# rasd3/TODA

Hardware: AMD Instinct MI355X
Metric: LiDAR training samples/sec (higher is better)
Workload: dtype f32

## Files before the change

include/toda.h:

```cpp
#ifndef TODA_H_
#define TODA_H_

#include <stddef.h>
#include <stdint.h>

#ifdef __cplusplus
extern "C" {
#endif

#define TODA_OK 0
#define TODA_EINVAL (-1)
#define TODA_EWORKSPACE (-2)
#define TODA_ELAUNCH (-3)
#define TODA_EFAULT (-4)

#define TODA_FAULT_BN2D 1u
#define TODA_FAULT_WINO 2u
#define TODA_FAULT_FPS 4u

const char* toda_last_error(void);
int toda_abi_version(void);
int toda_device_fault(void);

size_t toda_voxelize_workspace_bytes(int n_points, int max_voxels);
int toda_voxelize_hard(const float* points, int n, int c,
                       const float* range_host ,
                       const float* vsize_host ,
                       const int32_t* grid_host ,
                       int max_pts, int max_voxels,
                       float* voxels, int32_t* coords_zyx, int32_t* num_pts,
                       int32_t* m_dev, void* ws, size_t ws_bytes, void* stream);
size_t toda_voxelize_batch_workspace_bytes(int batch, int n_cap);
int toda_voxelize_batch(const float* const* points_host, const int32_t* n_points_host, int batch, int n_cap,
                        int c, int row_stride,
                        const float* range_host, const float* vsize_host, const int32_t* grid_host,
                        int max_pts, int max_voxels,
                        float* voxels, int32_t* coords_bzyx, int32_t* num_pts, int32_t* counts_dev,
                        void* ws, size_t ws_bytes, int ws_clean, void* stream);

int toda_mean_vfe_fwd(const float* voxels, const float* num_pts, int m, int p, int c,
                      float* out, void* stream);
int toda_mean_vfe_bwd(const float* grad_out, const float* num_pts, int m, int p, int c,
                      float* grad_voxels, void* stream);

size_t toda_dynvox_workspace_bytes(int n, int batch, const int32_t* grid_host, int pillar);
int toda_dynvox_count(const float* points, int n, int width, int batch, const float* range_host, const float* vsize_host,
                      const int32_t* grid_host, int pillar, int32_t* counts_dev, void* ws, size_t ws_bytes, void* stream);
int toda_dynvox_index(const float* points, int n, int width, int batch, const float* range_host, const float* vsize_host,
                      const int32_t* grid_host, int pillar, int m, int k, uint8_t* keep, int32_t* rows, int32_t* inv,
                      int32_t* seg_pts, int32_t* seg_off, int32_t* cnt, int32_t* coords, void* ws, size_t ws_bytes,
                      void* stream);
int toda_dynvox_seg_sum(const float* src, int ld, int col0, int ncol, const int32_t* rowmap, const int32_t* seg_off,
                        const int32_t* seg_pts, int m, int divide, float* out, void* stream);
int toda_dynvox_pillar_decorate(const float* points, int width, const int32_t* rows, const int32_t* inv,
                                const int32_t* coords, const float* mean, int k, const float* vsize_host,
                                const float* offset_host, int use_abs_xyz, int with_dist, float* out, int f, void* stream);
int toda_dynvox_seg_max_fwd(const float* x, int c, const int32_t* seg_off, const int32_t* seg_pts, int m, float* out,
                            int32_t* arg, void* stream);
int toda_dynvox_seg_max_bwd(const float* gout, const int32_t* arg, int m, int c, int k, float* gx, void* stream);
int toda_dynvox_gather_concat(const float* x, const float* xmax, const int32_t* inv, int k, int c, float* out, void* stream);

size_t toda_gridindex_bytes(int batch, const int32_t* shape_host );
int toda_gridindex_from_coords(const int32_t* idx, int n, const int32_t* n_dev,
                               int batch, const int32_t* shape_host,
                               void* gi, int32_t* rowof, void* stream);
int toda_gridindex_from_coords_unordered(const int32_t* idx, int n, const int32_t* n_dev,
                                         int batch, const int32_t* shape_host,
                                         void* gi, int32_t* rowof, int gi_clean, void* stream);
int toda_gridindex_clear(const int32_t* idx, int n, const int32_t* n_dev, int batch,
                         const int32_t* shape_host, void* gi, void* stream);
int toda_gridindex_from_conv(const int32_t* idx_in, int n_in, const int32_t* n_in_dev,
                             int batch, const int32_t* shape_in_host,
                             const int32_t* ksize_host, const int32_t* stride_host,
                             const int32_t* pad_host, const int32_t* shape_out_host,
                             void* gi_out, int32_t* idx_out, int32_t* n_out_dev,
                             int out_cap, void* stream);
int toda_gridindex_from_bitmap(const void* gi_in, int batch, const int32_t* shape_in_host,
                               const int32_t* ksize_host, const int32_t* stride_host,
                               const int32_t* pad_host, const int32_t* shape_out_host,
                               void* gi_out, int32_t* idx_out, int32_t* n_out_dev,
                               int out_cap, int in_rows_marked, void* stream);

int toda_rulebook_subm(const int32_t* idx, int n, int batch, const int32_t* shape_host,
                       const int32_t* ksize_host, const int32_t* dilation_host,
                       const void* gi, const int32_t* rowof,
                       int32_t* nbr, int32_t* pair_cnt, int cnt_zeroed, void* stream);
int toda_rulebook_conv(const int32_t* idx_in, int n_in, int batch,
                       const int32_t* shape_in_host, const int32_t* ksize_host,
                       const int32_t* stride_host, const int32_t* pad_host,
                       const int32_t* shape_out_host, const void* gi_out, int n_out,
                       int32_t* nbr_o2i, int32_t* nbr_i2o, int32_t* pair_cnt,
                       const int32_t* idx_out, const void* gi_in, const int32_t* rowof_in,
                       int cnt_zeroed, void* stream);

size_t toda_spconv_packed_weight_floats(int k_vol, int c_gather, int c_produce);
int toda_matrix_path(void);
int toda_set_matrix_path(int mode);
int toda_spconv_split_supported(int c_gather, int c_produce);
int toda_spconv_pack_weight(const float* w, int cout, int k_vol, int cin,
                            int transpose, int flip_k, float* wp, void* stream);
int toda_spconv_pack_weights(int n, const float* const* w_host, const int32_t* cout_host, const int32_t* k_vol_host,
                             const int32_t* cin_host, const int32_t* transpose_host, const int32_t* flip_k_host,
                             float* const* wp_host, void* stream);
int toda_spconv_gather_gemm(const float* in, int n_in, int c_gather, const float* wp,
                            const int32_t* nbr, int n_out, int k_vol, int c_produce,
                            const float* bias , float* out, void* stream);
int toda_spconv_gather_gemm_ordered(const float* in, int n_in, int c_gather, const float* wp,
                                    const int32_t* nbr, int n_out, int k_vol, int c_produce,
                                    const float* bias, float* out, const int32_t* order, void* stream);

int toda_rulebook_class_order(const int32_t* in_coords, int n_in, const int32_t* stride_host, const int32_t* padding_host,
                              int32_t* order, unsigned char* cls_sorted, void* stream);
int toda_spconv_gather_gemm_classed(const float* in, int n_in, int c_gather, const float* wp, const int32_t* nbr, int n_out,
                                    int k_vol, int c_produce, const float* bias, float* out, const int32_t* order,
                                    const unsigned char* cls_sorted, const int32_t* ksize_host, const int32_t* stride_host,
                                    const int32_t* padding_host, void* stream);
int toda_spconv_gather_gemm_compact_supported(int c_gather, int c_produce, int k_vol);
int toda_spconv_gather_gemm_compact(const float* in, int n_in, int c_gather, const float* w, int w_cout, int w_cin,
                                    int transpose, int flip_k, const int32_t* nbr, int n_out, int k_vol, int c_produce,
                                    const float* bias , float* out, void* stream);
size_t toda_spconv_gather_gemm_compact_stats_doubles(int n_out, int c_produce);
int toda_spconv_gather_gemm_compact_stats(const float* in, int n_in, int c_gather, const float* w, int w_cout, int w_cin,
                                          int transpose, int flip_k, const int32_t* nbr, int n_out, int k_vol,
                                          int c_produce, const float* bias , float* out, double* sums,
                                          size_t sums_doubles, int* blocks_out , void* stream);

size_t toda_spconv_wgrad_workspace_bytes(int n_out, int k_vol, int cin, int cout);
int toda_spconv_wgrad(const float* in, int n_in, const float* dout, const int32_t* nbr,
                      int n_out, int k_vol, int cin, int cout, float* dw,
                      void* ws, size_t ws_bytes, void* stream);
int toda_sparse_to_dense_fwd(const float* feat, const int32_t* idx, int n, int c,
                             int batch, const int32_t* shape_host, float* dense, void* stream);
int toda_sparse_to_dense_bwd(const float* grad_dense, const int32_t* idx, int n, int c,
                             int batch, const int32_t* shape_host, float* grad_feat, void* stream);

int toda_pillar_scatter_fwd(const float* feat, const int32_t* idx, int n, int c,
                            int batch, int ny, int nx, float* canvas, void* stream);
int toda_pillar_scatter_bwd(const float* grad_canvas, const int32_t* idx, int n, int c,
                            int batch, int ny, int nx, float* grad_feat, void* stream);

size_t toda_rows_reduce_doubles(int n, int c);
int toda_rows_moments(const float* x, int n, int c, double* sums ,
                      void* stream);
int toda_rows_affine_act(const float* x, const float* scale, const float* shift,
                         const float* residual , int n, int c, int relu,
                         float* y, void* stream);

int toda_bn_finalize(const double* sums , int n, int c,
                     const float* gamma, const float* beta, float* running_mean ,
                     float* running_var , float momentum, float eps, int training,
                     float* mean, float* invstd, float* scale, float* shift, void* stream);
int toda_bn_finalize_partials(double* sums, int blocks, int n, int c, const float* gamma, const float* beta,
                              float* running_mean , float* running_var , float momentum, float eps,
                              float* mean, float* invstd, float* scale, float* shift, void* stream);
int toda_rows_bn_bwd(const float* dy, const float* x, const float* stats, const float* gamma,
                     int n, int c, int relu, double* sums , float* dx,
                     void* stream);

int toda_rows_bn_bwd_res(const float* dy, const float* x, const float* residual , const float* stats,
                         const float* gamma, int n, int c, int relu, double* sums, float* dx,
                         float* dres , void* stream);
size_t toda_rows_bn_bwd_colsum_doubles(int n, int c);
int toda_rows_bn_bwd_res_colsum(const float* dy, const float* x, const float* residual , const float* stats,
                                const float* gamma, int n, int c, int relu, double* sums, float* dx,
                                float* dres , double* colsum_ws , float* dx_colsum ,
                                void* stream);

int toda_bn2d_supported(int batch, int c, int hw);
size_t toda_bn2d_sync_bytes(void);
int toda_bn2d_fwd(const float* x, int batch, int c, int hw, const float* gamma, const float* beta,
                  float* running_mean , float* running_var , float momentum, float eps, int relu,
                  float* y, float* save, void* sync , unsigned epoch, void* stream);
int toda_bn2d_bwd(const float* x, const float* dy, int batch, int c, int hw, const float* gamma, const float* beta,
                  const float* save, int relu, float* dx, float* dgamma, float* dbeta, void* sync ,
                  unsigned epoch, void* stream);
int toda_bn2d_fwd_into(const float* x, int batch, int c, int hw, const float* gamma, const float* beta,
                       float* running_mean , float* running_var , float momentum, float eps, int relu,
                       float* y, int y_channels, int y_channel0, float* save, void* sync , unsigned epoch,
                       void* stream);
int toda_bn2d_bwd_from(const float* x, const float* dy, int dy_channels, int dy_channel0, int batch, int c, int hw,
                       const float* gamma, const float* beta, const float* save, int relu, float* dx, float* dgamma,
                       float* dbeta, void* sync , unsigned epoch, void* stream);

int toda_center_assign(const float* gt_boxes, int batch, int n_gt, int code_size,
                       int num_classes, int fm_w, int fm_h,
                       const float* range_host , const float* vsize_host ,
                       int fm_stride, int max_objs, double gaussian_overlap, int min_radius,
                       float* heatmap ,
                       float* ret_boxes ,
                       int64_t* inds , int64_t* mask ,
                       void* stream);

size_t toda_anchor_assign_workspace_bytes(int batch, int n_gt);
int toda_anchor_assign(const void* const* anchors_host, const int32_t* locs_host, const int32_t* per_loc_host,
                       const float* matched_host, const float* unmatched_host, int n_classes, int anchor_stride,
                       const float* gt_boxes, int batch, int n_gt, int gt_stride, const int32_t* slot_of, int n_ids,
                       int code_size, int encode_angle_by_sincos, int multihead_order,
                       int32_t* labels , float* targets , float* weights ,
                       void* ws, size_t ws_bytes, void* stream);

int toda_boxes_iou_bev(const float* boxes_a, int na, const float* boxes_b, int nb,
                       float* iou , void* stream);
int toda_boxes_overlap_bev(const float* boxes_a, int na, const float* boxes_b, int nb,
                           float* overlap , void* stream);
size_t toda_nms_workspace_bytes(int n);
int toda_nms_rotated(const float* boxes_sorted, int n, float thresh, int64_t* keep ,
                     int32_t* n_keep_dev, void* ws, size_t ws_bytes, void* stream);

int toda_roi_grid_pool_bev(const float* feat, int B, int C, int H, int W, const float* rois, int N, int roi_stride,
                           float min_x, float min_y, float step_x, float step_y, int grid_size, float* out, void* stream);
int toda_roi_iou3d_max(const float* rois, int B, int N, int roi_stride, const int64_t* roi_labels, const float* gt, int M,
                       int gt_stride, int by_class, float* max_iou , int64_t* argmax , void* stream);

int toda_voxel_query(const float* new_xyz, const int32_t* new_coords, int M, const float* xyz, int N, const void* gi, const int32_t* rowof,
                     int batch, const int32_t* shape_host, float radius, const int32_t* ranges_host, int nsample, int32_t* idx,
                     uint8_t* empty, void* stream);
size_t toda_voxel_pool_moments_doubles(void);
int toda_voxel_pool_moments(const int32_t* idx, const uint8_t* empty, int M, int nsample, const float* xyz, int N, const float* new_xyz,
                            double* ws, void* stream);
int toda_voxel_pool_fwd(const float* f, int N, int C, const int32_t* idx, const uint8_t* empty, int M, int nsample, const float* xyz,
                        const float* new_xyz, const float* ab, float* out, uint8_t* arg, void* stream);
size_t toda_voxel_pool_table_bytes(int M, int nsample, int N);
int toda_voxel_pool_table(const int32_t* idx, const uint8_t* empty, int M, int nsample, int N, int32_t* off, int32_t* ent, void* ws,
                          size_t ws_bytes, void* stream);
int toda_voxel_pool_bwd_feat(const float* gout, const uint8_t* arg, int M, int nsample, int C, const int32_t* off, const int32_t* ent,
                             int N, float* gf, void* stream);
size_t toda_voxel_pool_bwd_pos_doubles(int C);
int toda_voxel_pool_bwd_pos(const float* gout, const uint8_t* arg, const int32_t* idx, const uint8_t* empty, int M, int nsample, int C,
                            const float* xyz, int N, const float* new_xyz, double* ws, float* gab, void* stream);

int toda_fps_resident_blocks(void);
size_t toda_fps_workspace_bytes(int batch, int npoint);
int toda_fps(const float* xyz, const int32_t* starts_host, int batch, int npoint, int mode, float* temp, int32_t* idx, void* ws,
             size_t ws_bytes, void* stream);
int toda_ball_query_stack(const float* xyz, int N, const int32_t* xyz_start, const float* new_xyz, const int32_t* new_start, int batch,
                          int M, int nr, const float* radii_host, const int32_t* nsample_host, int32_t* const* idx_host,
                          uint8_t* const* empty_host, void* stream);
int toda_sa_gather_fwd(const float* P, int N, int C, const float* wd, const int32_t* idx, const uint8_t* empty, int M, int nsample,
                       const float* xyz, const float* new_xyz, float* z, void* stream);
int toda_sa_gather_bwd_feat(const float* gz, int M, int nsample, int C, const int32_t* off, const int32_t* ent, int N, float* gP,
                            void* stream);
size_t toda_sa_gather_bwd_pos_doubles(int C);
int toda_sa_gather_bwd_pos(const float* gz, const int32_t* idx, const uint8_t* empty, int M, int nsample, int C, const float* xyz, int N,
                           const float* new_xyz, double* ws, float* gwd, void* stream);
int toda_sa_max_fwd(const float* y, int M, int nsample, int C, float* out, uint8_t* arg, void* stream);
int toda_sa_max_bwd(const float* g, const uint8_t* arg, int M, int nsample, int C, float* gy, void* stream);
int toda_bev_interp_fwd(const float* map, int B, int C, int H, int W, const float* xy, const int32_t* bidx, int K, float* out,
                        int32_t* taps, float* wts, void* stream);
int toda_bev_interp_bwd(const float* g, int K, int C, const int32_t* off, const int32_t* ent, const float* wts, int B, int H, int W,
                        float* gmap, void* stream);

int toda_points_in_boxes(const float* points, int n, const int32_t* n_dev, int c, const float* boxes,
                         int k, int box_stride, int mode, int32_t* flags, void* stream);
int toda_points_sector(const float* points, int n, const int32_t* n_dev, int c, double lo, double hi,
                       int32_t* flags, void* stream);
int toda_points_rect(const float* points, int n, const int32_t* n_dev, int c, const double* lo_xy_host,
                     const double* hi_xy_host, int closed, int32_t* flags, void* stream);
int toda_points_polar_cell(const float* points, int n, const int32_t* n_dev, int c, float phase,
                           const double* yaw_edges_host, int n_yaw, const double* dis_edges_host, int n_dis,
                           float dis_lo, float dis_hi, int32_t* cell, void* stream);
int toda_points_polar_select(const float* points, int n, const int32_t* n_dev, int c, double lo, double hi, int yaw_mode,
                             int dis_mode, double dis_th, const float* pitch_range_dev, int32_t* flags, void* stream);
size_t toda_points_pitch_range_workspace_bytes(void);
int toda_points_pitch_range(const float* points, int n, const int32_t* n_dev, int c, float* range_dev, void* ws,
                            size_t ws_bytes, void* stream);
int toda_points_pitch_band(const float* points, int n, const int32_t* n_dev, int c, float z_offset, float clip_lo,
                           float clip_hi, const double* edges_host, int n_bands, int32_t* band, void* stream);
size_t toda_rows_select_workspace_bytes(int n);
int toda_rows_select_append(const float* src, int n, const int32_t* n_dev, int c, const int32_t* keys,
                            int match, int invert, float* dst, int cap_rows, int32_t* cursor_dev,
                            void* ws, size_t ws_bytes, void* stream);
int toda_points_rotate_z(const float* src, int n, const int32_t* n_dev, int c, double cosv, double sinv,
                         float* dst, void* stream);
int toda_points_world_transform(const float* src, int n, const int32_t* n_dev, int c, int flip_x, int flip_y,
                                int rotate, float cosv, float sinv, int rescale, float scale, float* dst,
                                void* stream);

int toda_points_box_steps_chunk(void);
int toda_points_box_steps(const float* src, int n, const int32_t* n_dev, int c, const double* steps, int n_steps,
                          float* dst, int32_t* keep, void* stream);
size_t toda_points_column_range_workspace_bytes(void);
int toda_points_column_range(const float* points, int n, const int32_t* n_dev, int c, int col, float* range_dev,
                             void* ws, size_t ws_bytes, void* stream);
int toda_points_in_pyramids(const float* points, int n, const int32_t* n_dev, int c, const double* pyramids, int np,
                            uint32_t* bits, int32_t* counts, void* stream);

int toda_points_fov_flags(const float* points, int n, const int32_t* n_dev, int c, const float* m_host,
                          const float* p2_host, int img_h, int img_w, int32_t* flags, void* stream);

int toda_sweeps_merge_max_sweeps(void);
int toda_sweeps_merge(const float* rows, int n, int n_sweeps, const int32_t* offsets_host, const double* matrices_host,
                      const int32_t* has_matrix_host, const int32_t* drop_ego_host, const double* time_lags_host,
                      float radius, const float* shift_host, float* out, int32_t* flags, void* stream);

int toda_waymo_frame(const float* rows, int n, int c_in, int use_nlz, float* out, int32_t* flags, void* stream);

int toda_spconv_gather_gemm_stats_supported(int c_gather, int c_produce);
size_t toda_spconv_gather_gemm_stats_doubles(int n_out, int c_produce);
int toda_spconv_gather_gemm_stats(const float* in, int n_in, int c_gather, const float* packed_w, const int32_t* nbr,
                                  int n_out, int k_vol, int c_produce, const float* bias, float* out, double* sums,
                                  size_t sums_doubles, void* stream);
int toda_spconv_gather_gemm_stats_partials(const float* in, int n_in, int c_gather, const float* wp, const int32_t* nbr,
                                           int n_out, int k_vol, int c_produce, const float* bias , float* out,
                                           double* sums, size_t sums_doubles, int* blocks_out, void* stream);

int toda_conv3x3_supported(int batch, int cin, int cout, int H, int W);
size_t toda_conv3x3_weight_floats(int cout, int cin);
int toda_conv3x3_transform_weight(const float* w, int cout, int cin, int mode, float* u, void* stream);
typedef struct toda_conv3x3_weight_entry {
    const float* w;
    int32_t cout, cin, mode, reserved;
    float* u;
} toda_conv3x3_weight_entry;
int toda_conv3x3_transform_weight_batch(const toda_conv3x3_weight_entry* table_host, int n, void* stream);
size_t toda_conv3x3_workspace_bytes(void);
size_t toda_conv3x3_wgrad_workspace_bytes(int batch, int cin, int cout, int H, int W);
int toda_conv3x3_wgrad(const float* x, const float* dy, int batch, int cin, int cout, int H, int W, float* dw,
                       void* ws, size_t ws_bytes, void* stream);
int toda_conv3x3_fwd(const float* x, const float* u, const float* bias, int batch, int cin, int cout, int H,
                     int W, float* y, void* ws, size_t ws_bytes, void* stream);

int toda_conv3x3s2_supported(int batch, int cin, int cout, int H, int W);
int toda_conv3x3s2_fwd(const float* x, const float* w, int batch, int cin, int cout, int H, int W, float* y, void* stream);
int toda_conv3x3s2_dgrad(const float* dy, const float* w, int batch, int cin, int cout, int H, int W, float* dx, void* stream);
size_t toda_conv3x3s2_wgrad_workspace_bytes(int batch, int cin, int cout, int H, int W);
int toda_conv3x3s2_wgrad(const float* x, const float* dy, int batch, int cin, int cout, int H, int W, float* dw, void* ws,
                         size_t ws_bytes, void* stream);
int toda_deconv_supported(int batch, int cin, int cout, int H, int W, int s);
int toda_deconv_fwd(const float* x, const float* w, int batch, int cin, int cout, int H, int W, int s, float* y, void* stream);
int toda_deconv_dgrad(const float* dy, const float* w, int batch, int cin, int cout, int H, int W, int s, float* dx, void* stream);
size_t toda_deconv_wgrad_workspace_bytes(int batch, int cin, int cout, int H, int W, int s);
int toda_deconv_wgrad(const float* x, const float* dy, int batch, int cin, int cout, int H, int W, int s, float* dw, void* ws,
                      size_t ws_bytes, void* stream);

size_t toda_center_loss_workspace_bytes(int batch, int classes, int H, int W, int max_objs, int code_size);
int toda_center_loss_fwd(const float* hm_logits, const float* heatmap, int batch, int classes, int H, int W, int n_branch,
                         const float* const* reg_maps_host, const int32_t* reg_channels_host, const int64_t* inds,
                         const int64_t* mask, const float* target_boxes, int max_objs, int code_size,
                         const float* code_weights_host, float cls_weight, float loc_weight, float* hm_prob, float* out4,
                         void* ws, size_t ws_bytes, void* stream);
int toda_center_loss_bwd(const float* out4, const float* up_hm, const float* up_loc, int batch, int classes, int H, int W,
                         int n_branch, float* const* reg_grads_host, const int32_t* reg_channels_host, const int64_t* inds,
                         const int64_t* mask, int max_objs, int code_size, const float* code_weights_host, float cls_weight, float loc_weight,
                         float* hm_grad, const void* ws, size_t ws_bytes, void* stream);

int toda_conv3x3_narrow_supported(int batch, int cin, int cout, int H, int W);
int toda_conv3x3_narrow_fwd(int n, const float* const* x_host, const float* const* w_host, const float* const* bias_host,
                            const int32_t* cout_host, int batch, int cin, int H, int W, long long x_image_stride,
                            float* const* y_host, void* stream);
int toda_conv3x3_narrow_dgrad(int n, const float* const* dy_host, const float* const* w_host, const int32_t* cout_host,
                              int batch, int cin, int H, int W, long long dx_image_stride, float* const* dx_host, void* stream);
size_t toda_conv3x3_narrow_wgrad_workspace_bytes(int n, int batch, int cin, int H);
int toda_conv3x3_narrow_wgrad(int n, const float* const* x_host, const float* const* dy_host, const int32_t* cout_host,
                              int batch, int cin, int H, int W, long long x_image_stride, float* out, void* ws, size_t ws_bytes,
                              void* stream);

int toda_timing_begin(int capacity);
int toda_timing_end(float* ms_out_host, int cap, int* n_out_host);

int toda_clip_adam_chunk(void);
int toda_clip_adam_step(const unsigned long long* param, const unsigned long long* grad, const unsigned long long* exp_avg,
                        const unsigned long long* exp_avg_sq, const long long* numel, const int* chunk_tensor,
                        const long long* chunk_off, int n_chunks, double* partial, float* norm_out, float max_norm,
                        float lr, float beta1, float beta2, float eps, float weight_decay, int step, void* stream);

int toda_eval_overlaps(const float* box3d, const float* bbox, const int32_t* box_off, const float* query3d,
                       const float* query_bbox, const int32_t* query_off, const long long* out_off, int n_frames,
                       long long n_pairs, int metric, int criterion, float* out, void* stream);
size_t toda_eval_match_workspace_bytes(int n_frames, int n_thresh, int n_det_total);
int toda_eval_match_scores(const float* overlaps, const long long* ov_off, const int32_t* det_off, const int32_t* gt_off,
                           const int32_t* ign_det, const int32_t* ign_gt, const double* det_score, int n_frames,
                           int n_det_total, double min_overlap, double* scores_out, int32_t* count_out, void* ws,
                           size_t ws_bytes, void* stream);
int toda_eval_match(const float* overlaps, const long long* ov_off, const int32_t* det_off, const int32_t* gt_off,
                    const int32_t* ign_det, const int32_t* ign_gt, const double* det_score, const double* det_alpha,
                    const double* gt_alpha, const double* det_bbox, const double* dc_bbox, const int32_t* dc_off, int n_frames,
                    int n_det_total, const double* thresholds, int n_thresh, double min_overlap, int metric, int compute_aos,
                    double* pr, void* ws, size_t ws_bytes, void* stream);

#ifdef __cplusplus
}
#endif
#endif
```

toda_amd/csrc/bn_fold.cuh:

```cuda
#pragma once
#include "common.h"

namespace toda {

constexpr int DN_BLOCK = 256;

__device__ __forceinline__ double fold_column(const double* __restrict__ src, int blocks, double* part) {
    double acc = 0.0;
    for (int g = threadIdx.x; g < blocks; g += DN_BLOCK) acc += src[g];
    part[threadIdx.x] = acc;
    __syncthreads();
    for (int w = DN_BLOCK / 2; w > 0; w >>= 1) {
        if (threadIdx.x < w) part[threadIdx.x] += part[threadIdx.x + w];
        __syncthreads();
    }
    return part[0];
}

__device__ __forceinline__ void bn_write_channel(int ch, float mean, float var, float eps, const float* __restrict__ gamma,
                                                 const float* __restrict__ beta, float* __restrict__ mean_out,
                                                 float* __restrict__ invstd_out, float* __restrict__ scale_out,
                                                 float* __restrict__ shift_out) {
    const float invstd = 1.0f / sqrtf(var + eps);
    const float g = gamma ? gamma[ch] : 1.0f, b = beta ? beta[ch] : 0.0f;
    mean_out[ch] = mean;
    invstd_out[ch] = invstd;
    scale_out[ch] = g * invstd;
    shift_out[ch] = b - mean * g * invstd;
}

__device__ __forceinline__ void bn_train_channel(int ch, double sum, double sumsq, int n, const float* __restrict__ gamma,
                                                 const float* __restrict__ beta, float* __restrict__ running_mean,
                                                 float* __restrict__ running_var, float momentum, float eps,
                                                 float* __restrict__ mean_out, float* __restrict__ invstd_out,
                                                 float* __restrict__ scale_out, float* __restrict__ shift_out) {
    const double m = sum / (double)n;
    double v = sumsq / (double)n - m * m;
    if (v < 0.0) v = 0.0;
    const float mean = (float)m, var = (float)v;
    if (running_mean) {
        const double unbiased = n > 1 ? v * (double)n / (double)(n - 1) : v;
        running_mean[ch] = (1.0f - momentum) * running_mean[ch] + momentum * mean;
        running_var[ch] = (1.0f - momentum) * running_var[ch] + momentum * (float)unbiased;
    }
    bn_write_channel(ch, mean, var, eps, gamma, beta, mean_out, invstd_out, scale_out, shift_out);
}

__global__ void __launch_bounds__(DN_BLOCK) fold_partials_kernel(double* __restrict__ sums, int blocks, int cols);

}
```

toda_amd/csrc/dense.hip:

```cpp
#include "bn_fold.cuh"
#include "common.h"

namespace toda {

typedef float f32x4 __attribute__((ext_vector_type(4)));

constexpr int DN_ROWS = 64;
constexpr int DN_CH = 32;

struct DenseGeom {
    int D, H, W;
    int pillar;
};

__device__ __forceinline__ long long spatial_offset(const int4 q, const DenseGeom& g) {
    if (g.pillar) return (long long)q.y + (long long)q.z * g.W + q.w;
    return ((long long)q.y * g.H + q.z) * g.W + q.w;
}

template <bool FWD>
__global__ void __launch_bounds__(DN_BLOCK)
dense_tile_kernel(float* __restrict__ feat, const int4* __restrict__ idx, int n, int c, DenseGeom g,
                  float* __restrict__ dense) {
    __shared__ float tile[DN_CH][DN_ROWS + 1];
    __shared__ long long base[DN_ROWS];
    const int row0 = blockIdx.x * DN_ROWS, c0 = blockIdx.y * DN_CH;
    const long long vol = (long long)g.D * g.H * g.W;
    if (threadIdx.x < DN_ROWS) {
        const int r = row0 + threadIdx.x;
        long long b = -1;
        if (r < n) {
            const int4 q = idx[r];
            b = (long long)q.x * c * vol + spatial_offset(q, g);
        }
        base[threadIdx.x] = b;
    }
    const int fr = threadIdx.x >> 2, fc = (threadIdx.x & 3) * 8;
    const int dr = threadIdx.x & 63, dc = threadIdx.x >> 6;
    if (FWD) {
        if (row0 + fr < n) {
#pragma unroll
            for (int j = 0; j < 8; ++j) {
                const int ch = c0 + fc + j;
                tile[fc + j][fr] = ch < c ? feat[(size_t)(row0 + fr) * c + ch] : 0.f;
            }
        }
        __syncthreads();
        const long long b = base[dr];
        if (b >= 0) {
#pragma unroll
            for (int j = 0; j < DN_CH / 4; ++j) {
                const int ch = dc + 4 * j;
                if (c0 + ch < c) dense[b + (long long)(c0 + ch) * vol] = tile[ch][dr];
            }
        }
    } else {
        __syncthreads();
        const long long b = base[dr];
#pragma unroll
        for (int j = 0; j < DN_CH / 4; ++j) {
            const int ch = dc + 4 * j;
            tile[ch][dr] = (b >= 0 && c0 + ch < c) ? dense[b + (long long)(c0 + ch) * vol] : 0.f;
        }
        __syncthreads();
        if (row0 + fr < n) {
#pragma unroll
            for (int j = 0; j < 8; ++j) {
                const int ch = c0 + fc + j;
                if (ch < c) feat[(size_t)(row0 + fr) * c + ch] = tile[fc + j][fr];
            }
        }
    }
}

#ifndef TODA_MOM_ROWS
#define TODA_MOM_ROWS 256
#endif
constexpr int MOM_ROWS = TODA_MOM_ROWS;
constexpr int MOM_MAX_BLOCKS = 2048;

template <class Load>
__device__ __forceinline__ void rows_reduce2(int n, int c, int rows_per_block, Load load, double* __restrict__ sums) {
    __shared__ float sh[2][DN_BLOCK][4];
    const int lanes = c >> 2;
    const int rows_par = DN_BLOCK / lanes;
    const int cl = threadIdx.x % lanes, rsub = threadIdx.x / lanes;
    const int row_begin = blockIdx.x * rows_per_block;
    const int row_end = min(n, row_begin + rows_per_block);
    f32x4 s0 = f32x4{0.f, 0.f, 0.f, 0.f}, t0 = s0, s1 = s0, t1 = s0;
    int r = row_begin + rsub;
    for (; r + rows_par < row_end; r += 2 * rows_par) {
        f32x4 a, b, a2, b2;
        load(r, cl, a, b);
        load(r + rows_par, cl, a2, b2);
        s0 += a;
        t0 += b;
        s1 += a2;
        t1 += b2;
    }
    if (r < row_end) {
        f32x4 a, b;
        load(r, cl, a, b);
        s0 += a;
        t0 += b;
    }
    s0 += s1;
    t0 += t1;
#pragma unroll
    for (int j = 0; j < 4; ++j) {
        sh[0][threadIdx.x][j] = s0[j];
        sh[1][threadIdx.x][j] = t0[j];
    }
    __syncthreads();
    if (threadIdx.x < 2 * c) {
        const int q = threadIdx.x / c, ch = threadIdx.x % c;
        double acc = 0.0;
        for (int j = 0; j < rows_par; ++j) acc += sh[q][j * lanes + (ch >> 2)][ch & 3];
        sums[2 * c + (size_t)(q * c + ch) * gridDim.x + blockIdx.x] = acc;
    }
}

__global__ void __launch_bounds__(DN_BLOCK)
fold_partials_kernel(double* __restrict__ sums, int blocks, int cols) {
    __shared__ double part[DN_BLOCK];
    const double total = fold_column(sums + cols + (size_t)blockIdx.x * blocks, blocks, part);
    if (threadIdx.x == 0) sums[blockIdx.x] = total;
}

static inline void reduce_plan(int n, int* blocks, int* rows_per_block) {
    const int g = cdiv(n > 0 ? n : 1, MOM_ROWS);
    *blocks = g < MOM_MAX_BLOCKS ? g : MOM_MAX_BLOCKS;
    *rows_per_block = cdiv(n > 0 ? n : 1, *blocks);
}

__global__ void __launch_bounds__(DN_BLOCK)
rows_moments_kernel(const float* __restrict__ x, int n, int c, int rows_per_block, double* __restrict__ sums) {
    const f32x4* x4 = reinterpret_cast<const f32x4*>(x);
    const int lanes = c >> 2;
    rows_reduce2(n, c, rows_per_block, [&](int r, int cl, f32x4& a, f32x4& b) {
        a = x4[(size_t)r * lanes + cl];
        b = a * a;
    }, sums);
}

constexpr int EW_BLOCKS = 2048;

__global__ void __launch_bounds__(DN_BLOCK)
rows_affine_act_kernel(const f32x4* __restrict__ x, const float* __restrict__ scale, const float* __restrict__ shift,
                       const f32x4* __restrict__ res, long long n4, int c, int relu, f32x4* __restrict__ y) {
    const long long t0 = (long long)blockIdx.x * DN_BLOCK + threadIdx.x;
    const long long stride = (long long)gridDim.x * DN_BLOCK;
    const int ch = (int)((t0 * 4) % c);
    const f32x4 sc = *reinterpret_cast<const f32x4*>(scale + ch), sf = *reinterpret_cast<const f32x4*>(shift + ch);
    for (long long t = t0; t < n4; t += stride) {
        f32x4 v = x[t] * sc + sf;
        if (res) v += res[t];
        if (relu) {
#pragma unroll
            for (int j = 0; j < 4; ++j) v[j] = fmaxf(v[j], 0.f);
        }
        y[t] = v;
    }
}

__global__ void __launch_bounds__(DN_BLOCK)
rows_bn_bwd_reduce_kernel(const float* __restrict__ dy, const float* __restrict__ x, const float* __restrict__ res,
                          const float* __restrict__ stats, int n, int c, int relu, int rows_per_block,
                          double* __restrict__ sums) {
    const f32x4* dy4 = reinterpret_cast<const f32x4*>(dy);
    const f32x4* x4 = reinterpret_cast<const f32x4*>(x);
    const f32x4* r4 = reinterpret_cast<const f32x4*>(res);
    const int lanes = c >> 2;
    const int cl0 = threadIdx.x % lanes;
    const f32x4 mu = reinterpret_cast<const f32x4*>(stats)[cl0];
    const f32x4 is = reinterpret_cast<const f32x4*>(stats + c)[cl0];
    const f32x4 sc = reinterpret_cast<const f32x4*>(stats + 2 * c)[cl0];
    const f32x4 sf = reinterpret_cast<const f32x4*>(stats + 3 * c)[cl0];
    rows_reduce2(n, c, rows_per_block, [&](int r, int cl, f32x4& a, f32x4& b) {
        const f32x4 g = dy4[(size_t)r * lanes + cl], xv = x4[(size_t)r * lanes + cl];
        const f32x4 rv = r4 ? r4[(size_t)r * lanes + cl] : f32x4{0.f, 0.f, 0.f, 0.f};
#pragma unroll
        for (int j = 0; j < 4; ++j) {
            float pre = xv[j] * sc[j] + sf[j];
            if (r4) pre += rv[j];
            const float dz = (relu && !(pre > 0.f)) ? 0.f : g[j];
            a[j] = dz;
            b[j] = dz * ((xv[j] - mu[j]) * is[j]);
        }
    }, sums);
}

__global__ void __launch_bounds__(DN_BLOCK)
rows_bn_bwd_apply_kernel(const f32x4* __restrict__ dy, const f32x4* __restrict__ x, const f32x4* __restrict__ res,
                         const float* __restrict__ stats, const float* __restrict__ gamma, double* __restrict__ sums,
                         long long n4, int c, int n, int relu, f32x4* __restrict__ dx, f32x4* __restrict__ dres,
                         double* __restrict__ colsum_part) {
    if (blockIdx.x == 0 && threadIdx.x < 2 * c) reinterpret_cast<float*>(sums + 2 * c)[threadIdx.x] = (float)sums[threadIdx.x];
    const long long t0 = (long long)blockIdx.x * DN_BLOCK + threadIdx.x;
    const long long stride = (long long)gridDim.x * DN_BLOCK;
    const int ch = (int)((t0 * 4) % c);
    const float inv_n = 1.0f / (float)n;
    const f32x4 mu = *reinterpret_cast<const f32x4*>(stats + ch);
    const f32x4 is = *reinterpret_cast<const f32x4*>(stats + c + ch);
    const f32x4 sc = *reinterpret_cast<const f32x4*>(stats + 2 * c + ch);
    const f32x4 sf = *reinterpret_cast<const f32x4*>(stats + 3 * c + ch);
    const f32x4 ga = *reinterpret_cast<const f32x4*>(gamma + ch);
    f32x4 m1, m2;
#pragma unroll
    for (int j = 0; j < 4; ++j) {
        m1[j] = (float)(sums[ch + j] * (double)inv_n);
        m2[j] = (float)(sums[c + ch + j] * (double)inv_n);
    }
    const f32x4 k1 = ga * is, k2 = is * m2;
    f32x4 csum = {0.f, 0.f, 0.f, 0.f};
    for (long long t = t0; t < n4; t += stride) {
        const f32x4 g = dy[t], xv = x[t];
        const f32x4 rv = res ? res[t] : f32x4{0.f, 0.f, 0.f, 0.f};
        f32x4 out, dzv;
#pragma unroll
        for (int j = 0; j < 4; ++j) {
            float pre = xv[j] * sc[j] + sf[j];
            if (res) pre += rv[j];
            const float dz = (relu && !(pre > 0.f)) ? 0.f : g[j];
            dzv[j] = dz;
            out[j] = k1[j] * (dz - m1[j] - (xv[j] - mu[j]) * k2[j]);
        }
        dx[t] = out;
        csum += out;
        if (dres) dres[t] = dzv;
    }
    if (colsum_part) {
        __shared__ float cs[DN_BLOCK][4];
#pragma unroll
        for (int j = 0; j < 4; ++j) cs[threadIdx.x][j] = csum[j];
        __syncthreads();
        if (threadIdx.x < c) {
            const int lanes = c >> 2, cl = threadIdx.x >> 2, j = threadIdx.x & 3;
            double acc = 0.0;
            for (int t = cl; t < DN_BLOCK; t += lanes) acc += (double)cs[t][j];
            colsum_part[(size_t)threadIdx.x * gridDim.x + blockIdx.x] = acc;
        }
    }
}

__global__ void __launch_bounds__(DN_BLOCK)
colsum_fold_kernel(const double* __restrict__ part, int blocks, float* __restrict__ out) {
    __shared__ double sh[DN_BLOCK];
    const double total = fold_column(part + (size_t)blockIdx.x * blocks, blocks, sh);
    if (threadIdx.x == 0) out[blockIdx.x] = (float)total;
}

__global__ void __launch_bounds__(DN_BLOCK)
bn_finalize_kernel(const double* __restrict__ sums, int n, int c, const float* __restrict__ gamma,
                   const float* __restrict__ beta, float* __restrict__ running_mean, float* __restrict__ running_var,
                   float momentum, float eps, int training, float* __restrict__ mean_out, float* __restrict__ invstd_out,
                   float* __restrict__ scale_out, float* __restrict__ shift_out) {
    const int ch = threadIdx.x;
    if (ch >= c) return;
    if (training)
        bn_train_channel(ch, sums[ch], sums[c + ch], n, gamma, beta, running_mean, running_var, momentum, eps, mean_out, invstd_out,
                         scale_out, shift_out);
    else
        bn_write_channel(ch, running_mean[ch], running_var[ch], eps, gamma, beta, mean_out, invstd_out, scale_out, shift_out);
}

__global__ void __launch_bounds__(DN_BLOCK)
bn_fold_finalize_kernel(double* __restrict__ sums, int blocks, int n, int c, const float* __restrict__ gamma,
                        const float* __restrict__ beta, float* __restrict__ running_mean, float* __restrict__ running_var,
                        float momentum, float eps, float* __restrict__ mean_out, float* __restrict__ invstd_out,
                        float* __restrict__ scale_out, float* __restrict__ shift_out) {
    __shared__ double part[DN_BLOCK];
    const int ch = blockIdx.x;
    const double sum = fold_column(sums + 2 * c + (size_t)ch * blocks, blocks, part);
    __syncthreads();
    const double sumsq = fold_column(sums + 2 * c + (size_t)(c + ch) * blocks, blocks, part);
    if (threadIdx.x != 0) return;
    sums[ch] = sum;
    sums[c + ch] = sumsq;
    bn_train_channel(ch, sum, sumsq, n, gamma, beta, running_mean, running_var, momentum, eps, mean_out, invstd_out, scale_out,
                     shift_out);
}

static int ew_grid(long long n4, int c) {
    long long blocks = (n4 + DN_BLOCK - 1) / DN_BLOCK;
    if (blocks > EW_BLOCKS) blocks = EW_BLOCKS;
    while ((blocks * DN_BLOCK * 4) % c != 0) ++blocks;
    return (int)blocks;
}

static int scatter_common(bool fwd, float* feat, const int32_t* idx, int n, int c, int batch, DenseGeom g,
                          float* dense, hipStream_t s) {
    TODA_CHECK_ARG(n >= 0 && c >= 1 && batch >= 1, "sparse<->dense: bad sizes n=%d c=%d batch=%d", n, c, batch);
    const size_t total = (size_t)batch * c * g.D * g.H * g.W;
    if (fwd) TODA_HIP(hipMemsetAsync(dense, 0, total * sizeof(float), s));
    if (n == 0) return TODA_OK;
    const dim3 grid(cdiv(n, DN_ROWS), cdiv(c, DN_CH));
    if (fwd)
        hipLaunchKernelGGL(HIP_KERNEL_NAME(dense_tile_kernel<true>), grid, dim3(DN_BLOCK), 0, s, feat, (const int4*)idx, n,
                           c, g, dense);
    else
        hipLaunchKernelGGL(HIP_KERNEL_NAME(dense_tile_kernel<false>), grid, dim3(DN_BLOCK), 0, s, feat, (const int4*)idx, n,
                           c, g, dense);
    TODA_LAUNCH_CHECK();
    return TODA_OK;
}

}

using namespace toda;

extern "C" int toda_sparse_to_dense_fwd(const float* feat, const int32_t* idx, int n, int c, int batch,
                                        const int32_t* shape_host, float* dense, void* stream) {
    const DenseGeom g{shape_host[0], shape_host[1], shape_host[2], 0};
    return scatter_common(true, const_cast<float*>(feat), idx, n, c, batch, g, dense, (hipStream_t)stream);
}
extern "C" int toda_sparse_to_dense_bwd(const float* grad_dense, const int32_t* idx, int n, int c, int batch,
                                        const int32_t* shape_host, float* grad_feat, void* stream) {
    const DenseGeom g{shape_host[0], shape_host[1], shape_host[2], 0};
    return scatter_common(false, grad_feat, idx, n, c, batch, g, const_cast<float*>(grad_dense), (hipStream_t)stream);
}
extern "C" int toda_pillar_scatter_fwd(const float* feat, const int32_t* idx, int n, int c, int batch, int ny, int nx,
                                       float* canvas, void* stream) {
    const DenseGeom g{1, ny, nx, 1};
    return scatter_common(true, const_cast<float*>(feat), idx, n, c, batch, g, canvas, (hipStream_t)stream);
}
extern "C" int toda_pillar_scatter_bwd(const float* grad_canvas, const int32_t* idx, int n, int c, int batch, int ny,
                                       int nx, float* grad_feat, void* stream) {
    const DenseGeom g{1, ny, nx, 1};
    return scatter_common(false, grad_feat, idx, n, c, batch, g, const_cast<float*>(grad_canvas), (hipStream_t)stream);
}

extern "C" size_t toda_rows_reduce_doubles(int n, int c) {
    int blocks, rpb;
    reduce_plan(n, &blocks, &rpb);
    return (size_t)2 * c * (1 + (size_t)blocks);
}

extern "C" int toda_rows_moments(const float* x, int n, int c, double* sums, void* stream) {
    hipStream_t s = (hipStream_t)stream;
    TODA_CHECK_ARG(c >= 4 && c % 4 == 0 && c <= DN_BLOCK / 2 && DN_BLOCK % c == 0,
                   "rows_moments: channels must be a multiple of 4 dividing 256, <= 128 (got %d)", c);
    if (n <= 0) {
        TODA_HIP(hipMemsetAsync(sums, 0, 2 * c * sizeof(double), s));
        return TODA_OK;
    }
    int blocks, rpb;
    reduce_plan(n, &blocks, &rpb);
    hipLaunchKernelGGL(rows_moments_kernel, dim3(blocks), dim3(DN_BLOCK), 0, s, x, n, c, rpb, sums);
    hipLaunchKernelGGL(fold_partials_kernel, dim3(2 * c), dim3(DN_BLOCK), 0, s, sums, blocks, 2 * c);
    TODA_LAUNCH_CHECK();
    return TODA_OK;
}

extern "C" int toda_rows_affine_act(const float* x, const float* scale, const float* shift, const float* residual,
                                    int n, int c, int relu, float* y, void* stream) {
    TODA_CHECK_ARG(c >= 4 && c % 4 == 0 && c <= 1024, "rows_affine_act: channels must be a multiple of 4, <= 1024 (got %d)", c);
    if (n <= 0) return TODA_OK;
    const long long n4 = (long long)n * c / 4;
    hipLaunchKernelGGL(rows_affine_act_kernel, dim3(ew_grid(n4, c)), dim3(DN_BLOCK), 0, (hipStream_t)stream,
                       (const f32x4*)x, scale, shift, (const f32x4*)residual, n4, c, relu, (f32x4*)y);
    TODA_LAUNCH_CHECK();
    return TODA_OK;
}

extern "C" size_t toda_rows_bn_bwd_colsum_doubles(int n, int c) {
    if (n <= 0 || c < 4) return 1;
    return (size_t)c * ew_grid((long long)n * c / 4, c);
}

extern "C" int toda_rows_bn_bwd_res_colsum(const float* dy, const float* x, const float* residual, const float* stats,
                                           const float* gamma, int n, int c, int relu, double* sums, float* dx, float* dres,
                                           double* colsum_ws, float* dx_colsum, void* stream) {
    hipStream_t s = (hipStream_t)stream;
    TODA_CHECK_ARG((colsum_ws == nullptr) == (dx_colsum == nullptr), "rows_bn_bwd: colsum workspace and result go together");
    TODA_CHECK_ARG(c >= 4 && c % 4 == 0 && c <= DN_BLOCK / 2 && DN_BLOCK % c == 0,
                   "rows_bn_bwd: channels must be a multiple of 4 dividing 256, <= 128 (got %d)", c);
    if (n <= 0) {
        TODA_HIP(hipMemsetAsync(sums, 0, 3 * c * sizeof(double), s));
        if (dx_colsum) TODA_HIP(hipMemsetAsync(dx_colsum, 0, c * sizeof(float), s));
        return TODA_OK;
    }
    int blocks, rpb;
    reduce_plan(n, &blocks, &rpb);
    hipLaunchKernelGGL(rows_bn_bwd_reduce_kernel, dim3(blocks), dim3(DN_BLOCK), 0, s, dy, x, residual, stats, n, c, relu, rpb, sums);
    hipLaunchKernelGGL(fold_partials_kernel, dim3(2 * c), dim3(DN_BLOCK), 0, s, sums, blocks, 2 * c);
    const long long n4 = (long long)n * c / 4;
    const int grid = ew_grid(n4, c);
    hipLaunchKernelGGL(rows_bn_bwd_apply_kernel, dim3(grid), dim3(DN_BLOCK), 0, s, (const f32x4*)dy,
                       (const f32x4*)x, (const f32x4*)residual, stats, gamma, sums, n4, c, n, relu, (f32x4*)dx, (f32x4*)dres, colsum_ws);
    if (dx_colsum) hipLaunchKernelGGL(colsum_fold_kernel, dim3(c), dim3(DN_BLOCK), 0, s, (const double*)colsum_ws, grid, dx_colsum);
    TODA_LAUNCH_CHECK();
    return TODA_OK;
}

extern "C" int toda_rows_bn_bwd_res(const float* dy, const float* x, const float* residual, const float* stats,
                                    const float* gamma, int n, int c, int relu, double* sums, float* dx, float* dres,
                                    void* stream) {
    return toda_rows_bn_bwd_res_colsum(dy, x, residual, stats, gamma, n, c, relu, sums, dx, dres, nullptr, nullptr, stream);
}

extern "C" int toda_rows_bn_bwd(const float* dy, const float* x, const float* stats, const float* gamma, int n, int c,
                                int relu, double* sums, float* dx, void* stream) {
    return toda_rows_bn_bwd_res(dy, x, nullptr, stats, gamma, n, c, relu, sums, dx, nullptr, stream);
}

extern "C" int toda_bn_finalize_partials(double* sums, int blocks, int n, int c, const float* gamma, const float* beta,
                                         float* running_mean, float* running_var, float momentum, float eps, float* mean,
                                         float* invstd, float* scale, float* shift, void* stream) {
    TODA_CHECK_ARG(sums && mean && invstd && scale && shift, "bn_finalize_partials: null argument");
    TODA_CHECK_ARG(c >= 1 && c <= DN_BLOCK && blocks >= 1 && n >= 1, "bn_finalize_partials: channels must be <= 256, blocks and rows >= 1 (got %d, %d, %d)", c,
                   blocks, n);
    TODA_CHECK_ARG((running_mean == nullptr) == (running_var == nullptr), "bn_finalize_partials: running_mean and running_var go together");
    hipLaunchKernelGGL(bn_fold_finalize_kernel, dim3(c), dim3(DN_BLOCK), 0, (hipStream_t)stream, sums, blocks, n, c, gamma, beta, running_mean,
                       running_var, momentum, eps, mean, invstd, scale, shift);
    TODA_LAUNCH_CHECK();
    return TODA_OK;
}

extern "C" int toda_bn_finalize(const double* sums, int n, int c, const float* gamma, const float* beta,
                                float* running_mean, float* running_var, float momentum, float eps, int training,
                                float* mean, float* invstd, float* scale, float* shift, void* stream) {
    TODA_CHECK_ARG(c >= 1 && c <= DN_BLOCK, "bn_finalize: channels must be <= 256 (got %d)", c);
    TODA_CHECK_ARG(training || (running_mean && running_var), "bn_finalize: eval mode needs running statistics");
    TODA_CHECK_ARG(!training || n >= 1, "bn_finalize: training mode needs rows >= 1 (got %d)", n);
    hipLaunchKernelGGL(bn_finalize_kernel, dim3(1), dim3(DN_BLOCK), 0, (hipStream_t)stream, sums, n, c, gamma, beta,
                       running_mean, running_var, momentum, eps, training, mean, invstd, scale, shift);
    TODA_LAUNCH_CHECK();
    return TODA_OK;
}
```

toda_amd/csrc/spconv.hip:

```cpp
#include <stdlib.h>

#include <type_traits>

#include <hip/hip_ext.h>

#include <mutex>
#include <vector>

#include "bn_fold.cuh"
#include "common.h"


namespace toda {

typedef float f32x4 __attribute__((ext_vector_type(4)));

constexpr int SC_BLOCK = 256;

static int tiles_pow2(int channels) {
    int t = (channels + 15) / 16, p = 1;
    while (p < t) p <<= 1;
    return p;
}

// ... 919 lines not shown
    int max_chunks = env_chunks > 0 ? env_chunks : ((tiles_pow2(cin) * tiles_pow2(cout) >= 16) ? 48 : 144);
    if (env_chunks <= 0 && k_vol <= 9) max_chunks *= 2;
    int ch = k_vol <= 9 ? n_out / 1024 : n_out / 2048;
    if (ch < 1) ch = 1;
    if (ch > max_chunks) ch = max_chunks;
    if (env_chunks <= 0 && k_vol > 9 && max_chunks == 48 && n_out / 4096 > 48) ch = n_out / 4096 < 96 ? n_out / 4096 : 96;
    if (ch >= 8) ch = (ch + 7) / 8 * 8;
    int rpc = (n_out + ch - 1) / ch;
    rpc = (rpc + 15) / 16 * 16;
    if (rpc < 16) rpc = 16;
    *rows_per_chunk = rpc;
    *chunks = n_out > 0 ? (n_out + rpc - 1) / rpc : 1;
}

}

#include "spconv_split.cuh"

using namespace toda;

#include <atomic>
static std::atomic<int> g_matrix_path{-1};
static int matrix_path() {
    int m = g_matrix_path.load(std::memory_order_relaxed);
    if (m < 0) {
        const char* e = getenv("TODA_MM");
        m = (e && (e[0] == 'n' || e[0] == '0')) ? 0 : 1;
        g_matrix_path.store(m, std::memory_order_relaxed);
    }
    return m;
}
static inline bool use_split(int c_gather, int c_produce) { return matrix_path() == 1 && toda::split_shape_ok(c_gather, c_produce); }

extern "C" int toda_matrix_path(void) { return matrix_path(); }
extern "C" int toda_set_matrix_path(int mode) {
    TODA_CHECK_ARG(mode == 0 || mode == 1, "set_matrix_path: mode must be 0 (native) or 1 (split)");
    g_matrix_path.store(mode, std::memory_order_relaxed);
    return TODA_OK;
}
extern "C" int toda_spconv_split_supported(int c_gather, int c_produce) { return toda::split_shape_ok(c_gather, c_produce) ? 1 : 0; }

extern "C" size_t toda_spconv_packed_weight_floats(int k_vol, int c_gather, int c_produce) {
    const size_t native = (size_t)k_vol * tiles_pow2(c_gather) * tiles_pow2(c_produce) * 256;
    if (!toda::split_shape_ok(c_gather, c_produce)) return native;
    const size_t split = toda::split_packed_bytes(k_vol, c_gather, c_produce) / 4;
    return split > native ? split : native;
}

static void split_pack_fill(toda::SplitPackBatch& b, int i, const float* w, int cout, int k_vol, int cin, int transpose, int flip_k, float* wp) {
    const int cgather = transpose ? cout : cin, cprod = transpose ? cin : cout;
    b.w[i] = w, b.wps[i] = reinterpret_cast<toda::u32x4*>(wp), b.cout[i] = cout, b.K[i] = k_vol, b.cin[i] = cin;
    b.transpose[i] = transpose != 0, b.flip[i] = flip_k != 0;
    b.KC[i] = (unsigned char)(cgather / 32), b.NT[i] = (unsigned char)(cprod / 16);
}

extern "C" int toda_spconv_pack_weight(const float* w, int cout, int k_vol, int cin, int transpose, int flip_k,
                                       float* wp, void* stream) {
    TODA_CHECK_ARG(cout >= 1 && cin >= 1 && k_vol >= 1, "pack_weight: bad shape");
    const int cgather = transpose ? cout : cin, cprod = transpose ? cin : cout;
    TODA_CHECK_ARG(cgather <= 128 && cprod <= 128, "pack_weight: channels > 128 unsupported (gather %d, produce %d)",
                   cgather, cprod);
    if (use_split(cgather, cprod)) {
        toda::SplitPackBatch b = {};
        split_pack_fill(b, 0, w, cout, k_vol, cin, transpose, flip_k, wp);
        hipLaunchKernelGGL(split_pack_batch_kernel, dim3(cdiv((long long)k_vol * b.KC[0] * b.NT[0] * 192, SC_BLOCK), 1), dim3(SC_BLOCK), 0,
                           (hipStream_t)stream, b);
        TODA_LAUNCH_CHECK();
        return TODA_OK;
    }
    const int Q = tiles_pow2(cgather), NT = tiles_pow2(cprod);
    const long long total = (long long)k_vol * Q * NT * 256;
    hipLaunchKernelGGL(pack_weight_kernel, dim3(cdiv(total, SC_BLOCK)), dim3(SC_BLOCK), 0, (hipStream_t)stream, w, cout,
                       k_vol, cin, transpose, flip_k, Q, NT, wp);
    TODA_LAUNCH_CHECK();
    return TODA_OK;
}

extern "C" int toda_spconv_pack_weights(int n, const float* const* w, const int32_t* cout, const int32_t* k_vol, const int32_t* cin,
                                        const int32_t* transpose, const int32_t* flip_k, float* const* wp, void* stream) {
    TODA_CHECK_ARG(n >= 0 && w && cout && k_vol && cin && transpose && flip_k && wp, "pack_weights: null argument");
    PackBatch b = {};
    toda::SplitPackBatch sb = {};
    int m = 0, sm = 0;
    long long most = 0, smost = 0;
    auto flush = [&]() -> int {
        if (m > 0) {
            hipLaunchKernelGGL(pack_weight_batch_kernel, dim3(cdiv(most, SC_BLOCK), m), dim3(SC_BLOCK), 0, (hipStream_t)stream, b);
            TODA_LAUNCH_CHECK();
        }
        m = 0, most = 0;
        return TODA_OK;
    };
    auto sflush = [&]() -> int {
        if (sm > 0) {
            hipLaunchKernelGGL(split_pack_batch_kernel, dim3(cdiv(smost, SC_BLOCK), sm), dim3(SC_BLOCK), 0, (hipStream_t)stream, sb);
            TODA_LAUNCH_CHECK();
        }
        sm = 0, smost = 0;
        return TODA_OK;
    };
    for (int s = 0; s < n; ++s) {
        TODA_CHECK_ARG(w[s] && wp[s] && cout[s] >= 1 && cin[s] >= 1 && k_vol[s] >= 1, "pack_weights: bad segment %d", s);
        const int cgather = transpose[s] ? cout[s] : cin[s], cprod = transpose[s] ? cin[s] : cout[s];
        TODA_CHECK_ARG(cgather <= 128 && cprod <= 128, "pack_weights: channels > 128 unsupported (segment %d)", s);
        if (use_split(cgather, cprod)) {
            split_pack_fill(sb, sm, w[s], cout[s], k_vol[s], cin[s], transpose[s], flip_k[s], wp[s]);
            const long long total = (long long)k_vol[s] * sb.KC[sm] * sb.NT[sm] * 192;
            if (total > smost) smost = total;
            if (++sm == toda::SPLIT_PACK_MAX_SEG) {
                const int rc = sflush();
                if (rc != TODA_OK) return rc;
            }
            continue;
        }
        const int i = m;
        b.w[i] = w[s], b.wp[i] = wp[s], b.cout[i] = cout[s], b.K[i] = k_vol[s], b.cin[i] = cin[s];
        b.transpose[i] = transpose[s] != 0, b.flip[i] = flip_k[s] != 0;
        b.Q[i] = (unsigned char)tiles_pow2(cgather), b.NT[i] = (unsigned char)tiles_pow2(cprod);
        const long long total = (long long)k_vol[s] * b.Q[i] * b.NT[i] * 256;
        if (total > most) most = total;
        if (++m == PACK_MAX_SEG) {
            const int rc = flush();
            if (rc != TODA_OK) return rc;
        }
    }
    {
        const int rc = flush();
        if (rc != TODA_OK) return rc;
    }
    return sflush();
}

namespace toda {
constexpr int CLS_ROWS = 8192, CLS_PER = CLS_ROWS / 256;
struct ClassGeom {
    int stride[3], pad[3];
};
__global__ void __launch_bounds__(256)
class_order_kernel(const int4* __restrict__ coords, int n, const ClassGeom gm, int32_t* __restrict__ order, unsigned char* __restrict__ cls_sorted) {
    __shared__ int cnt[8][256 + 1];
    const int base = blockIdx.x * CLS_ROWS, t = threadIdx.x;
    unsigned char c[CLS_PER];
    int mine[8] = {0, 0, 0, 0, 0, 0, 0, 0};
#pragma unroll
    for (int i = 0; i < CLS_PER; ++i) {
        const int r = base + t * CLS_PER + i;
        int cl = 0;
        if (r < n) {
            const int4 v = coords[r];
            cl = (((v.y + gm.pad[0]) % gm.stride[0]) * gm.stride[1] + (v.z + gm.pad[1]) % gm.stride[1]) * gm.stride[2] + (v.w + gm.pad[2]) % gm.stride[2];
            ++mine[cl & 7];
        }
        c[i] = (unsigned char)cl;
    }
#pragma unroll
    for (int k = 0; k < 8; ++k) cnt[k][t] = mine[k];
    __syncthreads();
    if (t < 8) {
        int run = 0;
        for (int j = 0; j < 256; ++j) {
            const int v = cnt[t][j];
            cnt[t][j] = run;
            run += v;
        }
        cnt[t][256] = run;
    }
    __syncthreads();
    int cls_base[8], run = 0;
#pragma unroll
    for (int k = 0; k < 8; ++k) {
        cls_base[k] = run + cnt[k][t];
        run += cnt[k][256];
    }
#pragma unroll
    for (int i = 0; i < CLS_PER; ++i) {
        const int r = base + t * CLS_PER + i;
        if (r >= n) break;
        const int k = c[i] & 7;
        int pos = 0;
#pragma unroll
        for (int q = 0; q < 8; ++q)
            if (q == k) pos = cls_base[q]++;
        order[base + pos] = r;
        cls_sorted[base + pos] = c[i];
    }
}

static int class_table(const int32_t* ksize, const int32_t* stride, const int32_t* pad, GatherClasses* out) {
    const int n_class = stride[0] * stride[1] * stride[2];
    if (n_class < 1 || n_class > 8 || ksize[0] * ksize[1] * ksize[2] > 27) return -1;
    *out = GatherClasses{};
    for (int rz = 0; rz < stride[0]; ++rz)
        for (int ry = 0; ry < stride[1]; ++ry)
            for (int rx = 0; rx < stride[2]; ++rx) {
                const int c = (rz * stride[1] + ry) * stride[2] + rx;
                int m = 0;
                for (int kz = 0; kz < ksize[0]; ++kz)
                    for (int ky = 0; ky < ksize[1]; ++ky)
                        for (int kx = 0; kx < ksize[2]; ++kx)
                            if (kz % stride[0] == rz && ky % stride[1] == ry && kx % stride[2] == rx)
                                out->k[c][m++] = (unsigned char)((kz * ksize[1] + ky) * ksize[2] + kx);
                out->count[c] = (unsigned char)m;
            }
    return 0;
}
}

extern "C" int toda_rulebook_class_order(const int32_t* in_coords, int n_in, const int32_t* stride, const int32_t* padding, int32_t* order,
                                         unsigned char* cls_sorted, void* stream) {
    TODA_CHECK_ARG(in_coords && stride && padding && order && cls_sorted && n_in >= 0, "rulebook_class_order: null argument");
    ClassGeom gm;
    for (int a = 0; a < 3; ++a) {
        TODA_CHECK_ARG(stride[a] >= 1 && stride[a] <= 2 && padding[a] >= 0, "rulebook_class_order: stride 1 or 2 per axis (got %d)", stride[a]);
        gm.stride[a] = stride[a], gm.pad[a] = padding[a];
    }
    if (n_in == 0) return TODA_OK;
    hipLaunchKernelGGL(class_order_kernel, dim3(cdiv(n_in, CLS_ROWS)), dim3(256), 0, (hipStream_t)stream, (const int4*)in_coords, n_in, gm, order,
                       cls_sorted);
    TODA_LAUNCH_CHECK();
    return TODA_OK;
}

namespace toda {
struct LaunchTimer {
    std::vector<hipEvent_t> ev;
    int used = 0;
    bool on = false;
};
static LaunchTimer g_timer;
static std::mutex g_timer_mu;
static inline void timer_next(hipEvent_t* start, hipEvent_t* stop) {
    *start = *stop = nullptr;
    if (!g_timer.on) return;
    std::lock_guard<std::mutex> lock(g_timer_mu);
    if (!g_timer.on || 2 * (g_timer.used + 1) > (int)g_timer.ev.size()) return;
    *start = g_timer.ev[2 * g_timer.used];
    *stop = g_timer.ev[2 * g_timer.used + 1];
    g_timer.used++;
}
}

#define GG_LAUNCH(kernel, grid, block, shmem, stream, ...)                                              \
    do {                                                                                               \
        hipEvent_t t0_, t1_;                                                                           \
        toda::timer_next(&t0_, &t1_);                                                                  \
        hipExtLaunchKernelGGL(kernel, grid, block, shmem, stream, t0_, t1_, 0, __VA_ARGS__);           \
    } while (0)

extern "C" int toda_timing_begin(int capacity) {
    TODA_CHECK_ARG(capacity > 0 && capacity <= (1 << 20), "timing_begin: capacity in (0, 2^20]");
    std::lock_guard<std::mutex> lock(toda::g_timer_mu);
    for (hipEvent_t e : g_timer.ev) (void)hipEventDestroy(e);
    g_timer.ev.assign((size_t)2 * capacity, nullptr);
    for (auto& e : g_timer.ev) TODA_HIP(hipEventCreate(&e));
    g_timer.used = 0;
    g_timer.on = true;
    return TODA_OK;
}

extern "C" int toda_timing_end(float* ms_out, int cap, int* n_out) {
    std::lock_guard<std::mutex> lock(toda::g_timer_mu);
    g_timer.on = false;
    const int n = g_timer.used < cap ? g_timer.used : cap;
    for (int i = 0; i < n; ++i) {
        TODA_HIP(hipEventSynchronize(g_timer.ev[2 * i + 1]));
        TODA_HIP(hipEventElapsedTime(&ms_out[i], g_timer.ev[2 * i], g_timer.ev[2 * i + 1]));
    }
    if (n_out) *n_out = g_timer.used;
    for (hipEvent_t e : g_timer.ev) (void)hipEventDestroy(e);
    g_timer.ev.clear();
    g_timer.used = 0;
    return TODA_OK;
}

namespace toda {
static bool gg_stats_supported(int c_gather, int c_produce) {
    const int Q = tiles_pow2(c_gather), NT = tiles_pow2(c_produce);
    return (c_gather & 3) == 0 && Q >= 2 && NT >= Q && Q * NT <= 32 && !(Q == 8 && NT == 8) && c_produce % 4 == 0 && c_produce == 16 * NT;
}

template <int V>
using tile_c = std::integral_constant<int, V>;
template <class F>
static void with_tiles(int tiles, F&& f) {
    switch (tiles) {
        case 1: f(tile_c<1>{}); break;
        case 2: f(tile_c<2>{}); break;
        case 4: f(tile_c<4>{}); break;
        default: f(tile_c<8>{}); break;
    }
}
template <class F>
static void with_tiles(int a, int b, F&& f) {
    with_tiles(a, [&](auto ta) { with_tiles(b, [&](auto tb) { f(ta, tb); }); });
}

struct GatherRoute {
    enum Family { SPLIT, LDS_128, LDS, REG } family;
    int rt, block, grid;
    bool vec;
};
}

static int gather_route(int c_gather, int c_produce, int n_out, bool stats, bool cls_sorted, GatherRoute* r) {
    const int Q = tiles_pow2(c_gather), NT = tiles_pow2(c_produce);
    const bool vec_ok = (c_gather & 3) == 0;
    static const int env_lds_raw = getenv("TODA_GG_LDS") ? atoi(getenv("TODA_GG_LDS")) : 1;
    const int env_lds = env_lds_raw == 2 ? 1 : (env_lds_raw == 1 ? (Q >= 2 && NT >= Q) : 0);
    r->rt = 2, r->block = SC_BLOCK, r->vec = vec_ok;
    if (use_split(c_gather, c_produce)) {
        TODA_CHECK_ARG(!(cls_sorted && stats), "gather_gemm (split path): no statistics on a class-sorted launch");
        r->family = GatherRoute::SPLIT;
    } else if (vec_ok && Q == 8 && NT == 8 && !cls_sorted) {
        r->family = GatherRoute::LDS_128, r->rt = 1, r->block = 512;
    } else if ((env_lds || stats) && !cls_sorted && vec_ok && Q * NT <= 32) {
        r->family = GatherRoute::LDS, r->rt = NT < 8 ? 2 : 1;
    } else {
        TODA_CHECK_ARG(!stats, "gather_gemm: statistics requested on a launch shape without the fused epilogue");
        TODA_CHECK_ARG(vec_ok || Q == 1, "gather_gemm: gathered channel counts above 16 must be multiples of 4 (got %d)", c_gather);
        r->family = GatherRoute::REG;
        r->rt = NT < 8 ? 2 : (Q < 8 ? 1 : 2);
    }
    r->grid = cdiv(cdiv(n_out, 16 * r->rt), r->block / 64);
    return TODA_OK;
}

static int gather_gemm_impl(const float* in, int n_in, int c_gather, const float* wp, const int32_t* nbr, int n_out, int k_vol,
                            int c_produce, const float* bias, float* out, const int32_t* order, double* stats, int* blocks_out, void* stream,
                            const unsigned char* cls_sorted = nullptr, const toda::GatherClasses* cls_table = nullptr) {
    toda::GatherClasses classes = {};
    if (cls_sorted && cls_table) classes = *cls_table;
    else cls_sorted = nullptr;
    TODA_CHECK_ARG(c_gather >= 1 && c_gather <= 128 && c_produce >= 1 && c_produce <= 128,
                   "gather_gemm: channels must be in [1,128] (gather %d, produce %d)", c_gather, c_produce);
    TODA_CHECK_ARG(n_out >= 0 && n_in >= 0 && k_vol >= 1, "gather_gemm: bad sizes");
    TODA_CHECK_ARG((unsigned long long)n_in * c_gather * 4ull < 0xFFFFFFF0ull, "gather_gemm: gathered table must be < 4 GiB");
    if (n_out == 0) return TODA_OK;
    if (n_in == 0) {
        TODA_CHECK_ARG(bias == nullptr, "gather_gemm: empty input with bias is unsupported");
        TODA_HIP(hipMemsetAsync(out, 0, (size_t)n_out * c_produce * sizeof(float), (hipStream_t)stream));
        return TODA_OK;
    }
    GatherRoute r;
    const int rc = gather_route(c_gather, c_produce, n_out, stats != nullptr, cls_sorted != nullptr, &r);
    if (rc != TODA_OK) return rc;
    hipStream_t s = (hipStream_t)stream;
    const dim3 grid(r.grid), block(r.block);
    switch (r.family) {
        case GatherRoute::SPLIT:
            with_tiles(c_gather / 32, c_produce / 16, [&](auto kc, auto nt) {
                constexpr int KC = decltype(kc)::value, NT = decltype(nt)::value;
                if constexpr (KC <= 4 && NT >= 2)
                    GG_LAUNCH(HIP_KERNEL_NAME(gg_split_kernel<KC, NT, (NT == 8 ? 3 : 4), (NT == 2)>), grid, block, 0, s, in, n_in,
                              reinterpret_cast<const toda::u32x4*>(wp), nbr, n_out, k_vol, c_produce, bias, out, order, stats, cls_sorted, classes);
            });
            break;
        case GatherRoute::LDS_128:
            GG_LAUNCH(HIP_KERNEL_NAME(gather_gemm_lds_kernel<8, 8, 1, true, false, 512>), grid, block, 0, s, in, n_in, c_gather, wp, nbr, n_out,
                      k_vol, c_produce, bias, out, order, stats);
            break;
        case GatherRoute::LDS:
            with_tiles(tiles_pow2(c_gather), tiles_pow2(c_produce), [&](auto q, auto nt) {
                constexpr int Q = decltype(q)::value, NT = decltype(nt)::value, RT = NT < 8 ? 2 : 1;
                GG_LAUNCH(HIP_KERNEL_NAME(gather_gemm_lds_kernel<Q, NT, RT, true, true, SC_BLOCK, (Q <= 4 && NT <= 4 && RT == 2)>), grid, block, 0,
                          s, in, n_in, c_gather, wp, nbr, n_out, k_vol, c_produce, bias, out, order, stats);
            });
            break;
        case GatherRoute::REG: {
            auto reg = [&](auto q, auto nt, auto rt, auto vec) {
                constexpr int Q = decltype(q)::value, NT = decltype(nt)::value, RT = decltype(rt)::value;
                constexpr bool VEC = decltype(vec)::value;
                if (cls_sorted && VEC)
                    GG_LAUNCH(HIP_KERNEL_NAME(gather_gemm_kernel<Q, NT, RT, true, true>), grid, block, 0, s, in, n_in, c_gather, wp, nbr, n_out,
                              k_vol, c_produce, bias, out, order, cls_sorted, classes);
                else
                    GG_LAUNCH(HIP_KERNEL_NAME(gather_gemm_kernel<Q, NT, RT, VEC>), grid, block, 0, s, in, n_in, c_gather, wp, nbr, n_out, k_vol,
                              c_produce, bias, out, order, nullptr, classes);
            };
            if (!r.vec) {
                with_tiles(tiles_pow2(c_produce), [&](auto nt) {
                    reg(tile_c<1>{}, nt, tile_c<(decltype(nt)::value < 8 ? 2 : 1)>{}, std::false_type{});
                });
            } else {
                with_tiles(tiles_pow2(c_gather), tiles_pow2(c_produce), [&](auto q, auto nt) {
                    if constexpr (decltype(nt)::value < 8) reg(q, nt, tile_c<2>{}, std::true_type{});
                    else if (r.rt == 2) reg(q, nt, tile_c<2>{}, std::true_type{});
                    else reg(q, nt, tile_c<1>{}, std::true_type{});
                });
            }
            break;
        }
    }
    TODA_LAUNCH_CHECK();
    if (stats) {
        if (blocks_out) {
            *blocks_out = r.grid;
        } else {
            hipLaunchKernelGGL(toda::fold_partials_kernel, dim3(2 * c_produce), dim3(256), 0, s, stats, r.grid, 2 * c_produce);
            TODA_LAUNCH_CHECK();
        }
    }
    return TODA_OK;
}

extern "C" int toda_spconv_gather_gemm_ordered(const float* in, int n_in, int c_gather, const float* wp, const int32_t* nbr,
                                               int n_out, int k_vol, int c_produce, const float* bias, float* out,
                                               const int32_t* order, void* stream) {
    return gather_gemm_impl(in, n_in, c_gather, wp, nbr, n_out, k_vol, c_produce, bias, out, order, nullptr, nullptr, stream);
}

extern "C" int toda_spconv_gather_gemm_classed(const float* in, int n_in, int c_gather, const float* wp, const int32_t* nbr, int n_out, int k_vol,
                                               int c_produce, const float* bias, float* out, const int32_t* order,
                                               const unsigned char* cls_sorted, const int32_t* ksize, const int32_t* stride,
                                               const int32_t* padding, void* stream) {
    TODA_CHECK_ARG(order && cls_sorted && ksize && stride && padding, "gather_gemm_classed: null argument");
    TODA_CHECK_ARG(ksize[0] * ksize[1] * ksize[2] == k_vol, "gather_gemm_classed: kernel size does not match the table's %d offsets", k_vol);
    GatherClasses table;
    TODA_CHECK_ARG(class_table(ksize, stride, padding, &table) == 0, "gather_gemm_classed: needs <= 8 residue classes and <= 27 offsets");
    return gather_gemm_impl(in, n_in, c_gather, wp, nbr, n_out, k_vol, c_produce, bias, out, order, nullptr, nullptr, stream, cls_sorted, &table);
}

extern "C" int toda_spconv_gather_gemm_stats_supported(int c_gather, int c_produce) {
    return gg_stats_supported(c_gather, c_produce) ? 1 : 0;
}

extern "C" size_t toda_spconv_gather_gemm_stats_doubles(int n_out, int c_produce) {
    return (size_t)2 * c_produce * (1 + (size_t)cdiv(n_out > 0 ? n_out : 1, 64));
}

extern "C" int toda_spconv_gather_gemm_stats(const float* in, int n_in, int c_gather, const float* wp, const int32_t* nbr,
                                             int n_out, int k_vol, int c_produce, const float* bias, float* out, double* sums,
                                             size_t sums_doubles, void* stream) {
    TODA_CHECK_ARG(sums != nullptr && gg_stats_supported(c_gather, c_produce) && n_out > 0 && n_in > 0,
                   "gather_gemm_stats: unsupported channel pair (%d -> %d) or empty table", c_gather, c_produce);
    TODA_CHECK_ARG(sums_doubles >= toda_spconv_gather_gemm_stats_doubles(n_out, c_produce), "gather_gemm_stats: statistics buffer too small");
    return gather_gemm_impl(in, n_in, c_gather, wp, nbr, n_out, k_vol, c_produce, bias, out, nullptr, sums, nullptr, stream);
}

extern "C" int toda_spconv_gather_gemm_stats_partials(const float* in, int n_in, int c_gather, const float* wp, const int32_t* nbr,
                                                      int n_out, int k_vol, int c_produce, const float* bias, float* out, double* sums,
                                                      size_t sums_doubles, int* blocks_out, void* stream) {
    TODA_CHECK_ARG(sums != nullptr && blocks_out != nullptr && gg_stats_supported(c_gather, c_produce) && n_out > 0 && n_in > 0,
                   "gather_gemm_stats_partials: unsupported channel pair (%d -> %d), empty table or null argument", c_gather, c_produce);
    TODA_CHECK_ARG(sums_doubles >= toda_spconv_gather_gemm_stats_doubles(n_out, c_produce), "gather_gemm_stats_partials: statistics buffer too small");
    *blocks_out = 0;
    const int rc = gather_gemm_impl(in, n_in, c_gather, wp, nbr, n_out, k_vol, c_produce, bias, out, nullptr, sums, blocks_out, stream);
    if (rc == TODA_OK && *blocks_out <= 0) {
        set_error("gather_gemm_stats_partials: the launch took no statistics");
        return TODA_EINVAL;
    }
    return rc;
}

extern "C" int toda_spconv_gather_gemm(const float* in, int n_in, int c_gather, const float* wp, const int32_t* nbr,
                                       int n_out, int k_vol, int c_produce, const float* bias, float* out,
                                       void* stream) {
    return toda_spconv_gather_gemm_ordered(in, n_in, c_gather, wp, nbr, n_out, k_vol, c_produce, bias, out, nullptr, stream);
}

extern "C" int toda_spconv_gather_gemm_compact_supported(int c_gather, int c_produce, int k_vol) {
    return k_vol == CG_K && c_gather >= 1 && c_gather <= 32 && c_produce >= 1 && c_produce <= 32 && c_produce % 4 == 0;
}

static int gather_gemm_compact_impl(const float* in, int n_in, int c_gather, const float* w, int w_cout, int w_cin, int transpose,
                                    int flip_k, const int32_t* nbr, int n_out, int k_vol, int c_produce, const float* bias,
                                    float* out, double* stats, void* stream) {
    TODA_CHECK_ARG(toda_spconv_gather_gemm_compact_supported(c_gather, c_produce, k_vol),
                   "gather_gemm_compact: needs K = 27, <= 32 gathered and <= 32 produced channels (a multiple of 4) (got K %d, %d -> %d)", k_vol, c_gather,
                   c_produce);
    TODA_CHECK_ARG((transpose ? w_cout : w_cin) == c_gather && (transpose ? w_cin : w_cout) == c_produce,
                   "gather_gemm_compact: weight [%d][27][%d] (transpose %d) does not map %d -> %d channels", w_cout, w_cin, transpose, c_gather, c_produce);
    TODA_CHECK_ARG(n_out >= 0 && n_in >= 0, "gather_gemm_compact: bad sizes");
    TODA_CHECK_ARG((unsigned long long)n_in * c_gather * 4ull < 0xFFFFFFF0ull && (unsigned long long)n_out * CG_K * 4ull < 0xFFFFFFF0ull,
                   "gather_gemm_compact: gathered table and neighbour table must be < 4 GiB each");
    if (n_out == 0) return TODA_OK;
    hipStream_t s = (hipStream_t)stream;
    const dim3 grid(cdiv(n_out, CG_ROWS), cdiv(c_produce, 16));
    const bool vec = c_gather % 4 == 0;
#define CG_LAUNCH(QQ, VV)                                                                                                       \
    hipLaunchKernelGGL(HIP_KERNEL_NAME(gather_gemm_compact_kernel<QQ, VV>), grid, dim3(CG_BLOCK), 0, s, in, n_in, c_gather, w, w_cout, w_cin, \
                       transpose, flip_k, nbr, n_out, c_produce, bias, out, stats)
    if (c_gather <= 16) {
        if (vec) CG_LAUNCH(1, true);
        else CG_LAUNCH(1, false);
    } else {
        if (vec) CG_LAUNCH(2, true);
        else CG_LAUNCH(2, false);
    }
#undef CG_LAUNCH
    TODA_LAUNCH_CHECK();
    return TODA_OK;
}

extern "C" int toda_spconv_gather_gemm_compact(const float* in, int n_in, int c_gather, const float* w, int w_cout, int w_cin, int transpose,
                                               int flip_k, const int32_t* nbr, int n_out, int k_vol, int c_produce, const float* bias,
                                               float* out, void* stream) {
    return gather_gemm_compact_impl(in, n_in, c_gather, w, w_cout, w_cin, transpose, flip_k, nbr, n_out, k_vol, c_produce, bias, out, nullptr, stream);
}

extern "C" size_t toda_spconv_gather_gemm_compact_stats_doubles(int n_out, int c_produce) {
    return (size_t)2 * c_produce * (1 + (size_t)cdiv(n_out > 0 ? n_out : 1, CG_ROWS));
}

extern "C" int toda_spconv_gather_gemm_compact_stats(const float* in, int n_in, int c_gather, const float* w, int w_cout, int w_cin,
                                                     int transpose, int flip_k, const int32_t* nbr, int n_out, int k_vol, int c_produce,
                                                     const float* bias, float* out, double* sums, size_t sums_doubles, int* blocks_out,
                                                     void* stream) {
    TODA_CHECK_ARG(sums != nullptr && n_out > 0, "gather_gemm_compact_stats: null statistics buffer or no output rows");
    TODA_CHECK_ARG(sums_doubles >= toda_spconv_gather_gemm_compact_stats_doubles(n_out, c_produce), "gather_gemm_compact_stats: statistics buffer too small");
    const int rc = gather_gemm_compact_impl(in, n_in, c_gather, w, w_cout, w_cin, transpose, flip_k, nbr, n_out, k_vol, c_produce, bias, out, sums, stream);
    if (rc != TODA_OK) return rc;
    const int blocks = cdiv(n_out, CG_ROWS);
    if (blocks_out) {
        *blocks_out = blocks;
        return TODA_OK;
    }
    hipLaunchKernelGGL(toda::fold_partials_kernel, dim3(2 * c_produce), dim3(256), 0, (hipStream_t)stream, sums, blocks, 2 * c_produce);
    TODA_LAUNCH_CHECK();
    return TODA_OK;
}

extern "C" size_t toda_spconv_wgrad_workspace_bytes(int n_out, int k_vol, int cin, int cout) {
    int chunks, rpc;
    wgrad_plan(n_out, k_vol, cin, cout, &chunks, &rpc);
    return align_up((size_t)chunks * k_vol * cin * cout * sizeof(float), 256);
}

extern "C" int toda_spconv_wgrad(const float* in, int n_in, const float* dout, const int32_t* nbr, int n_out, int k_vol,
                                 int cin, int cout, float* dw, void* ws, size_t ws_bytes, void* stream) {
    TODA_CHECK_ARG(cin >= 1 && cin <= 128 && cout >= 1 && cout <= 128, "wgrad: channels must be in [1,128]");
    TODA_CHECK_ARG(n_out >= 0 && n_in >= 0 && k_vol >= 1, "wgrad: bad sizes");
    TODA_CHECK_ARG((unsigned long long)n_in * cin * 4ull < 0xFFFFFFF0ull && (unsigned long long)n_out * cout * 4ull < 0xFFFFFFF0ull,
                   "wgrad: feature tables must be < 4 GiB");
    hipStream_t s = (hipStream_t)stream;
    const long long elems = (long long)cout * k_vol * cin;
    if (n_out == 0 || n_in == 0) {
        TODA_HIP(hipMemsetAsync(dw, 0, elems * sizeof(float), s));
        return TODA_OK;
    }
    int chunks, rpc;
    wgrad_plan(n_out, k_vol, cin, cout, &chunks, &rpc);
    const size_t need = (size_t)chunks * elems * sizeof(float);
    if (ws_bytes < need) {
        set_error("wgrad: workspace %zu < required %zu", ws_bytes, need);
        return TODA_EWORKSPACE;
    }
    const int MT = tiles_pow2(cin), NT = tiles_pow2(cout);
    static const int env_sub = getenv("TODA_WG_SUB") ? atoi(getenv("TODA_WG_SUB")) : 7;
    static const int env_wg_xcd = getenv("TODA_WG_XCD") ? atoi(getenv("TODA_WG_XCD")) : 1;
    const int chunks_launch = env_wg_xcd ? (chunks + 7) / 8 * 8 : chunks;
    const int xcd_chunks = env_wg_xcd ? chunks_launch : -chunks;
    const bool exact = cin == 16 * MT && cout == 16 * NT;
    float* slab = (float*)ws;

    enum { SPLIT, COOP, TILED } family;
    int mtb = MT < 4 ? MT : 4, ntb = NT < 4 ? NT : 4, nsub_n = 1, grid = chunks_launch * k_vol;
    if (matrix_path() == 1 && toda::wgrad_split_shape_ok(cin, cout)) {
        family = SPLIT;
    } else if (MT == 8 && NT == 8 && (env_sub & 4)) {
        family = COOP, nsub_n = 2;
    } else {
        family = TILED;
        if (MT == 8 && (env_sub & 1)) mtb = 8;
        if (NT == 8 && (env_sub & 2)) ntb = 8;
        nsub_n = NT / ntb;
        grid *= (MT / mtb) * nsub_n;
    }
    auto split = [&](auto kernel) {
        hipLaunchKernelGGL(kernel, dim3(grid), dim3(SC_BLOCK), 0, s, in, n_in, dout, nbr, n_out, k_vol, rpc, slab, xcd_chunks);
    };
    auto native = [&](auto kernel) {
        hipLaunchKernelGGL(kernel, dim3(grid), dim3(SC_BLOCK), 0, s, in, n_in, cin, dout, cout, nbr, n_out, k_vol, rpc, MT, NT, nsub_n, slab,
                           xcd_chunks);
    };
    switch (family) {
        case SPLIT:
            if (cin == 128 && cout == 128) split(wgrad_split_kernel<4, 4, 2, 2>);
            else if (cin == 64 && cout == 128) split(wgrad_split_kernel<4, 4, 1, 2>);
            else if (cin == 128 && cout == 64) split(wgrad_split_kernel<4, 4, 2, 1>);
            else if (cin == 32 && cout == 32) split(wgrad_split_kernel<2, 2>);
            else if (cin == 32) split(wgrad_split_kernel<2, 4>);
            else if (cout == 32) split(wgrad_split_kernel<4, 2>);
            else split(wgrad_split_kernel<4, 4>);
            break;
        case COOP:
            if (exact) native(wgrad_kernel<4, 4, true, true>);
            else native(wgrad_kernel<4, 4, true>);
            break;
        case TILED:
            with_tiles(mtb, ntb, [&](auto m, auto n) {
                constexpr int MTB = decltype(m)::value, NTB = decltype(n)::value;
                if (exact) native(wgrad_kernel<MTB, NTB, false, true>);
                else native(wgrad_kernel<MTB, NTB>);
            });
            break;
    }
    hipLaunchKernelGGL(wgrad_reduce_kernel, dim3(cdiv(elems, SC_BLOCK)), dim3(SC_BLOCK), 0, s, slab, chunks, elems, dw);
    TODA_LAUNCH_CHECK();
    return TODA_OK;
}
```

toda_amd/csrc/spconv_split.cuh:

```cuda
#pragma once
#include "split_common.cuh"

namespace toda {

#ifndef WGS_ACCS
#define WGS_ACCS 2
#endif
#ifndef SP_STAMPS
#define SP_STAMPS 0
#endif
#if SP_STAMPS
#define SP_STAMP(i)                                                                               \
    do {                                                                                          \
        unsigned long long t_;                                                                    \
        __builtin_amdgcn_sched_barrier(0);                                                        \
        asm volatile("s_memtime %0\n\ts_waitcnt lgkmcnt(0)" : "=s"(t_)::"memory");                \
        __builtin_amdgcn_sched_barrier(0);                                                        \
        seg[i] += t_ - t_prev;                                                                    \
        t_prev = t_;                                                                              \
    } while (0)
#else
#define SP_STAMP(i)
#endif
#ifndef SP_ABLATE
#define SP_ABLATE 0
#endif
__device__ __forceinline__ void sp_split8(const f32x4& v0, const f32x4& v1, u32x4& h, u32x4& m, u32x4& l) {
#pragma unroll
    for (int p = 0; p < 4; ++p) {
        const float x0 = p < 2 ? v0[2 * p] : v1[2 * p - 4], x1 = p < 2 ? v0[2 * p + 1] : v1[2 * p - 3];
        h[p] = sp_pack_hi(x0, x1);
#if SP_ABLATE & 1
        m[p] = h[p] ^ 0x00010001u, l[p] = h[p] ^ 0x00020002u;
        continue;
#endif
        const float r0 = x0 - sp_trunc(x0), r1 = x1 - sp_trunc(x1);
        m[p] = sp_pack_hi(r0, r1);
        const float l0 = r0 - sp_trunc(r0), l1 = r1 - sp_trunc(r1);
        l[p] = sp_pack_hi(l0, l1);
    }
}
__device__ __forceinline__ unsigned short sp_plane_of(float v, int plane) {
    const float h = sp_trunc(v), r = v - h, m = sp_trunc(r), l = r - m;
    const float pick = plane == 0 ? h : (plane == 1 ? m : l);
    return (unsigned short)(__builtin_bit_cast(unsigned, pick) >> 16);
}

constexpr int SPLIT_PACK_MAX_SEG = 48;
struct SplitPackBatch {
    const float* w[SPLIT_PACK_MAX_SEG];
    u32x4* wps[SPLIT_PACK_MAX_SEG];
    int cout[SPLIT_PACK_MAX_SEG], K[SPLIT_PACK_MAX_SEG], cin[SPLIT_PACK_MAX_SEG];
    unsigned char transpose[SPLIT_PACK_MAX_SEG], flip[SPLIT_PACK_MAX_SEG], KC[SPLIT_PACK_MAX_SEG], NT[SPLIT_PACK_MAX_SEG];
};
__global__ void __launch_bounds__(SC_BLOCK)
split_pack_batch_kernel(const SplitPackBatch b) {
    const int sg = blockIdx.y;
    const int K = b.K[sg], KC = b.KC[sg], NT = b.NT[sg], cin = b.cin[sg], cout = b.cout[sg];
    const long long e = (long long)blockIdx.x * SC_BLOCK + threadIdx.x;
    if (e >= (long long)K * KC * NT * 192) return;
    const int lane = (int)(e & 63);
    long long t = e >> 6;
    const int plane = (int)(t % 3);
    t /= 3;
    const int n = (int)(t % NT);
    t /= NT;
    const int kc = (int)(t % KC);
    const int k = (int)(t / KC);
    const int c = lane & 15, g = lane >> 4;
    const int pch = NT * c + n;
    const int kk = b.flip[sg] ? K - 1 - k : k;
    const float* __restrict__ w = b.w[sg];
    unsigned short v[8];
#pragma unroll
    for (int j = 0; j < 8; ++j) {
        const int gch = 32 * kc + 16 * (j >> 2) + 4 * g + (j & 3);
        float x = 0.0f;
        if (!b.transpose[sg]) {
            if (gch < cin && pch < cout) x = w[((size_t)pch * K + kk) * cin + gch];
        } else {
            if (gch < cout && pch < cin) x = w[((size_t)gch * K + kk) * cin + pch];
        }
        v[j] = sp_plane_of(x, plane);
    }
    b.wps[sg][e] = u32x4{(unsigned)v[0] | ((unsigned)v[1] << 16), (unsigned)v[2] | ((unsigned)v[3] << 16), (unsigned)v[4] | ((unsigned)v[5] << 16),
                         (unsigned)v[6] | ((unsigned)v[7] << 16)};
}

template <int KC, int NT, int WAVES, bool IL = false>
__global__ void __launch_bounds__(SC_BLOCK, WAVES)
gg_split_kernel(const float* __restrict__ in, int n_in, const u32x4* __restrict__ wps, const int* __restrict__ nbr, int n_out, int K, int cp,
                const float* __restrict__ bias, float* __restrict__ out, const int* __restrict__ order, double* __restrict__ stats,
                const unsigned char* __restrict__ cls_sorted, const GatherClasses classes) {
    constexpr int RT = 2;
    constexpr int CG = 32 * KC;
    constexpr int UNITS = NT * 3;
    constexpr int SLICE = UNITS * 64;
    static_assert(2 * SLICE * 16 >= (SC_BLOCK / 64) * 2 * 16 * NT * 4, "the statistics scratch aliases the weight buffers");
    __shared__ u32x4 wl[2 * SLICE];
    const int lane = threadIdx.x & 63, wv = threadIdx.x >> 6;
    const int blk = xcd_chunked_block(blockIdx.x, gridDim.x);
    const int wave = blk * (SC_BLOCK / 64) + wv;
    const int r = lane & 15, g = lane >> 4;
    const int row0 = wave * (16 * RT);

    f32x4 acc[RT][NT];
#pragma unroll
    for (int n = 0; n < NT; ++n) {
        float b = 0.0f;
        if (bias && NT * r + n < cp) b = bias[NT * r + n];
#pragma unroll
        for (int rt = 0; rt < RT; ++rt) acc[rt][n] = f32x4{b, b, b, b};
    }
    const __amdgpu_buffer_rsrc_t in_rsrc = table_rsrc(in, (unsigned)n_in * (unsigned)CG * 4u);
    int rows[RT];
    bool live[RT];
#pragma unroll
    for (int rt = 0; rt < RT; ++rt) {
        live[rt] = row0 + rt * 16 + r < n_out;
        rows[rt] = live[rt] ? (order ? order[row0 + rt * 16 + r] : row0 + rt * 16 + r) : n_out - 1;
    }
    int KE = K;
    bool listed = false;
    unsigned long long kpack = 0;
    if (cls_sorted) {
        const int p = row0 + (lane & (16 * RT - 1));
        const int c = cls_sorted[p < n_out ? p : n_out - 1], c0 = __builtin_amdgcn_readfirstlane(c);
        const bool same = __all(c == c0 || p >= n_out);
        int* cw = reinterpret_cast<int*>(wl);
        if (lane == 0) cw[wv] = same ? c0 : -1;
        __syncthreads();
        int cb = cw[0];
#pragma unroll
        for (int w = 1; w < SC_BLOCK / 64; ++w) cb = (cw[w] == cb) ? cb : -1;
        __syncthreads();
        if (cb >= 0 && classes.count[cb & 7] > 0 && classes.count[cb & 7] <= 8) {
            listed = true;
            KE = classes.count[cb & 7];
#pragma unroll
            for (int i = 0; i < 8; ++i) kpack |= (unsigned long long)classes.k[cb & 7][i] << (8 * i);
            kpack = ((unsigned long long)__builtin_amdgcn_readfirstlane((int)(kpack >> 32)) << 32) | (unsigned)__builtin_amdgcn_readfirstlane((int)kpack);
        }
    }
    auto kof = [&](int j) { return listed ? (int)((kpack >> (8 * j)) & 0xFF) : j; };
    auto load_ids = [&](int j, int (&dst)[RT]) {
        const int kk = kof(j < KE ? j : KE - 1);
#pragma unroll
        for (int rt = 0; rt < RT; ++rt) {
            dst[rt] = __builtin_nontemporal_load(nbr + (size_t)kk * n_out + rows[rt]);
        }
    };
    auto gather = [&](const int (&src)[RT], int part, bool valid, f32x4 (&raw)[RT][2]) {
#pragma unroll
        for (int rt = 0; rt < RT; ++rt) {
            const bool ok = src[rt] >= 0 && valid;
            const unsigned base = (unsigned)src[rt] * (unsigned)(CG * 4) + (unsigned)(16 * g) + 128u * (unsigned)part;
#pragma unroll
            for (int i = 0; i < 2; ++i)
                raw[rt][i] = __builtin_bit_cast(f32x4, __builtin_amdgcn_raw_buffer_load_b128(in_rsrc, ok ? base + 64u * i : OOB, 0, 0));
        }
    };
    auto gather_rt = [&](const int (&src)[RT], int part, bool valid, f32x4 (&raw)[RT][2], int rt) {
        const bool ok = src[rt] >= 0 && valid;
        const unsigned base = (unsigned)src[rt] * (unsigned)(CG * 4) + (unsigned)(16 * g) + 128u * (unsigned)part;
#pragma unroll
        for (int i = 0; i < 2; ++i)
            raw[rt][i] = __builtin_bit_cast(f32x4, __builtin_amdgcn_raw_buffer_load_b128(in_rsrc, ok ? base + 64u * i : OOB, 0, 0));
    };
    auto stage = [&](int st, int buf) {
        const int sc = st < KE * KC ? st : KE * KC - 1;
        const int ss = kof(sc / KC) * KC + sc % KC;
#pragma unroll
        for (int t = 0; t < (UNITS + SC_BLOCK / 64 - 1) / (SC_BLOCK / 64); ++t) {
            const int u = t * (SC_BLOCK / 64) + wv;
            if (UNITS % (SC_BLOCK / 64) == 0 || u < UNITS)
                __builtin_amdgcn_global_load_lds(reinterpret_cast<const float*>(wps + (size_t)ss * SLICE + u * 64 + lane),
                                                 reinterpret_cast<float*>(&wl[buf * SLICE + u * 64]), 16, 0, 0);
        }
    };

    int idA[RT], idB[RT], idC[RT];
    f32x4 raw[RT][2];
    load_ids(0, idA);
    load_ids(1, idB);
    stage(0, 0);
    gather(idA, 0, true, raw);
    __syncthreads();

#if SP_STAMPS
    unsigned long long seg[6] = {0, 0, 0, 0, 0, 0}, t_prev;
    asm volatile("s_memtime %0\n\ts_waitcnt lgkmcnt(0)" : "=s"(t_prev)::"memory");
#endif
    auto body = [&](int k, const int (&ids_cur)[RT], const int (&ids_nxt)[RT], int (&ids_new)[RT]) {
        SP_STAMP(5);
        bool any = false;
#pragma unroll
        for (int rt = 0; rt < RT; ++rt) any = any || __any(ids_cur[rt] >= 0);
#pragma unroll
        for (int part = 0; part < KC; ++part) {
            const int cur = (k * KC + part) & 1;
            u32x4 ah[RT], am[RT], al[RT];
            f32x4 (&rw)[RT][2] = raw;
            if (any) {
#pragma unroll
                for (int rt = 0; rt < RT; ++rt) sp_split8(rw[rt][0], rw[rt][1], ah[rt], am[rt], al[rt]);
            }
            SP_STAMP(0);
            if constexpr (IL) {
                constexpr int PIECES = RT + 2;
                auto piece = [&](int p) {
                    if (p == 0) {
#if !(SP_ABLATE & 4)
                        stage(k * KC + part + 1, cur ^ 1);
#endif
                    } else if (p <= RT) {
                        if (part + 1 < KC) gather_rt(ids_cur, part + 1, true, raw, p - 1);
                        else gather_rt(ids_nxt, 0, k + 1 < KE, raw, p - 1);
                    } else if (part == KC - 1) load_ids(k + 2, ids_new);
                    asm volatile("" ::: "memory");
                };
                if (any) {
                    const u32x4* __restrict__ wb = wl + cur * SLICE + lane;
#pragma unroll
                    for (int n = 0; n < NT; ++n) {
                        const bf16x8 bh = __builtin_bit_cast(bf16x8, wb[(n * 3 + 0) * 64]), bm = __builtin_bit_cast(bf16x8, wb[(n * 3 + 1) * 64]),
                                     bl = __builtin_bit_cast(bf16x8, wb[(n * 3 + 2) * 64]);
#pragma unroll
                        for (int p = 0; p < PIECES; ++p)
                            if (p * NT / PIECES == n) piece(p);
#define SP_TERM(AA, BB)                                                                                                              \
    _Pragma("unroll") for (int rt = 0; rt < RT; ++rt)                                                                                \
        acc[rt][n] = __builtin_amdgcn_mfma_f32_16x16x32_bf16(__builtin_bit_cast(bf16x8, AA[rt]), BB, acc[rt][n], 0, 0, 0)
                        SP_TERM(al, bh);
                        SP_TERM(ah, bl);
                        SP_TERM(am, bm);
                        SP_TERM(am, bh);
                        SP_TERM(ah, bm);
                        SP_TERM(ah, bh);
#undef SP_TERM
                    }
                } else {
#pragma unroll
                    for (int p = 0; p < PIECES; ++p) piece(p);
                }
            } else {
#if !(SP_ABLATE & 4)
            stage(k * KC + part + 1, cur ^ 1);
#endif
            asm volatile("" ::: "memory");
#if SP_ABLATE & 8
            if (k < 0)
#endif
            if (part + 1 < KC) gather(ids_cur, part + 1, true, raw);
            else gather(ids_nxt, 0, k + 1 < KE, raw);
            asm volatile("" ::: "memory");
#if !(SP_ABLATE & 16)
            if (part == KC - 1) load_ids(k + 2, ids_new);
#endif
            asm volatile("" ::: "memory");
            SP_STAMP(1);
            if (any) {
                const u32x4* __restrict__ wb = wl + cur * SLICE + lane;
#pragma unroll
                for (int n = 0; n < NT; ++n) {
                    const bf16x8 bh = __builtin_bit_cast(bf16x8, wb[(n * 3 + 0) * 64]), bm = __builtin_bit_cast(bf16x8, wb[(n * 3 + 1) * 64]),
                                 bl = __builtin_bit_cast(bf16x8, wb[(n * 3 + 2) * 64]);
#if SP_ABLATE & 2
#define SP_TERM(AA, BB)                                                                                                              \
    _Pragma("unroll") for (int rt = 0; rt < RT; ++rt)                                                                                \
        acc[rt][n][0] += __builtin_bit_cast(float, AA[rt][0] ^ __builtin_bit_cast(u32x4, BB)[0])
#else
#define SP_TERM(AA, BB)                                                                                                              \
    _Pragma("unroll") for (int rt = 0; rt < RT; ++rt)                                                                                \
        acc[rt][n] = __builtin_amdgcn_mfma_f32_16x16x32_bf16(__builtin_bit_cast(bf16x8, AA[rt]), BB, acc[rt][n], 0, 0, 0)
#endif
                    SP_TERM(al, bh);
                    SP_TERM(ah, bl);
                    SP_TERM(am, bm);
                    SP_TERM(am, bh);
                    SP_TERM(ah, bm);
                    SP_TERM(ah, bh);
#undef SP_TERM
                }
            }
            }
            SP_STAMP(2);
#if SP_ABLATE & (4 | 8 | 16)
            asm volatile("s_waitcnt vmcnt(0)" ::: "memory");
#else
            if (part == KC - 1) asm volatile("s_waitcnt vmcnt(%0)" ::"n"(RT * 2 + RT) : "memory");
            else asm volatile("s_waitcnt vmcnt(%0)" ::"n"(RT * 2) : "memory");
#endif
            SP_STAMP(3);
            __builtin_amdgcn_s_barrier();
            SP_STAMP(4);
        }
    };
    for (int k = 0;;) {
        body(k, idA, idB, idC);
        if (++k >= KE) break;
        body(k, idB, idC, idA);
        if (++k >= KE) break;
        body(k, idC, idA, idB);
        if (++k >= KE) break;
    }
    asm volatile("s_waitcnt vmcnt(0)" ::: "memory");
    if (row0 >= n_out && !stats) return;

#if SP_STAMPS
    if (stats) {
        if (lane == 0)
            for (int i = 0; i < 6; ++i) reinterpret_cast<unsigned long long*>(stats)[(size_t)wave * 6 + i] = seg[i];
        stats = nullptr;
    }
#endif
    if (stats) {
        float (*st_sh)[2][16 * NT] = reinterpret_cast<float (*)[2][16 * NT]>(wl);
        float sm[NT], sq[NT];
#pragma unroll
        for (int n = 0; n < NT; ++n) {
            sm[n] = sq[n] = 0.0f;
#pragma unroll
            for (int rt = 0; rt < RT; ++rt)
#pragma unroll
                for (int reg = 0; reg < 4; ++reg)
                    if (row0 + rt * 16 + 4 * g + reg < n_out) {
                        const float v = acc[rt][n][reg];
                        sm[n] += v;
                        sq[n] += v * v;
                    }
            sm[n] += __shfl_xor(sm[n], 16, 64);
            sq[n] += __shfl_xor(sq[n], 16, 64);
            sm[n] += __shfl_xor(sm[n], 32, 64);
            sq[n] += __shfl_xor(sq[n], 32, 64);
            if (g == 0) {
                st_sh[wv][0][NT * r + n] = sm[n];
                st_sh[wv][1][NT * r + n] = sq[n];
            }
        }
        __syncthreads();
        if ((int)threadIdx.x < 2 * cp) {
            const int qq = threadIdx.x / cp, ch = threadIdx.x - qq * cp;
            double a = 0.0;
#pragma unroll
            for (int w = 0; w < SC_BLOCK / 64; ++w) a += (double)st_sh[w][qq][ch];
            stats[2 * cp + (size_t)(qq * cp + ch) * gridDim.x + blk] = a;
        }
    }

    const bool full = cp == 16 * NT;
#pragma unroll
    for (int rt = 0; rt < RT; ++rt) {
#pragma unroll
        for (int reg = 0; reg < 4; ++reg) {
            const int pos = row0 + rt * 16 + 4 * g + reg;
            const int row = __shfl(rows[rt], 4 * g + reg, 64);
            if (pos >= n_out) continue;
            float* dst = out + (size_t)row * cp + NT * r;
            if (full) {
                if constexpr (NT == 2) {
                    *reinterpret_cast<float2*>(dst) = make_float2(acc[rt][0][reg], acc[rt][1][reg]);
                } else {
#pragma unroll
                    for (int n = 0; n < NT; n += 4)
                        *reinterpret_cast<f32x4*>(dst + n) = f32x4{acc[rt][n][reg], acc[rt][n + 1][reg], acc[rt][n + 2][reg], acc[rt][n + 3][reg]};
                }
            } else {
#pragma unroll
                for (int n = 0; n < NT; ++n)
                    if (NT * r + n < cp) dst[n] = acc[rt][n][reg];
            }
        }
    }
}

template <int MTB, int NTB, int QM = 1, int QN = 1>
__global__ void __launch_bounds__(SC_BLOCK, (MTB * NTB <= 4) ? 4 : ((MTB == 4 && NTB == 2) ? 3 : 2))
wgrad_split_kernel(const float* __restrict__ in, int n_in, const float* __restrict__ dout, const int* __restrict__ nbr, int n_out, int K,
                   int rows_per_chunk, float* __restrict__ slab, int xcd_chunks) {
    static_assert((MTB == 2 || MTB == 4) && (NTB == 2 || NTB == 4), "32 or 64 channels a side");
    static_assert(QM * QN == 1 || (MTB == 4 && NTB == 4), "quarters are 64 x 64");
    static_assert(QM * QN == 1 || QM * QN == 2 || QM * QN == 4, "1, 2 or 4 quarters");
    constexpr int NQ = QM * QN, TEAMS = (SC_BLOCK / 64) / NQ;
    constexpr int MT = MTB * QM, NT = NTB * QN;
    constexpr int cin = 16 * MT, cout = 16 * NT;
    constexpr int QCAP = 64 + 32;
    __shared__ float red[TEAMS == 1 ? 1 : NQ * MTB * NTB * 4 * 64];
    __shared__ int q_in[SC_BLOCK / 64][QCAP], q_out[SC_BLOCK / 64][QCAP];
    const int lane = threadIdx.x & 63, wv = threadIdx.x >> 6;
    const int ii = lane & 15, g = lane >> 4;
    const int n_chunks = xcd_chunks < 0 ? -xcd_chunks : xcd_chunks;
    int chunk, k;
    {
        const int b = blockIdx.x;
        if (xcd_chunks > 0) {
            const int xcd = b & 7, t = (b >> 3) / K;
            k = (b >> 3) - t * K;
            chunk = t * 8 + xcd;
        } else {
            chunk = b % n_chunks;
            k = b / n_chunks;
        }
    }
    const int row_begin = chunk * rows_per_chunk;
    if (row_begin >= n_out) return;
    const int row_end = min(n_out, row_begin + rows_per_chunk);
    int* qi = q_in[wv];
    int* qo = q_out[wv];

    f32x4 acc[MTB][NTB];
#if WGS_ACCS >= 2
    f32x4 acc_s[MTB][NTB];
#endif
#if WGS_ACCS >= 3
    f32x4 acc_m[MTB][NTB];
#endif
#pragma unroll
    for (int m = 0; m < MTB; ++m)
#pragma unroll
        for (int n = 0; n < NTB; ++n) {
            acc[m][n] = f32x4{0.f, 0.f, 0.f, 0.f};
#if WGS_ACCS >= 2
            acc_s[m][n] = f32x4{0.f, 0.f, 0.f, 0.f};
#endif
#if WGS_ACCS >= 3
            acc_m[m][n] = f32x4{0.f, 0.f, 0.f, 0.f};
#endif
        }
    const __amdgpu_buffer_rsrc_t in_rsrc = table_rsrc(in, (unsigned)n_in * (unsigned)cin * 4u);
    const __amdgpu_buffer_rsrc_t dout_rsrc = table_rsrc(dout, (unsigned)n_out * (unsigned)cout * 4u);
    const int qd = wv % NQ, team = wv / NQ;
    const int m0 = (qd / QN) * MTB, n0 = (qd % QN) * NTB;
    const unsigned lane_a = (unsigned)(MT * ii + m0) * 4u, lane_b = (unsigned)(NT * ii + n0) * 4u;
    constexpr unsigned row_a = (unsigned)cin * 4u, row_b = (unsigned)cout * 4u;

    auto round32 = [&](int d, int limit, auto full_tag) {
        constexpr bool FULL = decltype(full_tag)::value;
        float a[8][MTB], b[8][NTB];
#pragma unroll
        for (int j = 0; j < 8; ++j) {
            const int p = d + 8 * g + j;
            const bool ok = FULL || p < limit;
            const int pc = ok ? p : d;
            const unsigned ia = (unsigned)qi[pc] + lane_a, ib = (unsigned)qo[pc] + lane_b;
            if constexpr (MTB == 4) {
                const f32x4 v = __builtin_bit_cast(f32x4, __builtin_amdgcn_raw_buffer_load_b128(in_rsrc, ok ? ia : OOB, 0, 0));
#pragma unroll
                for (int m = 0; m < 4; ++m) a[j][m] = v[m];
            } else {
                const f32x2w v = __builtin_bit_cast(f32x2w, __builtin_amdgcn_raw_buffer_load_b64(in_rsrc, ok ? ia : OOB, 0, 0));
                a[j][0] = v[0], a[j][1] = v[1];
            }
            if constexpr (NTB == 4) {
                const f32x4 v = __builtin_bit_cast(f32x4, __builtin_amdgcn_raw_buffer_load_b128(dout_rsrc, ok ? ib : OOB, 0, 0));
#pragma unroll
                for (int n = 0; n < 4; ++n) b[j][n] = v[n];
            } else {
                const f32x2w v = __builtin_bit_cast(f32x2w, __builtin_amdgcn_raw_buffer_load_b64(dout_rsrc, ok ? ib : OOB, 0, 0));
                b[j][0] = v[0], b[j][1] = v[1];
            }
        }
        u32x4 ah[MTB], am[MTB], al[MTB];
#pragma unroll
        for (int m = 0; m < MTB; ++m)
#pragma unroll
            for (int q = 0; q < 4; ++q) {
                unsigned h_, m_, l_;
                sp_split2(a[2 * q][m], a[2 * q + 1][m], h_, m_, l_);
                ah[m][q] = h_, am[m][q] = m_, al[m][q] = l_;
            }
#pragma unroll
        for (int n = 0; n < NTB; ++n) {
            u32x4 bh, bm, bl;
#pragma unroll
            for (int q = 0; q < 4; ++q) {
                unsigned h_, m_, l_;
                sp_split2(b[2 * q][n], b[2 * q + 1][n], h_, m_, l_);
                bh[q] = h_, bm[q] = m_, bl[q] = l_;
            }
#define WS_TERM(ACC, AA, BB)                                                                                             \
    _Pragma("unroll") for (int m = 0; m < MTB; ++m)                                                                       \
        ACC[m][n] = __builtin_amdgcn_mfma_f32_16x16x32_bf16(__builtin_bit_cast(bf16x8, AA[m]), __builtin_bit_cast(bf16x8, BB), ACC[m][n], 0, 0, 0)
#if WGS_ACCS == 1
            WS_TERM(acc, al, bh);
            WS_TERM(acc, ah, bl);
            WS_TERM(acc, am, bm);
            WS_TERM(acc, am, bh);
            WS_TERM(acc, ah, bm);
            WS_TERM(acc, ah, bh);
#elif WGS_ACCS == 2
            WS_TERM(acc_s, al, bh);
            WS_TERM(acc_s, ah, bl);
            WS_TERM(acc_s, am, bm);
            WS_TERM(acc, am, bh);
            WS_TERM(acc, ah, bm);
            WS_TERM(acc, ah, bh);
#else
            WS_TERM(acc_s, al, bh);
            WS_TERM(acc_s, ah, bl);
            WS_TERM(acc_s, am, bm);
            WS_TERM(acc_m, am, bh);
            WS_TERM(acc_m, ah, bm);
            WS_TERM(acc, ah, bh);
#endif
#undef WS_TERM
        }
    };

    int qn = 0;
    constexpr int BSTEP = TEAMS * 64;
    const int base0 = row_begin + team * 64;
    int iv_next = nbr[(size_t)k * n_out + min(base0 + lane, n_out - 1)];
    for (int base = base0; base < row_end; base += BSTEP) {
        const int o = base + lane;
        const int iv = iv_next;
        iv_next = nbr[(size_t)k * n_out + min(o + BSTEP, n_out - 1)];
        const int i = o < row_end ? iv : -1;
        const unsigned long long vote = __ballot(i >= 0);
        if (vote == 0) continue;
        if (i >= 0) {
            const int pos = qn + __popcll(vote & ((1ull << lane) - 1));
            qi[pos] = (int)((unsigned)i * row_a);
            qo[pos] = (int)((unsigned)o * row_b);
        }
        qn += __popcll(vote);
        __builtin_amdgcn_wave_barrier();
        int done = 0;
        while (qn - done >= 32) {
            round32(done, qn, std::true_type{});
            done += 32;
        }
        const int left = qn - done;
        if (done > 0 && left > 0) {
            int ti = 0, to = 0;
            if (lane < left) {
                ti = qi[done + lane];
                to = qo[done + lane];
            }
            __builtin_amdgcn_wave_barrier();
            if (lane < left) {
                qi[lane] = ti;
                qo[lane] = to;
            }
        }
        qn = left;
        __builtin_amdgcn_wave_barrier();
    }
    if (qn > 0) round32(0, qn, std::false_type{});
#if WGS_ACCS >= 2
#pragma unroll
    for (int m = 0; m < MTB; ++m)
#pragma unroll
        for (int n = 0; n < NTB; ++n) {
#if WGS_ACCS >= 3
            acc[m][n] = (acc_s[m][n] + acc_m[m][n]) + acc[m][n];
#else
            acc[m][n] = acc_s[m][n] + acc[m][n];
#endif
        }
#endif

    for (int src = 1; src < TEAMS; ++src) {
        float* const rq = red + qd * (MTB * NTB * 4 * 64);
        if (team == src) {
#pragma unroll
            for (int m = 0; m < MTB; ++m)
#pragma unroll
                for (int n = 0; n < NTB; ++n)
#pragma unroll
                    for (int reg = 0; reg < 4; ++reg) rq[((m * NTB + n) * 4 + reg) * 64 + lane] = acc[m][n][reg];
        }
        __syncthreads();
        if (team == 0) {
#pragma unroll
            for (int m = 0; m < MTB; ++m)
#pragma unroll
                for (int n = 0; n < NTB; ++n)
#pragma unroll
                    for (int reg = 0; reg < 4; ++reg) acc[m][n][reg] += rq[((m * NTB + n) * 4 + reg) * 64 + lane];
        }
        __syncthreads();
    }
    if (team != 0) return;
    float* dst = slab + (size_t)chunk * cout * K * cin;
#pragma unroll
    for (int m = 0; m < MTB; ++m)
#pragma unroll
        for (int n = 0; n < NTB; ++n)
#pragma unroll
            for (int reg = 0; reg < 4; ++reg) {
                const int ci = MT * (4 * g + reg) + m0 + m;
                const int co = NT * ii + n0 + n;
                dst[((size_t)co * K + k) * cin + ci] = acc[m][n][reg];
            }
}

static inline bool wgrad_split_shape_ok(int cin, int cout) {
    return ((cin == 32 || cin == 64) && (cout == 32 || cout == 64)) || ((cin == 64 || cin == 128) && (cout == 64 || cout == 128));
}

static inline bool split_shape_ok(int c_gather, int c_produce) {
    return (c_gather == 32 || c_gather == 64 || c_gather == 128) && (c_produce == 32 || c_produce == 64 || c_produce == 128);
}
static inline size_t split_packed_bytes(int k_vol, int c_gather, int c_produce) {
    return (size_t)k_vol * (c_gather / 32) * (c_produce / 16) * 3 * 1024;
}

}
```

toda_amd/lib.py:

```python
import ctypes as C
import os

import torch

_HERE = os.path.dirname(os.path.abspath(__file__))
LIB_PATH = os.environ.get("TODA_HIP_LIB") or os.path.join(_HERE, "libtoda_hip.so")

_vp, _i, _sz, _dbl = C.c_void_p, C.c_int, C.c_size_t, C.c_double

SIGNATURES = {
    "toda_last_error": (C.c_char_p, []),
    "toda_abi_version": (_i, []),
    "toda_device_fault": (_i, []),
    "toda_voxelize_workspace_bytes": (_sz, [_i, _i]),
    "toda_voxelize_hard": (_i, [_vp, _i, _i, _vp, _vp, _vp, _i, _i, _vp, _vp, _vp, _vp, _vp, _sz, _vp]),
    "toda_mean_vfe_fwd": (_i, [_vp, _vp, _i, _i, _i, _vp, _vp]),
    "toda_mean_vfe_bwd": (_i, [_vp, _vp, _i, _i, _i, _vp, _vp]),
    "toda_dynvox_workspace_bytes": (_sz, [_i, _i, _vp, _i]),
    "toda_dynvox_count": (_i, [_vp, _i, _i, _i, _vp, _vp, _vp, _i, _vp, _vp, _sz, _vp]),
    "toda_dynvox_index": (_i, [_vp, _i, _i, _i, _vp, _vp, _vp, _i, _i, _i, _vp, _vp, _vp, _vp, _vp, _vp, _vp, _vp, _sz, _vp]),
    "toda_dynvox_seg_sum": (_i, [_vp, _i, _i, _i, _vp, _vp, _vp, _i, _i, _vp, _vp]),
    "toda_dynvox_pillar_decorate": (_i, [_vp, _i, _vp, _vp, _vp, _vp, _i, _vp, _vp, _i, _i, _vp, _i, _vp]),
    "toda_dynvox_seg_max_fwd": (_i, [_vp, _i, _vp, _vp, _i, _vp, _vp, _vp]),
    "toda_dynvox_seg_max_bwd": (_i, [_vp, _vp, _i, _i, _i, _vp, _vp]),
    "toda_dynvox_gather_concat": (_i, [_vp, _vp, _vp, _i, _i, _vp, _vp]),
    "toda_gridindex_bytes": (_sz, [_i, _vp]),
    "toda_gridindex_from_coords": (_i, [_vp, _i, _vp, _i, _vp, _vp, _vp, _vp]),
    "toda_gridindex_from_conv": (_i, [_vp, _i, _vp, _i, _vp, _vp, _vp, _vp, _vp, _vp, _vp, _vp, _i, _vp]),
    "toda_rulebook_subm": (_i, [_vp, _i, _i, _vp, _vp, _vp, _vp, _vp, _vp, _vp, _i, _vp]),
    "toda_rulebook_conv": (_i, [_vp, _i, _i, _vp, _vp, _vp, _vp, _vp, _vp, _i, _vp, _vp, _vp, _vp, _vp, _vp, _i, _vp]),
    "toda_voxelize_batch_workspace_bytes": (_sz, [_i, _i]),
    "toda_voxelize_batch": (_i, [_vp, _vp, _i, _i, _i, _i, _vp, _vp, _vp, _i, _i, _vp, _vp, _vp, _vp, _vp, _sz, _i, _vp]),
    "toda_gridindex_from_coords_unordered": (_i, [_vp, _i, _vp, _i, _vp, _vp, _vp, _i, _vp]),
    "toda_gridindex_clear": (_i, [_vp, _i, _vp, _i, _vp, _vp, _vp]),
    "toda_gridindex_from_bitmap": (_i, [_vp, _i, _vp, _vp, _vp, _vp, _vp, _vp, _vp, _vp, _i, _i, _vp]),
    "toda_spconv_packed_weight_floats": (_sz, [_i, _i, _i]),
    "toda_matrix_path": (_i, []),
    "toda_set_matrix_path": (_i, [_i]),
    "toda_spconv_split_supported": (_i, [_i, _i]),
    "toda_spconv_pack_weight": (_i, [_vp, _i, _i, _i, _i, _i, _vp, _vp]),
    "toda_spconv_pack_weights": (_i, [_i, _vp, _vp, _vp, _vp, _vp, _vp, _vp, _vp]),
    "toda_spconv_gather_gemm": (_i, [_vp, _i, _i, _vp, _vp, _i, _i, _i, _vp, _vp, _vp]),
    "toda_spconv_gather_gemm_ordered": (_i, [_vp, _i, _i, _vp, _vp, _i, _i, _i, _vp, _vp, _vp, _vp]),
    "toda_rulebook_class_order": (_i, [_vp, _i, _vp, _vp, _vp, _vp, _vp]),
    "toda_spconv_gather_gemm_classed": (_i, [_vp, _i, _i, _vp, _vp, _i, _i, _i, _vp, _vp, _vp, _vp, _vp, _vp, _vp, _vp]),
    "toda_spconv_gather_gemm_stats_supported": (_i, [_i, _i]),
    "toda_spconv_gather_gemm_stats_doubles": (_sz, [_i, _i]),
    "toda_spconv_gather_gemm_stats": (_i, [_vp, _i, _i, _vp, _vp, _i, _i, _i, _vp, _vp, _vp, _sz, _vp]),
    "toda_spconv_gather_gemm_stats_partials": (_i, [_vp, _i, _i, _vp, _vp, _i, _i, _i, _vp, _vp, _vp, _sz, _vp, _vp]),
    "toda_spconv_gather_gemm_compact_supported": (_i, [_i, _i, _i]),
    "toda_spconv_gather_gemm_compact": (_i, [_vp, _i, _i, _vp, _i, _i, _i, _i, _vp, _i, _i, _i, _vp, _vp, _vp]),
    "toda_spconv_gather_gemm_compact_stats_doubles": (_sz, [_i, _i]),
    "toda_spconv_gather_gemm_compact_stats": (_i, [_vp, _i, _i, _vp, _i, _i, _i, _i, _vp, _i, _i, _i, _vp, _vp, _vp, _sz, _vp, _vp]),
    "toda_spconv_wgrad_workspace_bytes": (_sz, [_i, _i, _i, _i]),
    "toda_spconv_wgrad": (_i, [_vp, _i, _vp, _vp, _i, _i, _i, _i, _vp, _vp, _sz, _vp]),
    "toda_sparse_to_dense_fwd": (_i, [_vp, _vp, _i, _i, _i, _vp, _vp, _vp]),
    "toda_sparse_to_dense_bwd": (_i, [_vp, _vp, _i, _i, _i, _vp, _vp, _vp]),
    "toda_pillar_scatter_fwd": (_i, [_vp, _vp, _i, _i, _i, _i, _i, _vp, _vp]),
    "toda_pillar_scatter_bwd": (_i, [_vp, _vp, _i, _i, _i, _i, _i, _vp, _vp]),
    "toda_rows_reduce_doubles": (_sz, [_i, _i]),
    "toda_rows_moments": (_i, [_vp, _i, _i, _vp, _vp]),
    "toda_rows_affine_act": (_i, [_vp, _vp, _vp, _vp, _i, _i, _i, _vp, _vp]),
    "toda_bn_finalize": (_i, [_vp, _i, _i, _vp, _vp, _vp, _vp, C.c_float, C.c_float, _i, _vp, _vp, _vp, _vp, _vp]),
    "toda_bn_finalize_partials": (_i, [_vp, _i, _i, _i, _vp, _vp, _vp, _vp, C.c_float, C.c_float, _vp, _vp, _vp, _vp, _vp]),
    "toda_rows_bn_bwd": (_i, [_vp, _vp, _vp, _vp, _i, _i, _i, _vp, _vp, _vp]),
    "toda_rows_bn_bwd_res": (_i, [_vp, _vp, _vp, _vp, _vp, _i, _i, _i, _vp, _vp, _vp, _vp]),
    "toda_rows_bn_bwd_colsum_doubles": (_sz, [_i, _i]),
    "toda_rows_bn_bwd_res_colsum": (_i, [_vp, _vp, _vp, _vp, _vp, _i, _i, _i, _vp, _vp, _vp, _vp, _vp, _vp]),
    "toda_conv3x3s2_supported": (_i, [_i, _i, _i, _i, _i]),
    "toda_conv3x3s2_fwd": (_i, [_vp, _vp, _i, _i, _i, _i, _i, _vp, _vp]),
    "toda_conv3x3s2_dgrad": (_i, [_vp, _vp, _i, _i, _i, _i, _i, _vp, _vp]),
    "toda_conv3x3s2_wgrad_workspace_bytes": (_sz, [_i, _i, _i, _i, _i]),
    "toda_conv3x3s2_wgrad": (_i, [_vp, _vp, _i, _i, _i, _i, _i, _vp, _vp, _sz, _vp]),
    "toda_deconv_supported": (_i, [_i, _i, _i, _i, _i, _i]),
    "toda_deconv_fwd": (_i, [_vp, _vp, _i, _i, _i, _i, _i, _i, _vp, _vp]),
    "toda_deconv_dgrad": (_i, [_vp, _vp, _i, _i, _i, _i, _i, _i, _vp, _vp]),
    "toda_deconv_wgrad_workspace_bytes": (_sz, [_i, _i, _i, _i, _i, _i]),
    "toda_deconv_wgrad": (_i, [_vp, _vp, _i, _i, _i, _i, _i, _i, _vp, _vp, _sz, _vp]),
    "toda_bn2d_supported": (_i, [_i, _i, _i]),
    "toda_bn2d_sync_bytes": (_sz, []),
    "toda_bn2d_fwd": (_i, [_vp, _i, _i, _i, _vp, _vp, _vp, _vp, C.c_float, C.c_float, _i, _vp, _vp, _vp, C.c_uint, _vp]),
    "toda_bn2d_bwd": (_i, [_vp, _vp, _i, _i, _i, _vp, _vp, _vp, _i, _vp, _vp, _vp, _vp, C.c_uint, _vp]),
    "toda_bn2d_fwd_into": (_i, [_vp, _i, _i, _i, _vp, _vp, _vp, _vp, C.c_float, C.c_float, _i, _vp, _i, _i, _vp, _vp, C.c_uint, _vp]),
    "toda_bn2d_bwd_from": (_i, [_vp, _vp, _i, _i, _i, _i, _i, _vp, _vp, _vp, _i, _vp, _vp, _vp, _vp, C.c_uint, _vp]),
    "toda_boxes_iou_bev": (_i, [_vp, _i, _vp, _i, _vp, _vp]),
    "toda_boxes_overlap_bev": (_i, [_vp, _i, _vp, _i, _vp, _vp]),
    "toda_nms_workspace_bytes": (_sz, [_i]),
    "toda_nms_rotated": (_i, [_vp, _i, C.c_float, _vp, _vp, _vp, _sz, _vp]),
    "toda_roi_grid_pool_bev": (_i, [_vp, _i, _i, _i, _i, _vp, _i, _i, C.c_float, C.c_float, C.c_float, C.c_float, _i, _vp, _vp]),
    "toda_roi_iou3d_max": (_i, [_vp, _i, _i, _i, _vp, _vp, _i, _i, _i, _vp, _vp, _vp]),
    "toda_voxel_query": (_i, [_vp, _vp, _i, _vp, _i, _vp, _vp, _i, _vp, C.c_float, _vp, _i, _vp, _vp, _vp]),
    "toda_voxel_pool_moments_doubles": (_sz, []),
    "toda_voxel_pool_moments": (_i, [_vp, _vp, _i, _i, _vp, _i, _vp, _vp, _vp]),
    "toda_voxel_pool_fwd": (_i, [_vp, _i, _i, _vp, _vp, _i, _i, _vp, _vp, _vp, _vp, _vp, _vp]),
    "toda_voxel_pool_table_bytes": (_sz, [_i, _i, _i]),
    "toda_voxel_pool_table": (_i, [_vp, _vp, _i, _i, _i, _vp, _vp, _vp, _sz, _vp]),
    "toda_voxel_pool_bwd_feat": (_i, [_vp, _vp, _i, _i, _i, _vp, _vp, _i, _vp, _vp]),
    "toda_voxel_pool_bwd_pos_doubles": (_sz, [_i]),
    "toda_voxel_pool_bwd_pos": (_i, [_vp, _vp, _vp, _vp, _i, _i, _i, _vp, _i, _vp, _vp, _vp, _vp]),
    "toda_fps_resident_blocks": (_i, []),
    "toda_fps_workspace_bytes": (_sz, [_i, _i]),
    "toda_fps": (_i, [_vp, _vp, _i, _i, _i, _vp, _vp, _vp, _sz, _vp]),
    "toda_ball_query_stack": (_i, [_vp, _i, _vp, _vp, _vp, _i, _i, _i, _vp, _vp, _vp, _vp, _vp]),
    "toda_sa_gather_fwd": (_i, [_vp, _i, _i, _vp, _vp, _vp, _i, _i, _vp, _vp, _vp, _vp]),
    "toda_sa_gather_bwd_feat": (_i, [_vp, _i, _i, _i, _vp, _vp, _i, _vp, _vp]),
    "toda_sa_gather_bwd_pos_doubles": (_sz, [_i]),
    "toda_sa_gather_bwd_pos": (_i, [_vp, _vp, _vp, _i, _i, _i, _vp, _i, _vp, _vp, _vp, _vp]),
    "toda_sa_max_fwd": (_i, [_vp, _i, _i, _i, _vp, _vp, _vp]),
    "toda_sa_max_bwd": (_i, [_vp, _vp, _i, _i, _i, _vp, _vp]),
    "toda_bev_interp_fwd": (_i, [_vp, _i, _i, _i, _i, _vp, _vp, _i, _vp, _vp, _vp, _vp]),
    "toda_bev_interp_bwd": (_i, [_vp, _i, _i, _vp, _vp, _vp, _i, _i, _i, _vp, _vp]),
    "toda_clip_adam_chunk": (_i, []),
    "toda_clip_adam_step": (_i, [_vp, _vp, _vp, _vp, _vp, _vp, _vp, _i, _vp, _vp, C.c_float, C.c_float, C.c_float, C.c_float, C.c_float, C.c_float, _i, _vp]),
    "toda_points_in_boxes": (_i, [_vp, _i, _vp, _i, _vp, _i, _i, _i, _vp, _vp]),
    "toda_points_sector": (_i, [_vp, _i, _vp, _i, _dbl, _dbl, _vp, _vp]),
    "toda_points_rect": (_i, [_vp, _i, _vp, _i, _vp, _vp, _i, _vp, _vp]),
    "toda_points_polar_cell": (_i, [_vp, _i, _vp, _i, C.c_float, _vp, _i, _vp, _i, C.c_float, C.c_float, _vp, _vp]),
    "toda_points_polar_select": (_i, [_vp, _i, _vp, _i, _dbl, _dbl, _i, _i, _dbl, _vp, _vp, _vp]),
    "toda_points_pitch_range_workspace_bytes": (_sz, []),
    "toda_points_pitch_range": (_i, [_vp, _i, _vp, _i, _vp, _vp, _sz, _vp]),
    "toda_points_pitch_band": (_i, [_vp, _i, _vp, _i, C.c_float, C.c_float, C.c_float, _vp, _i, _vp, _vp]),
    "toda_rows_select_workspace_bytes": (_sz, [_i]),
    "toda_rows_select_append": (_i, [_vp, _i, _vp, _i, _vp, _i, _i, _vp, _i, _vp, _vp, _sz, _vp]),
    "toda_points_rotate_z": (_i, [_vp, _i, _vp, _i, _dbl, _dbl, _vp, _vp]),
    "toda_points_world_transform": (_i, [_vp, _i, _vp, _i, _i, _i, _i, C.c_float, C.c_float, _i, C.c_float, _vp, _vp]),
    "toda_points_box_steps_chunk": (_i, []),
    "toda_points_box_steps": (_i, [_vp, _i, _vp, _i, _vp, _i, _vp, _vp, _vp]),
    "toda_points_column_range_workspace_bytes": (_sz, []),
    "toda_points_column_range": (_i, [_vp, _i, _vp, _i, _i, _vp, _vp, _sz, _vp]),
    "toda_points_in_pyramids": (_i, [_vp, _i, _vp, _i, _vp, _i, _vp, _vp, _vp]),
    "toda_points_fov_flags": (_i, [_vp, _i, _vp, _i, _vp, _vp, _i, _i, _vp, _vp]),
    "toda_sweeps_merge_max_sweeps": (_i, []),
    "toda_sweeps_merge": (_i, [_vp, _i, _i, _vp, _vp, _vp, _vp, _vp, C.c_float, _vp, _vp, _vp, _vp]),
    "toda_waymo_frame": (_i, [_vp, _i, _i, _i, _vp, _vp, _vp]),
    "toda_conv3x3_supported": (_i, [_i, _i, _i, _i, _i]),
    "toda_conv3x3_weight_floats": (_sz, [_i, _i]),
    "toda_conv3x3_transform_weight": (_i, [_vp, _i, _i, _i, _vp, _vp]),
    "toda_conv3x3_transform_weight_batch": (_i, [_vp, _i, _vp]),
    "toda_conv3x3_workspace_bytes": (_sz, []),
    "toda_conv3x3_wgrad_workspace_bytes": (_sz, [_i, _i, _i, _i, _i]),
    "toda_conv3x3_wgrad": (_i, [_vp, _vp, _i, _i, _i, _i, _i, _vp, _vp, _sz, _vp]),
    "toda_conv3x3_fwd": (_i, [_vp, _vp, _vp, _i, _i, _i, _i, _i, _vp, _vp, _sz, _vp]),
    "toda_conv3x3_narrow_supported": (_i, [_i, _i, _i, _i, _i]),
    "toda_conv3x3_narrow_fwd": (_i, [_i, _vp, _vp, _vp, _vp, _i, _i, _i, _i, C.c_longlong, _vp, _vp]),
    "toda_conv3x3_narrow_dgrad": (_i, [_i, _vp, _vp, _vp, _i, _i, _i, _i, C.c_longlong, _vp, _vp]),
    "toda_conv3x3_narrow_wgrad_workspace_bytes": (_sz, [_i, _i, _i, _i]),
    "toda_conv3x3_narrow_wgrad": (_i, [_i, _vp, _vp, _vp, _i, _i, _i, _i, C.c_longlong, _vp, _vp, _sz, _vp]),
    "toda_center_loss_workspace_bytes": (_sz, [_i, _i, _i, _i, _i, _i]),
    "toda_center_loss_fwd": (_i, [_vp, _vp, _i, _i, _i, _i, _i, _vp, _vp, _vp, _vp, _vp, _i, _i, _vp, C.c_float, C.c_float, _vp, _vp, _vp, _sz, _vp]),
    "toda_center_loss_bwd": (_i, [_vp, _vp, _vp, _i, _i, _i, _i, _i, _vp, _vp, _vp, _vp, _i, _i, _vp, C.c_float, C.c_float, _vp, _vp, _sz, _vp]),
    "toda_timing_begin": (_i, [_i]),
    "toda_timing_end": (_i, [_vp, _i, _vp]),
    "toda_center_assign": (_i, [_vp, _i, _i, _i, _i, _i, _i, _vp, _vp, _i, _i, _dbl, _i, _vp, _vp, _vp, _vp, _vp]),
    "toda_anchor_assign_workspace_bytes": (_sz, [_i, _i]),
    "toda_anchor_assign": (_i, [_vp, _vp, _vp, _vp, _vp, _i, _i, _vp, _i, _i, _i, _vp, _i, _i, _i, _i, _vp, _vp, _vp, _vp, _sz, _vp]),
    "toda_eval_overlaps": (_i, [_vp, _vp, _vp, _vp, _vp, _vp, _vp, _i, C.c_longlong, _i, _i, _vp, _vp]),
    "toda_eval_match_workspace_bytes": (_sz, [_i, _i, _i]),
    "toda_eval_match_scores": (_i, [_vp, _vp, _vp, _vp, _vp, _vp, _vp, _i, _i, _dbl, _vp, _vp, _vp, _sz, _vp]),
    "toda_eval_match": (_i, [_vp, _vp, _vp, _vp, _vp, _vp, _vp, _vp, _vp, _vp, _vp, _vp, _i, _i, _vp, _i, _dbl, _i, _i, _vp, _vp, _sz, _vp]),
}

_lib = None


def load():
    global _lib
    if _lib is not None:
        return _lib
    if not os.path.exists(LIB_PATH):
        raise RuntimeError(
            f"{LIB_PATH} not found: build it with `python -c 'import __graft_entry__ as g; g.build()'` "
            "(hipcc --offload-arch=gfx950).  toda_amd has no CPU fallback."
        )
    try:
        lib = C.CDLL(LIB_PATH)
    except OSError as e:
        raise RuntimeError(f"cannot load {LIB_PATH}: {e}") from e
    for name, (res, args) in SIGNATURES.items():
        try:
            fn = getattr(lib, name)
        except AttributeError as e:
            raise RuntimeError(f"{LIB_PATH} does not export {name}") from e
        fn.restype = res
        fn.argtypes = args
    _lib = lib
    return lib


def last_error():
    return load().toda_last_error().decode()


def check(rc, what):
    if rc != 0:
        raise RuntimeError(f"{what} failed (code {rc}): {last_error()}")


def ptr(t):
    if t is None:
        return None
    if not t.is_cuda:
        raise RuntimeError("toda_amd ops need tensors on the GPU (there is no CPU path)")
    if not t.is_contiguous():
        raise RuntimeError("toda_amd ops need contiguous tensors")
    return t.data_ptr()


_raw_stream = getattr(torch._C, "_cuda_getCurrentRawStream", None)
_raw_device = getattr(torch._C, "_cuda_getDevice", None)


def stream():
    if _raw_stream is not None and _raw_device is not None:
        return _raw_stream(_raw_device())
    return torch.cuda.current_stream().cuda_stream


def host_ptrs(tensors):
    return (C.c_void_p * len(tensors))(*[ptr(t) for t in tensors])


def host_addrs(addrs):
    return (C.c_void_p * len(addrs))(*[int(a) for a in addrs])


def host_i32(vals):
    arr = (C.c_int32 * len(vals))(*[int(v) for v in vals])
    return arr


def host_f32(vals):
    arr = (C.c_float * len(vals))(*[float(v) for v in vals])
    return arr


def host_f64(vals):
    arr = (C.c_double * len(vals))(*[float(v) for v in vals])
    return arr


def hptr(arr):
    return C.cast(arr, C.c_void_p)


class Conv3x3WeightEntry(C.Structure):
    _fields_ = [("w", C.c_void_p), ("cout", C.c_int32), ("cin", C.c_int32), ("mode", C.c_int32), ("reserved", C.c_int32), ("u", C.c_void_p)]
```

toda_amd/ops.py:

```python
import numpy as np
import torch

from . import arena as _arena
from . import lib as L


def _triple(v):
    if isinstance(v, (list, tuple)):
        assert len(v) == 3
        return [int(x) for x in v]
    return [int(v)] * 3


def grid_size_xyz(pc_range, voxel_size):
    r = np.asarray(pc_range, dtype=np.float64)
    return np.round((r[3:6] - r[0:3]) / np.asarray(voxel_size, dtype=np.float64)).astype(np.int64)


import os as _os
import time as _time

_COUNT_PINNED = {}
_LAST_WAIT_S = 0.0

# ... 340 lines not shown
        self.n_in, self.n_out = n_in, n_out
        self.nbr_fwd = nbr_fwd
        self.nbr_bwd = nbr_bwd
        self.flip_bwd = flip_bwd
        self.pair_cnt = pair_cnt
        nbr_fwd._toda_pair_cnt = pair_cnt
        if nbr_bwd is not nbr_fwd:
            nbr_bwd._toda_pair_cnt = pair_cnt
        self.geom = geom
        self.in_indices = None
        self._inverse = None
        self._class_order = None

    def class_order(self):
        if (not CLASS_DGRAD or self.kind != "conv" or self.in_indices is None or self.k_vol > 27 or self.k_vol < 2
                or self.n_in < CLASS_DGRAD_MIN_ROWS or any(int(v) not in (1, 2) for v in self.geom["stride"])):
            return None
        if self._class_order is None:
            lib = L.load()
            dev = self.in_indices.device
            order = _alloc((self.n_in,), torch.int32, dev)
            cls = _alloc((self.n_in,), torch.uint8, dev)
            st, pd = L.host_i32(self.geom["stride"]), L.host_i32(self.geom["padding"])
            L.check(lib.toda_rulebook_class_order(L.ptr(self.in_indices), self.n_in, L.hptr(st), L.hptr(pd), L.ptr(order), L.ptr(cls), L.stream()),
                    "toda_rulebook_class_order")
            self._class_order = (order, cls)
        return self._class_order

    def num_pairs(self):
        return int(self.pair_cnt.sum().item())

    def inverse(self):
        if self.kind != "conv":
            raise ValueError("only the tables of a strided SparseConv3d have an inverse")
        if self._inverse is None:
            inv = Rulebook("inverse", self.ksize, self.n_out, self.n_in, self.nbr_bwd, self.nbr_fwd, False, self.pair_cnt, **self.geom)
            self._inverse = inv
        return self._inverse


def conv_out_shape(shape, ksize, stride, padding):
    return [(int(s) + 2 * p - k) // t + 1 for s, k, t, p in zip(shape, ksize, stride, padding)]


def build_subm_rulebook(indices, batch, shape, ksize=3, dilation=1, grid_index=None, pair_cnt=None):
    lib = L.load()
    ks, dl = _triple(ksize), _triple(dilation)
    indices = indices.contiguous()
    assert indices.dtype == torch.int32 and indices.shape[1] == 4
    n = indices.shape[0]
    if grid_index is None:
        grid_index = GridIndex.from_coords_unordered(indices, batch, shape, name=("gi_lazy", tuple(int(v) for v in shape)))
    K = ks[0] * ks[1] * ks[2]
    nbr = _alloc((K, n), torch.int32, indices.device)
    zeroed = pair_cnt is not None
    cnt = pair_cnt if zeroed else torch.empty((K,), dtype=torch.int32, device=indices.device)
    ks_c, dl_c = L.host_i32(ks), L.host_i32(dl)
    rc = lib.toda_rulebook_subm(L.ptr(indices), n, int(batch), L.hptr(grid_index._shape_c), L.hptr(ks_c), L.hptr(dl_c),
                                L.ptr(grid_index.buf), L.ptr(grid_index.rowof), L.ptr(nbr), L.ptr(cnt), int(zeroed), L.stream())
    L.check(rc, "toda_rulebook_subm")
    return Rulebook("subm", ks, n, n, nbr, nbr, True, cnt, dilation=dl), grid_index


def _conv_tables(indices, n_in, idx_out, n_out, batch, shape, out_shape, ks, st, pd, gi_out, gi_in=None, pair_cnt=None):
    lib = L.load()
    dev = indices.device
    K = ks[0] * ks[1] * ks[2]
    o2i = _alloc((K, n_out), torch.int32, dev)
    i2o = _alloc((K, n_in), torch.int32, dev)
    zeroed = pair_cnt is not None
    cnt = pair_cnt if zeroed else torch.empty((K,), dtype=torch.int32, device=dev)
    hs = [L.host_i32(v) for v in (shape, ks, st, pd, out_shape)]
    rc = lib.toda_rulebook_conv(L.ptr(indices), n_in, int(batch), L.hptr(hs[0]), L.hptr(hs[1]), L.hptr(hs[2]), L.hptr(hs[3]),
                                L.hptr(hs[4]), L.ptr(gi_out.buf), n_out, L.ptr(o2i), L.ptr(i2o), L.ptr(cnt),
                                L.ptr(idx_out) if gi_in is not None else None, L.ptr(gi_in.buf) if gi_in is not None else None,
                                L.ptr(gi_in.rowof) if gi_in is not None else None, int(zeroed), L.stream())
    L.check(rc, "toda_rulebook_conv")
    rb = Rulebook("conv", ks, n_in, n_out, o2i, i2o, False, cnt, stride=st, padding=pd, in_shape=[int(v) for v in shape])
    rb.in_indices = indices
    return rb


def _conv_cap(n_upper, batch, out_shape, ks, st):
    per_in = 1
    for k, s_ in zip(ks, st):
        per_in *= -(-k // s_)
    return int(min(n_upper * per_in, batch * out_shape[0] * out_shape[1] * out_shape[2]))


def build_conv_rulebook(indices, batch, shape, ksize, stride, padding):
    lib = L.load()
    ks, st, pd = _triple(ksize), _triple(stride), _triple(padding)
    indices = indices.contiguous()
    assert indices.dtype == torch.int32 and indices.shape[1] == 4
    n_in = indices.shape[0]
    shape = [int(s) for s in shape]
    out_shape = conv_out_shape(shape, ks, st, pd)
    dev = indices.device
    gi_out = GridIndex(batch, out_shape, dev)
    cap = _conv_cap(n_in, batch, out_shape, ks, st)
    idx_out = torch.empty((max(cap, 1), 4), dtype=torch.int32, device=dev)
    n_out_dev = torch.zeros((1,), dtype=torch.int32, device=dev)
    shi, sho = L.host_i32(shape), L.host_i32(out_shape)
    ks_c, st_c, pd_c = L.host_i32(ks), L.host_i32(st), L.host_i32(pd)
    rc = lib.toda_gridindex_from_conv(L.ptr(indices), n_in, None, int(batch), L.hptr(shi), L.hptr(ks_c), L.hptr(st_c),
                                      L.hptr(pd_c), L.hptr(sho), L.ptr(gi_out.buf), L.ptr(idx_out), L.ptr(n_out_dev),
                                      cap, L.stream())
    L.check(rc, "toda_gridindex_from_conv")
    n_out = int(n_out_dev.item())
    if n_out > cap:
        raise RuntimeError(f"strided rulebook: {n_out} outputs exceed the bound {cap}")
    idx_out = idx_out[:n_out]
    rb = _conv_tables(indices, n_in, idx_out, n_out, batch, shape, out_shape, ks, st, pd, gi_out)
    return idx_out, out_shape, rb, gi_out


def _plan_enqueue(level0, batch, shape, steps, counts, c0, gi0=None):
    lib = L.load()
    idx0, n_upper, n_dev = level0
    dev = idx0.device
    slot = _arena.current_slot()
    tag = slot.plans if slot is not None else 0
    if gi0 is None:
        gi0 = GridIndex.unordered_begin(batch, shape, dev, name=("gi0", tag))
    gi0.unordered_build(idx0, n_dev)
    levels = [{"idx": idx0, "n_upper": n_upper, "shape": [int(v) for v in shape], "gi": gi0}]
    li = 0
    for st in steps:
        if st["kind"] != "conv":
            continue
        cur = levels[-1]
        ks, sd, pd = _triple(st["ksize"]), _triple(st["stride"]), _triple(st["padding"])
        out_shape = conv_out_shape(cur["shape"], ks, sd, pd)
        cap = _conv_cap(cur["n_upper"], batch, out_shape, ks, sd)
        li += 1
        shape_c = L.host_i32(out_shape)
        buf, _ = _persistent(("gi", tag, li), (int(batch), tuple(out_shape)), lib.toda_gridindex_bytes(int(batch), L.hptr(shape_c)), dev)
        gi_out = GridIndex(batch, out_shape, dev, buf=buf)
        idx_out = _alloc((max(cap, 1), 4), torch.int32, dev)
        hs = [L.host_i32(v) for v in (cur["shape"], ks, sd, pd, out_shape)]
        rc = lib.toda_gridindex_from_bitmap(L.ptr(cur["gi"].buf), int(batch), L.hptr(hs[0]), L.hptr(hs[1]), L.hptr(hs[2]), L.hptr(hs[3]),
                                            L.hptr(hs[4]), L.ptr(gi_out.buf), L.ptr(idx_out), counts.data_ptr() + 4 * (c0 + li - 1),
                                            cap, 1 if li == 1 else 0, L.stream())
        L.check(rc, "toda_gridindex_from_bitmap")
        levels.append({"idx": idx_out, "n_upper": cap, "shape": out_shape, "gi": gi_out, "cap": cap, "step": st})
    if slot is not None:
        slot.plans += 1
    return levels


def _plan_tables(levels, level_counts, batch, steps, training):
    dev = levels[0]["idx"].device
    for lv, n in zip(levels, level_counts):
        if lv.get("cap") is not None and n > lv["cap"]:
            raise RuntimeError(f"strided rulebook {lv['step']['key']}: {n} outputs exceed the bound {lv['cap']}")
        lv["n"] = int(n)
        lv["idx"] = lv["idx"][:int(n)]
    keys = []
    for st in steps:
        if st["key"] not in keys:
            keys.append(st["key"])
    cnts = torch.zeros((len(keys), 64), dtype=torch.int32, device=dev)
    out = {}
    li = 0
    for st in steps:
        cur = levels[li]
        if st["kind"] == "subm":
            if st["key"] in out:
                continue
            ks = _triple(st["ksize"])
            rb, gi = build_subm_rulebook(cur["idx"], batch, cur["shape"], st["ksize"], st.get("dilation", 1), grid_index=cur["gi"],
                                         pair_cnt=cnts[keys.index(st["key"])][:ks[0] * ks[1] * ks[2]])
            out[st["key"]] = {"kind": "subm", "rb": rb, "n_in": cur["n"]}
        else:
            nxt = levels[li + 1]
            ks, sd, pd = _triple(st["ksize"]), _triple(st["stride"]), _triple(st["padding"])
            rb = _conv_tables(cur["idx"], cur["n"], nxt["idx"], nxt["n"], batch, cur["shape"], nxt["shape"], ks, sd, pd, nxt["gi"],
                              gi_in=cur["gi"], pair_cnt=cnts[keys.index(st["key"])][:ks[0] * ks[1] * ks[2]])
            if training:
                rb.class_order()
            out[st["key"]] = {"kind": "conv", "rb": rb, "n_in": cur["n"], "out_indices": nxt["idx"],
                              "out_shape": nxt["shape"], "gi": nxt["gi"]}
            li += 1
    return out


def build_index_plan(indices, batch, shape, steps, while_waiting=None, training=None):
    indices = indices.contiguous()
    n_conv = sum(1 for st in steps if st["kind"] == "conv")
    counts = _alloc((max(n_conv, 1),), torch.int32, indices.device)
    levels = _plan_enqueue((indices, indices.shape[0], None), batch, shape, steps, counts, 0)
    got = read_counts(counts, while_waiting) if n_conv else []
    if training is None:
        training = torch.is_grad_enabled()
    return _plan_tables(levels, [indices.shape[0]] + list(got[:n_conv]), batch, steps, training)


def build_input_plan(clouds, voxel_cfg, batch, shape, steps, training=True, while_waiting=None):
    n_conv = sum(1 for st in steps if st["kind"] == "conv")
    bsz = len(clouds)
    dev = clouds[0][0].device
    slot = _arena.current_slot()
    gi0 = GridIndex.unordered_begin(batch, shape, dev, name=("gi0", slot.plans if slot is not None else 0))
    counts = _alloc((bsz + 1 + n_conv,), torch.int32, dev)
    voxels, coords, num, _ = voxelize_enqueue(clouds, voxel_cfg["point_cloud_range"], voxel_cfg["voxel_size"],
                                              voxel_cfg["max_points_per_voxel"], voxel_cfg["max_num_voxels"], counts=counts,
                                              tag=slot.plans if slot is not None else 0)
    levels = _plan_enqueue((coords, coords.shape[0], counts[bsz:bsz + 1]), batch, shape, steps, counts, bsz + 1, gi0=gi0)
    got = read_counts(counts, while_waiting)
    m = got[bsz]
    plan = _plan_tables(levels, [m] + list(got[bsz + 1:bsz + 1 + n_conv]), batch, steps, training)
    return voxels[:m], levels[0]["idx"], num[:m], plan


MATRIX_PATHS = ("native", "split")
_MM = None


def matrix_path():
    global _MM
    if _MM is None:
        _MM = MATRIX_PATHS[L.load().toda_matrix_path()]
    return _MM


def set_matrix_path(name):
    global _MM
    L.check(L.load().toda_set_matrix_path(MATRIX_PATHS.index(name)), "toda_set_matrix_path")
    _MM = name


def _tag_mm(wp, cg, cp):
    wp._toda_mm = matrix_path() if L.load().toda_spconv_split_supported(int(cg), int(cp)) else None
    return wp


def _check_mm(wp):
    mm = getattr(wp, "_toda_mm", None)
    if mm is not None and mm != matrix_path():
        raise RuntimeError(f"packed sparse-conv operand was written under matrix path {mm!r}, the current path is {matrix_path()!r}: re-pack it")


def pack_weight(weight, transpose, flip_k):
    lib = L.load()
    cout, cin = weight.shape[0], weight.shape[-1]
    K = weight.numel() // (cout * cin)
    cg, cp = (cout, cin) if transpose else (cin, cout)
    n = lib.toda_spconv_packed_weight_floats(K, cg, cp)
    wp = torch.empty((n,), dtype=torch.float32, device=weight.device)
    rc = lib.toda_spconv_pack_weight(L.ptr(weight.contiguous()), cout, K, cin, int(transpose), int(flip_k), L.ptr(wp),
                                     L.stream())
    L.check(rc, "toda_spconv_pack_weight")
    return _tag_mm(wp, cg, cp)


def pack_weights_batched(items):
    lib = L.load()
    if not items:
        return []
    dev = items[0][0].device
    sizes, couts, ks, cins, pairs = [], [], [], [], []
    for w, tr, _ in items:
        cout, cin = w.shape[0], w.shape[-1]
        K = w.numel() // (cout * cin)
        cg, cp = (cout, cin) if tr else (cin, cout)
        sizes.append(lib.toda_spconv_packed_weight_floats(K, cg, cp))
        couts.append(cout), ks.append(K), cins.append(cin), pairs.append((cg, cp))
    flat = torch.empty((sum(sizes),), dtype=torch.float32, device=dev)
    outs, off = [], 0
    for n, (cg, cp) in zip(sizes, pairs):
        outs.append(_tag_mm(flat[off:off + n], cg, cp))
        off += n
    ws = [w.contiguous() for w, _, _ in items]
    rc = lib.toda_spconv_pack_weights(len(items), L.host_ptrs(ws), L.hptr(L.host_i32(couts)), L.hptr(L.host_i32(ks)), L.hptr(L.host_i32(cins)),
                                      L.hptr(L.host_i32([int(bool(t)) for _, t, _ in items])), L.hptr(L.host_i32([int(bool(f)) for _, _, f in items])),
                                      L.host_ptrs(outs), L.stream())
    L.check(rc, "toda_spconv_pack_weights")
    return outs


def gather_gemm_stats_supported(c_gather, c_produce):
    return bool(L.load().toda_spconv_gather_gemm_stats_supported(int(c_gather), int(c_produce)))


def gather_gemm_with_stats(feat, wp, nbr, c_produce, bias=None, partials=False):
    lib = L.load()
    K, n_out = nbr.shape
    out = torch.empty((n_out, c_produce), dtype=torch.float32, device=feat.device)
    nd = lib.toda_spconv_gather_gemm_stats_doubles(n_out, c_produce)
    sums = torch.empty((nd,), dtype=torch.float64, device=feat.device)
    if partials:
        import ctypes
        blocks = ctypes.c_int(0)
        rc = lib.toda_spconv_gather_gemm_stats_partials(L.ptr(feat), feat.shape[0], feat.shape[1], L.ptr(wp), L.ptr(nbr), n_out, K, c_produce,
                                                        L.ptr(bias), L.ptr(out), L.ptr(sums), nd, ctypes.addressof(blocks), L.stream())
        L.check(rc, "toda_spconv_gather_gemm_stats_partials")
        return out, sums, int(blocks.value)
    rc = lib.toda_spconv_gather_gemm_stats(L.ptr(feat), feat.shape[0], feat.shape[1], L.ptr(wp), L.ptr(nbr), n_out, K, c_produce,
                                           L.ptr(bias), L.ptr(out), L.ptr(sums), nd, L.stream())
    L.check(rc, "toda_spconv_gather_gemm_stats")
    return out, sums


def gather_gemm(feat, wp, nbr, c_produce, bias=None, order=None):
    lib = L.load()
    K, n_out = nbr.shape
    out = torch.empty((n_out, c_produce), dtype=torch.float32, device=feat.device)
    rc = lib.toda_spconv_gather_gemm_ordered(L.ptr(feat), feat.shape[0], feat.shape[1], L.ptr(wp), L.ptr(nbr), n_out, K,
                                             c_produce, L.ptr(bias), L.ptr(out), L.ptr(order), L.stream())
    L.check(rc, "toda_spconv_gather_gemm_ordered")
    return out


def _refuse_retired_knobs():
    retired = [k for k in ("TODA_GG_LINE", "TODA_HALO", "TODA_WG_TILE", "TODA_ROW_ORDER", "TODA_GG_WS", "TODA_GG_STAGE", "TODA_GG_WRES", "TODA_GG_LDS_PF",
                           "TODA_GG_BLK512", "TODA_GG_RT", "TODA_SPLIT_BLK", "TODA_SPLIT_KCS", "TODA_WINO_WGRAD") if _os.environ.get(k, "0") not in ("0", "")]
    if retired:
        raise RuntimeError(f"{', '.join(retired)}: these kernel variants were retired (profiles/EXPERIMENTS.md); unset the variable(s)")
    ablate = [k for k in ("TODA_GG_ABLATE", "TODA_WINO_ABLATE", "TODA_WINO_WG_ABLATE") if _os.environ.get(k, "0") not in ("0", "")]
    if ablate and not _os.environ.get("TODA_HIP_LIB"):
        raise RuntimeError(f"{', '.join(ablate)} only act in a measurement build (-DTODA_ABLATE=1, loaded through TODA_HIP_LIB): the library "
                           "that ships ignores them, and a run that believes it ablated something would report wrong conclusions")


_refuse_retired_knobs()


COMPACT = _os.environ.get("TODA_GG_COMPACT", "1") == "1"


def _compact_route(c_gather, c_produce, nbr):
    return (COMPACT and nbr.shape[0] == 27 and nbr.shape[1] > 0 and c_produce in (16, 32) and c_gather <= 32
            and (c_gather <= 16 or c_produce == 16))


def gather_gemm_compact_supported(c_gather, c_produce, k_vol):
    return bool(L.load().toda_spconv_gather_gemm_compact_supported(int(c_gather), int(c_produce), int(k_vol)))


def gather_gemm_compact(feat, weight, nbr, c_produce, bias=None, transpose=False, flip_k=False, stats=False):
    lib = L.load()
    K, n_out = nbr.shape
    out = torch.empty((n_out, c_produce), dtype=torch.float32, device=feat.device)
    if stats:
        import ctypes
        nd = lib.toda_spconv_gather_gemm_compact_stats_doubles(n_out, c_produce)
        sums = torch.empty((nd,), dtype=torch.float64, device=feat.device)
        blocks = ctypes.c_int(0)
        rc = lib.toda_spconv_gather_gemm_compact_stats(L.ptr(feat), feat.shape[0], feat.shape[1], L.ptr(weight), weight.shape[0], weight.shape[-1],
                                                       int(bool(transpose)), int(bool(flip_k)), L.ptr(nbr), n_out, K, c_produce, L.ptr(bias), L.ptr(out),
                                                       L.ptr(sums), nd, ctypes.addressof(blocks), L.stream())
        L.check(rc, "toda_spconv_gather_gemm_compact_stats")
        return out, sums, int(blocks.value)
    rc = lib.toda_spconv_gather_gemm_compact(L.ptr(feat), feat.shape[0], feat.shape[1], L.ptr(weight), weight.shape[0], weight.shape[-1],
                                             int(bool(transpose)), int(bool(flip_k)), L.ptr(nbr), n_out, K, c_produce, L.ptr(bias), L.ptr(out), L.stream())
    L.check(rc, "toda_spconv_gather_gemm_compact")
    return out


def gather_gemm_classed(feat, wp, nbr, c_produce, order, cls_sorted, ksize, stride, padding):
    lib = L.load()
    K, n_out = nbr.shape
    out = torch.empty((n_out, c_produce), dtype=torch.float32, device=feat.device)
    ks, st, pd = L.host_i32(ksize), L.host_i32(stride), L.host_i32(padding)
    rc = lib.toda_spconv_gather_gemm_classed(L.ptr(feat), feat.shape[0], feat.shape[1], L.ptr(wp), L.ptr(nbr), n_out, K, c_produce, None,
                                             L.ptr(out), L.ptr(order), L.ptr(cls_sorted), L.hptr(ks), L.hptr(st), L.hptr(pd), L.stream())
    L.check(rc, "toda_spconv_gather_gemm_classed")
    return out


def wgrad(feat, dout, nbr, wshape):
    lib = L.load()
    K, n_out = nbr.shape
    cout, cin = wshape[0], wshape[-1]
    dw = torch.empty(wshape, dtype=torch.float32, device=feat.device)
    ws_bytes = lib.toda_spconv_wgrad_workspace_bytes(n_out, K, cin, cout)
    ws = torch.empty((max(ws_bytes, 16),), dtype=torch.uint8, device=feat.device)
    rc = lib.toda_spconv_wgrad(L.ptr(feat), feat.shape[0], L.ptr(dout), L.ptr(nbr), n_out, K, cin, cout, L.ptr(dw),
                               L.ptr(ws), ws_bytes, L.stream())
    L.check(rc, "toda_spconv_wgrad")
    return dw


CLASS_DGRAD = _os.environ.get("TODA_CLASS_DGRAD", "1") == "1"
CLASS_DGRAD_MIN_ROWS = int(_os.environ.get("TODA_CLASS_DGRAD_MIN_ROWS", "4096"))
WGRAD_ON_SIDE_STREAM = _os.environ.get("TODA_WGRAD_STREAM", "0") == "1"
_SIDE_STREAMS = {}


def _side_stream(device):
    key = (device.type, device.index)
    if key not in _SIDE_STREAMS:
        _SIDE_STREAMS[key] = torch.cuda.Stream(device=device)
    return _SIDE_STREAMS[key]


class _SparseConv(torch.autograd.Function):

    @staticmethod
    def forward(ctx, features, weight, bias, rb, wp_fwd, want_stats=False, wp_bwd=None):
        features = features.contiguous()
        compact = _compact_route(features.shape[1], weight.shape[0], rb.nbr_fwd)
        if wp_fwd is None and not compact:
            wp_fwd = pack_weight(weight, False, False)
        if wp_fwd is not None:
            _check_mm(wp_fwd)
        sums, blocks = None, 0
        if compact and want_stats:
            out, sums, blocks = gather_gemm_compact(features, weight.contiguous(), rb.nbr_fwd, weight.shape[0], bias, stats=True)
        elif want_stats and FOLD_IN_FINALIZE:
            out, sums, blocks = gather_gemm_with_stats(features, wp_fwd, rb.nbr_fwd, weight.shape[0], bias, partials=True)
        elif want_stats:
            out, sums = gather_gemm_with_stats(features, wp_fwd, rb.nbr_fwd, weight.shape[0], bias)
        elif compact:
            out = gather_gemm_compact(features, weight.contiguous(), rb.nbr_fwd, weight.shape[0], bias)
        else:
            out = gather_gemm(features, wp_fwd, rb.nbr_fwd, weight.shape[0], bias)
        ctx.set_materialize_grads(False)
        ctx.save_for_backward(features, weight)
        ctx.rb = rb
        ctx.wp_bwd = wp_bwd
        ctx.has_bias = bias is not None
        if want_stats:
            ctx.mark_non_differentiable(sums)
            return out, sums, blocks
        return out

    @staticmethod
    def backward(ctx, gout, *unused):
        features, weight = ctx.saved_tensors
        rb = ctx.rb
        if gout is None:
            return None, None, None, None, None, None, None
        gout = gout.contiguous()
        gfeat = gw = gb = None
        need_d, need_w = ctx.needs_input_grad[0], ctx.needs_input_grad[1]
        side = _side_stream(gout.device) if (need_d and need_w and WGRAD_ON_SIDE_STREAM) else None
        if side is not None:
            main = torch.cuda.current_stream(gout.device)
            side.wait_stream(main)
            with torch.cuda.stream(side):
                gw = wgrad(features, gout, rb.nbr_fwd, tuple(weight.shape))
            for t in (features, gout, rb.nbr_fwd):
                t.record_stream(side)
            need_w = False
        if need_d and _compact_route(gout.shape[1], weight.shape[-1], rb.nbr_bwd):
            gfeat = gather_gemm_compact(gout, weight.contiguous(), rb.nbr_bwd, weight.shape[-1], None, True, rb.flip_bwd)
        elif need_d:
            wp_t = ctx.wp_bwd if ctx.wp_bwd is not None else pack_weight(weight, True, rb.flip_bwd)
            _check_mm(wp_t)
            co = rb.class_order()
            if co is not None:
                gfeat = gather_gemm_classed(gout, wp_t, rb.nbr_bwd, weight.shape[-1], co[0], co[1], rb.ksize, rb.geom["stride"], rb.geom["padding"])
            else:
                gfeat = gather_gemm(gout, wp_t, rb.nbr_bwd, weight.shape[-1], None)
        if need_w:
            gw = wgrad(features, gout, rb.nbr_fwd, tuple(weight.shape))
        if ctx.has_bias and ctx.needs_input_grad[2]:
            gb = _take_colsum(gout)
            if gb is None:
                gb = gout.sum(0)
        if side is not None:
            torch.cuda.current_stream(gout.device).wait_stream(side)
            gw.record_stream(torch.cuda.current_stream(gout.device))
        return gfeat, gw, gb, None, None, None, None


FUSE_BN_STATS = _os.environ.get("TODA_FUSE_BN_STATS", "1") == "1"
FOLD_IN_FINALIZE = _os.environ.get("TODA_BN_FOLD_FINALIZE", "1") == "1"


def sparse_conv(features, weight, bias, rulebook, packed_weight=None, want_stats=False, packed_dgrad=None):
    if not want_stats:
        return _SparseConv.apply(features, weight, bias, rulebook, packed_weight, False, packed_dgrad)
    narrow = FOLD_IN_FINALIZE and _compact_route(features.shape[1], weight.shape[0], rulebook.nbr_fwd)
    ok = (FUSE_BN_STATS and (narrow or gather_gemm_stats_supported(weight.shape[-1], weight.shape[0])) and rulebook.nbr_fwd.shape[1] > 1
          and features.shape[0] > 0)
    if not ok:
        return _SparseConv.apply(features, weight, bias, rulebook, packed_weight, False, packed_dgrad), None
    out, sums, blocks = _SparseConv.apply(features, weight, bias, rulebook, packed_weight, True, packed_dgrad)
    return out, ((sums, blocks) if blocks else sums)


class _ToDense(torch.autograd.Function):
    @staticmethod
    def forward(ctx, features, indices, batch, shape):
        lib = L.load()
        n, c = features.shape
        shape = [int(s) for s in shape]
        dense = torch.empty((batch, c, *shape), dtype=torch.float32, device=features.device)
        sh = L.host_i32(shape)
        rc = lib.toda_sparse_to_dense_fwd(L.ptr(features.contiguous()), L.ptr(indices), n, c, batch, L.hptr(sh),
                                          L.ptr(dense), L.stream())
        L.check(rc, "toda_sparse_to_dense_fwd")
        ctx.save_for_backward(indices)
        ctx.meta = (n, c, batch, shape)
        return dense

    @staticmethod
    def backward(ctx, gdense):
        (indices,) = ctx.saved_tensors
        n, c, batch, shape = ctx.meta
        g = torch.empty((n, c), dtype=torch.float32, device=gdense.device)
        sh = L.host_i32(shape)
        rc = L.load().toda_sparse_to_dense_bwd(L.ptr(gdense.contiguous()), L.ptr(indices), n, c, batch, L.hptr(sh),
                                               L.ptr(g), L.stream())
        L.check(rc, "toda_sparse_to_dense_bwd")
        return g, None, None, None


def sparse_to_dense(features, indices, batch, shape):
    return _ToDense.apply(features, indices.contiguous(), int(batch), shape)


class _PillarScatter(torch.autograd.Function):
    @staticmethod
    def forward(ctx, features, indices, batch, ny, nx):
        n, c = features.shape
        canvas = torch.empty((batch, c, ny, nx), dtype=torch.float32, device=features.device)
        rc = L.load().toda_pillar_scatter_fwd(L.ptr(features.contiguous()), L.ptr(indices), n, c, batch, ny, nx,
                                              L.ptr(canvas), L.stream())
        L.check(rc, "toda_pillar_scatter_fwd")
        ctx.save_for_backward(indices)
        ctx.meta = (n, c, batch, ny, nx)
        return canvas

    @staticmethod
    def backward(ctx, gcanvas):
        (indices,) = ctx.saved_tensors
        n, c, batch, ny, nx = ctx.meta
        g = torch.empty((n, c), dtype=torch.float32, device=gcanvas.device)
        rc = L.load().toda_pillar_scatter_bwd(L.ptr(gcanvas.contiguous()), L.ptr(indices), n, c, batch, ny, nx, L.ptr(g),
                                              L.stream())
        L.check(rc, "toda_pillar_scatter_bwd")
        return g, None, None, None, None


def pillar_scatter(features, indices, batch, ny, nx):
    return _PillarScatter.apply(features, indices.contiguous(), int(batch), int(ny), int(nx))


def rows_moments(x):
    n, c = x.shape
    lib = L.load()
    sums = torch.empty((lib.toda_rows_reduce_doubles(n, c),), dtype=torch.float64, device=x.device)
    L.check(lib.toda_rows_moments(L.ptr(x.contiguous()), n, c, L.ptr(sums), L.stream()), "toda_rows_moments")
    return sums[:2 * c]


def rows_affine_act(x, scale, shift, residual=None, relu=True):
    n, c = x.shape
    y = torch.empty_like(x)
    rc = L.load().toda_rows_affine_act(L.ptr(x.contiguous()), L.ptr(scale.contiguous()), L.ptr(shift.contiguous()),
                                       L.ptr(residual), n, c, int(bool(relu)), L.ptr(y), L.stream())
    L.check(rc, "toda_rows_affine_act")
    return y


_DX_COLSUM = {}
BN_BWD_COLSUM = _os.environ.get("TODA_BN_BWD_COLSUM", "1") == "1"


def _take_colsum(gout):
    ent = _DX_COLSUM.pop(gout.data_ptr(), None) if _DX_COLSUM else None
    if ent is None or ent[0].shape != gout.shape or ent[0]._version != ent[2] or gout.stride() != ent[0].stride():
        return None
    return ent[1]


class _BNRows(torch.autograd.Function):

    @staticmethod
    def forward(ctx, x, weight, bias, running_mean, running_var, training, momentum, eps, relu, residual=None, sums=None, colsum=False):
        lib = L.load()
        if _DX_COLSUM:
            _DX_COLSUM.clear()
        ctx.colsum = bool(colsum) and BN_BWD_COLSUM
        x = x.contiguous()
        residual = residual.contiguous() if residual is not None else None
        n, c = x.shape
        dev = x.device
        stats = torch.empty((4, c), dtype=torch.float32, device=dev)
        if isinstance(sums, tuple) and training:
            part, blocks = sums
            rc = lib.toda_bn_finalize_partials(L.ptr(part), int(blocks), n, c, L.ptr(weight), L.ptr(bias), L.ptr(running_mean), L.ptr(running_var),
                                               float(momentum), float(eps), L.ptr(stats[0]), L.ptr(stats[1]), L.ptr(stats[2]), L.ptr(stats[3]), L.stream())
            L.check(rc, "toda_bn_finalize_partials")
            sums = part
        else:
            if isinstance(sums, tuple):
                sums = None
            sums = _BNRows._finalize(lib, x, n, c, dev, sums, training, weight, bias, running_mean, running_var, momentum, eps, stats)
        y = torch.empty_like(x)
        rc = lib.toda_rows_affine_act(L.ptr(x), L.ptr(stats[2]), L.ptr(stats[3]), L.ptr(residual), n, c, int(bool(relu)), L.ptr(y),
                                      L.stream())
        L.check(rc, "toda_rows_affine_act")
        ctx.save_for_backward(x, stats, weight, residual)
        ctx.meta = (n, c, bool(relu), bool(training))
        return y

    @staticmethod
    def _finalize(lib, x, n, c, dev, sums, training, weight, bias, running_mean, running_var, momentum, eps, stats):
        if sums is None or not training:
            sums = torch.empty((lib.toda_rows_reduce_doubles(n, c),), dtype=torch.float64, device=dev)
            if training:
                L.check(lib.toda_rows_moments(L.ptr(x), n, c, L.ptr(sums), L.stream()), "toda_rows_moments")
        rc = lib.toda_bn_finalize(L.ptr(sums), n, c, L.ptr(weight), L.ptr(bias), L.ptr(running_mean), L.ptr(running_var),
                                  float(momentum), float(eps), int(bool(training)), L.ptr(stats[0]), L.ptr(stats[1]),
                                  L.ptr(stats[2]), L.ptr(stats[3]), L.stream())
        L.check(rc, "toda_bn_finalize")
        return sums

    @staticmethod
    def backward(ctx, gy):
        x, stats, weight, residual = ctx.saved_tensors
        n, c, relu, training = ctx.meta
        gy = gy.contiguous()
        want_res = residual is not None and ctx.needs_input_grad[9]
        if not training:
            pre = x * stats[2] + stats[3]
            if residual is not None:
                pre = pre + residual
            dz = gy * (pre > 0) if relu else gy
            gx = dz * stats[2]
            xhat = (x - stats[0]) * stats[1]
            return gx, (dz * xhat).sum(0), dz.sum(0), None, None, None, None, None, None, (dz if want_res else None), None, None
        sums = torch.empty((L.load().toda_rows_reduce_doubles(n, c),), dtype=torch.float64, device=x.device)
        gx = torch.empty_like(x)
        gamma = weight if weight is not None else torch.ones(c, device=x.device)
        gres = torch.empty_like(x) if want_res else None
        if ctx.colsum:
            lib = L.load()
            cs_ws = torch.empty((lib.toda_rows_bn_bwd_colsum_doubles(n, c),), dtype=torch.float64, device=x.device)
            cs = torch.empty((c,), dtype=torch.float32, device=x.device)
            rc = lib.toda_rows_bn_bwd_res_colsum(L.ptr(gy), L.ptr(x), L.ptr(residual), L.ptr(stats), L.ptr(gamma), n, c, int(relu),
                                                 L.ptr(sums), L.ptr(gx), L.ptr(gres), L.ptr(cs_ws), L.ptr(cs), L.stream())
            L.check(rc, "toda_rows_bn_bwd_res_colsum")
            _DX_COLSUM[gx.data_ptr()] = (gx, cs, gx._version)
        else:
            rc = L.load().toda_rows_bn_bwd_res(L.ptr(gy), L.ptr(x), L.ptr(residual), L.ptr(stats), L.ptr(gamma), n, c, int(relu),
                                               L.ptr(sums), L.ptr(gx), L.ptr(gres), L.stream())
            L.check(rc, "toda_rows_bn_bwd_res")
        gs = sums[2 * c:3 * c].view(torch.float32)
        return gx, gs[c:], gs[:c], None, None, None, None, None, None, gres, None, None


def bn_rows(x, bn, relu, residual=None, sums=None, colsum=False):
    training = bn.training or not bn.track_running_stats
    bump_bn_counter(bn)
    momentum = 0.0 if bn.momentum is None else bn.momentum
    return _BNRows.apply(x, bn.weight, bn.bias, bn.running_mean, bn.running_var, training, momentum, bn.eps, relu, residual, sums, colsum)


def bn_rows_supported(x, bn):
    c = x.shape[1]
    return (type(bn) is torch.nn.BatchNorm1d and x.is_cuda and x.dtype == torch.float32 and 4 <= c <= 128 and 256 % c == 0 and bn.affine and bn.momentum is not None
            and x.shape[0] > 1)


_BN2D_SYNC = {}


def _bn2d_sync(device):
    key = (device.index, L.stream())
    ent = _BN2D_SYNC.get(key)
    if ent is None:
        ent = _BN2D_SYNC[key] = [torch.zeros((L.load().toda_bn2d_sync_bytes(),), dtype=torch.uint8, device=device), 0]
    ent[1] = ent[1] % 0xFFFFFFF0 + 1
    return ent[0], ent[1]


class _BN2d(torch.autograd.Function):

    @staticmethod
    def forward(ctx, x, weight, bias, running_mean, running_var, momentum, eps, relu):
        lib = L.load()
        x = x.contiguous()
        b, c, h, w = x.shape
        y = torch.empty_like(x)
        save = torch.empty((2, c), dtype=torch.float32, device=x.device)
        ws, epoch = _bn2d_sync(x.device)
        rc = lib.toda_bn2d_fwd(L.ptr(x), b, c, h * w, L.ptr(weight), L.ptr(bias), L.ptr(running_mean), L.ptr(running_var), float(momentum),
                               float(eps), int(bool(relu)), L.ptr(y), L.ptr(save), L.ptr(ws), epoch, L.stream())
        L.check(rc, "toda_bn2d_fwd")
        ctx.save_for_backward(x, weight, bias, save)
        ctx.relu = bool(relu)
        return y

    @staticmethod
    def backward(ctx, gy):
        x, weight, bias, save = ctx.saved_tensors
        lib = L.load()
        b, c, h, w = x.shape
        gy = gy.contiguous()
        gx = torch.empty_like(x)
        gwb = torch.empty((2, c), dtype=torch.float32, device=x.device)
        ws, epoch = _bn2d_sync(x.device)
        rc = lib.toda_bn2d_bwd(L.ptr(x), L.ptr(gy), b, c, h * w, L.ptr(weight), L.ptr(bias), L.ptr(save), int(ctx.relu), L.ptr(gx),
                               L.ptr(gwb[0]), L.ptr(gwb[1]), L.ptr(ws), epoch, L.stream())
        L.check(rc, "toda_bn2d_bwd")
        return gx, gwb[0], gwb[1], None, None, None, None, None


class _BN2dCat(torch.autograd.Function):

    @staticmethod
    def forward(ctx, relu, n, *flat):
        lib = L.load()
        items = [flat[7 * i:7 * i + 7] for i in range(n)]
        xs = [it[0].contiguous() for it in items]
        b, _, h, w = xs[0].shape
        chans = [x.shape[1] for x in xs]
        out = torch.empty((b, sum(chans), h, w), dtype=torch.float32, device=xs[0].device)
        saves, c0 = [], 0
        for x, it in zip(xs, items):
            _, weight, bias, rm, rv, momentum, eps = it
            c = x.shape[1]
            save = torch.empty((2, c), dtype=torch.float32, device=x.device)
            ws, epoch = _bn2d_sync(x.device)
            rc = lib.toda_bn2d_fwd_into(L.ptr(x), b, c, h * w, L.ptr(weight), L.ptr(bias), L.ptr(rm), L.ptr(rv), float(momentum), float(eps),
                                        int(bool(relu)), L.ptr(out), out.shape[1], c0, L.ptr(save), L.ptr(ws), epoch, L.stream())
            L.check(rc, "toda_bn2d_fwd_into")
            saves.append(save)
            c0 += c
        ctx.save_for_backward(*xs, *[it[1] for it in items], *[it[2] for it in items], *saves)
        ctx.meta = (bool(relu), n, chans)
        return out

    @staticmethod
    def backward(ctx, g):
        relu, n, chans = ctx.meta
        t = ctx.saved_tensors
        xs, weights, biases, saves = t[:n], t[n:2 * n], t[2 * n:3 * n], t[3 * n:]
        lib = L.load()
        g = g.contiguous()
        b, ctot, h, w = g.shape
        grads, c0 = [], 0
        for x, weight, bias, save, c in zip(xs, weights, biases, saves, chans):
            gx = torch.empty_like(x)
            gwb = torch.empty((2, c), dtype=torch.float32, device=x.device)
            ws, epoch = _bn2d_sync(x.device)
            rc = lib.toda_bn2d_bwd_from(L.ptr(x), L.ptr(g), ctot, c0, b, c, h * w, L.ptr(weight), L.ptr(bias), L.ptr(save), int(relu), L.ptr(gx),
                                        L.ptr(gwb[0]), L.ptr(gwb[1]), L.ptr(ws), epoch, L.stream())
            L.check(rc, "toda_bn2d_bwd_from")
            grads += [gx, gwb[0], gwb[1], None, None, None, None]
            c0 += c
        return (None, None, *grads)


FUSED_BN2D = _os.environ.get("TODA_BN2D", "1") == "1"
BN2D_CAT = _os.environ.get("TODA_BN2D_CAT", "1") == "1"


def bn2d_supported(x, bn):
    if not (FUSED_BN2D and type(bn) is torch.nn.BatchNorm2d and bn.training and bn.affine and bn.track_running_stats and bn.momentum is not None):
        return False
    if not (x.is_cuda and x.dtype == torch.float32 and x.dim() == 4 and x.is_contiguous()):
        return False
    return bool(L.load().toda_bn2d_supported(x.shape[0], x.shape[1], x.shape[2] * x.shape[3]))


def bn2d(x, bn, relu):
    bump_bn_counter(bn)
    return _BN2d.apply(x, bn.weight, bn.bias, bn.running_mean, bn.running_var, bn.momentum, bn.eps, relu)


def bn2d_cat(pairs, relu=True):
    flat = []
    for x, bn in pairs:
        bump_bn_counter(bn)
        flat += [x, bn.weight, bn.bias, bn.running_mean, bn.running_var, bn.momentum, bn.eps]
    return _BN2dCat.apply(relu, len(pairs), *flat)


def bn_relu_tail(seq):
    mods = list(seq)
    if len(mods) >= 2 and type(mods[-1]) is torch.nn.ReLU and type(mods[-2]) is torch.nn.BatchNorm2d:
        return mods[:-2], mods[-2]
    return None


def run_dense_sequential(seq, x):
    mods = list(seq)
    conv3x3_prepack(mods, x)
    i = 0
    while i < len(mods):
        m = mods[i]
        if isinstance(m, torch.nn.Sequential):
            x = run_dense_sequential(m, x)
        elif (type(m) is torch.nn.ZeroPad2d and tuple(m.padding) == (1, 1, 1, 1) and i + 1 < len(mods) and type(mods[i + 1]) is torch.nn.Conv2d
              and mods[i + 1].padding == (0, 0) and conv3x3_supported(x, mods[i + 1])):
            x = conv3x3(x, mods[i + 1].weight, mods[i + 1].bias, conv3x3_prepacked(mods[i + 1]))
            i += 2
            continue
        elif (type(m) is torch.nn.ZeroPad2d and tuple(m.padding) == (1, 1, 1, 1) and i + 1 < len(mods) and conv3x3s2_supported(x, mods[i + 1])):
            x = conv3x3s2(x, mods[i + 1].weight, mods[i + 1].bias)
            i += 2
            continue
        elif deconv_supported(x, m):
            x = deconv(x, m.weight, m.stride[0], m.bias)
        elif type(m) is torch.nn.Conv2d and m.padding == (1, 1) and conv3x3_supported(x, m):
            x = conv3x3(x, m.weight, m.bias, conv3x3_prepacked(m))
        elif type(m) is torch.nn.BatchNorm2d and bn2d_supported(x, m):
            relu = i + 1 < len(mods) and type(mods[i + 1]) is torch.nn.ReLU
            x = bn2d(x, m, relu)
            i += 2 if relu else 1
            continue
        elif type(m) is torch.nn.BatchNorm2d and x.is_cuda and m.track_running_stats and m.momentum is not None:
            bump_bn_counter(m)
            x = torch.nn.functional.batch_norm(x, m.running_mean, m.running_var, m.weight, m.bias, m.training, m.momentum, m.eps)
        else:
            x = m(x)
        i += 1
    return x


DENSE_CONV = _os.environ.get("TODA_DENSE_CONV", "winograd")
_WINO_CACHE = {}


def conv3x3_supported(x, conv):
    if DENSE_CONV != "winograd" or type(conv) is not torch.nn.Conv2d or not x.is_cuda or x.dtype != torch.float32 or x.dim() != 4:
        return False
    if conv.kernel_size != (3, 3) or conv.stride != (1, 1) or conv.dilation != (1, 1) or conv.groups != 1:
        return False
    if conv.padding_mode != "zeros" or conv.in_channels != x.shape[1]:
        return False
    b, c, h, w = x.shape
    return bool(L.load().toda_conv3x3_supported(b, conv.in_channels, conv.out_channels, h, w))


def conv3x3_transform_weight(weight, mode):
    lib = L.load()
    cout, cin = weight.shape[0], weight.shape[1]
    n = lib.toda_conv3x3_weight_floats(cout, cin)
    u = torch.empty((2, n) if mode == 2 else (n,), dtype=torch.float32, device=weight.device)
    L.check(lib.toda_conv3x3_transform_weight(L.ptr(weight.contiguous()), cout, cin, int(mode), L.ptr(u), L.stream()),
            "toda_conv3x3_transform_weight")
    return u


def conv3x3_transform_weights_batched(items):
    lib = L.load()
    if not items:
        return []
    sizes = [lib.toda_conv3x3_weight_floats(w.shape[0], w.shape[1]) * (2 if mode == 2 else 1) for w, mode in items]
    flat = torch.empty((sum(sizes),), dtype=torch.float32, device=items[0][0].device)
    ws = [w.contiguous() for w, _ in items]
    table = (L.Conv3x3WeightEntry * len(items))()
    outs, off = [], 0
    for ent, w, (_, mode), n in zip(table, ws, items, sizes):
        u = flat[off:off + n]
        ent.w, ent.cout, ent.cin, ent.mode, ent.u = L.ptr(w), w.shape[0], w.shape[1], int(mode), L.ptr(u)
        outs.append(u.view(2, n // 2) if mode == 2 else u)
        off += n
    L.check(lib.toda_conv3x3_transform_weight_batch(L.hptr(table), len(items), L.stream()), "toda_conv3x3_transform_weight_batch")
    return outs


_WEIGHT_EPOCH = [0]


def weights_written_in_place():
    _WEIGHT_EPOCH[0] += 1


def _conv3x3_weight_tag(weight):
    return weight._version, weight.data_ptr(), _WEIGHT_EPOCH[0]


def _conv3x3_stack(mods, dx, out):
    prev = None
    for m in mods:
        if isinstance(m, torch.nn.Sequential):
            dx = _conv3x3_stack(list(m), dx, out)
        else:
            if (type(m) is torch.nn.Conv2d and m.kernel_size == (3, 3) and m.stride == (1, 1) and m.dilation == (1, 1) and m.groups == 1
                    and m.padding_mode == "zeros" and m.in_channels % 32 == 0 and m.out_channels % 32 == 0 and m.in_channels > 0
                    and (m.padding == (1, 1) or (m.padding == (0, 0) and type(prev) is torch.nn.ZeroPad2d and tuple(prev.padding) == (1, 1, 1, 1)))
                    and m.weight.is_cuda and m.weight.dtype == torch.float32):
                out.append((m, dx))
            if not dx and torch.is_grad_enabled() and isinstance(m, torch.nn.Module) and any(p.requires_grad for p in m.parameters(recurse=False)):
                dx = True
        prev = m
    return dx


def conv3x3_prepack(mods, x):
    if DENSE_CONV != "winograd" or not x.is_cuda:
        return 0
    stack = []
    _conv3x3_stack(mods, torch.is_grad_enabled() and x.requires_grad, stack)
    stale = []
    for conv, dx in stack:
        ent = conv.__dict__.get("_wino_u")
        tag = _conv3x3_weight_tag(conv.weight)
        if ent is None or ent[0] != tag or (dx and ent[2] is None):
            stale.append((conv, tag, dx))
    if len(stale) < 2:
        return 0
    with torch.no_grad():
        us = conv3x3_transform_weights_batched([(conv.weight.detach(), 2 if dx else 0) for conv, _, dx in stale])
    for (conv, tag, dx), u in zip(stale, us):
        conv.__dict__["_wino_u"] = (tag, u[0], u[1]) if dx else (tag, u, None)
    return len(stale)


def conv3x3_prepacked(conv):
    ent = conv.__dict__.get("_wino_u")
    if ent is not None and ent[0] == _conv3x3_weight_tag(conv.weight):
        return ent[1], ent[2]
    return None


def _conv3x3_workspace(device):
    key = (device.index, L.stream())
    ws = _WINO_CACHE.get(key)
    if ws is None:
        ws = _WINO_CACHE[key] = torch.zeros((L.load().toda_conv3x3_workspace_bytes(),), dtype=torch.uint8, device=device)
    return ws


def conv3x3_run(x, u, bias, cout):
    lib = L.load()
    b, cin, h, w = x.shape
    y = torch.empty((b, cout, h, w), dtype=torch.float32, device=x.device)
    ws = _conv3x3_workspace(x.device)
    L.check(lib.toda_conv3x3_fwd(L.ptr(x), L.ptr(u), L.ptr(bias), b, cin, cout, h, w, L.ptr(y), L.ptr(ws), ws.numel(), L.stream()),
            "toda_conv3x3_fwd")
    return y


# ... 1004 lines not shown
```

Measured before the change: 149.0.

## Fuse BatchNorm-backward reductions into sparse-conv data-gradient gather-GEMM epilogue

Adds a BatchNorm-backward epilogue to the split gather-GEMM kernel. When a sparse conv's data gradient feeds directly into a BN+ReLU backward, the kernel reads the BN input, applies the ReLU mask and accumulates the per-channel dz and dz·xhat partial sums while the output tile is still in registers. BN backward then only folds those partials and applies the dx formula, skipping its own reduction pass over gy and x. This needs Python-side tracking of forward/backward tensor pairs, and the pre-activation is now computed with fp contraction turned off so the masks match. The cost is extra loads of x in the GEMM epilogue and fragile pointer/version matching.

```diff
diff --git a/include/toda.h b/include/toda.h
--- a/include/toda.h
+++ b/include/toda.h
@@ -304,6 +304,19 @@
                                            int n_out, int k_vol, int c_produce, const float* bias , float* out,
                                            double* sums, size_t sums_doubles, int* blocks_out, void* stream);
 
+int toda_spconv_gather_gemm_bnbwd_supported(int c_gather, int c_produce);
+size_t toda_spconv_gather_gemm_bnbwd_doubles(int n_out, int c_produce);
+int toda_spconv_gather_gemm_bnbwd_ordered(const float* in, int n_in, int c_gather, const float* wp, const int32_t* nbr, int n_out, int k_vol,
+                                          int c_produce, float* out, const int32_t* order , const float* bn_x, const float* bn_stats,
+                                          int relu, double* sums, size_t sums_doubles, int* blocks_out, void* stream);
+int toda_spconv_gather_gemm_bnbwd_classed(const float* in, int n_in, int c_gather, const float* wp, const int32_t* nbr, int n_out, int k_vol,
+                                          int c_produce, float* out, const int32_t* order, const unsigned char* cls_sorted, const int32_t* ksize,
+                                          const int32_t* stride, const int32_t* padding, const float* bn_x, const float* bn_stats, int relu,
+                                          double* sums, size_t sums_doubles, int* blocks_out, void* stream);
+int toda_rows_bn_bwd_from_partials(const float* dy, const float* x, const float* stats, const float* gamma, int n, int c, int relu,
+                                   double* sums, int blocks, float* dx, double* colsum_ws , float* dx_colsum ,
+                                   void* stream);
+
 int toda_conv3x3_supported(int batch, int cin, int cout, int H, int W);
 size_t toda_conv3x3_weight_floats(int cout, int cin);
 int toda_conv3x3_transform_weight(const float* w, int cout, int cin, int mode, float* u, void* stream);
diff --git a/toda_amd/csrc/bn_fold.cuh b/toda_amd/csrc/bn_fold.cuh
--- a/toda_amd/csrc/bn_fold.cuh
+++ b/toda_amd/csrc/bn_fold.cuh
@@ -15,6 +15,11 @@
         __syncthreads();
     }
     return part[0];
+}
+
+__device__ __forceinline__ float bn_pre(float x, float scale, float shift) {
+#pragma clang fp contract(off)
+    return x * scale + shift;
 }
 
 __device__ __forceinline__ void bn_write_channel(int ch, float mean, float var, float eps, const float* __restrict__ gamma,
diff --git a/toda_amd/csrc/dense.hip b/toda_amd/csrc/dense.hip
--- a/toda_amd/csrc/dense.hip
+++ b/toda_amd/csrc/dense.hip
@@ -153,7 +153,10 @@
     const int ch = (int)((t0 * 4) % c);
     const f32x4 sc = *reinterpret_cast<const f32x4*>(scale + ch), sf = *reinterpret_cast<const f32x4*>(shift + ch);
     for (long long t = t0; t < n4; t += stride) {
-        f32x4 v = x[t] * sc + sf;
+        const f32x4 xv = x[t];
+        f32x4 v;
+#pragma unroll
+        for (int j = 0; j < 4; ++j) v[j] = bn_pre(xv[j], sc[j], sf[j]);
         if (res) v += res[t];
         if (relu) {
 #pragma unroll
@@ -181,7 +184,7 @@
         const f32x4 rv = r4 ? r4[(size_t)r * lanes + cl] : f32x4{0.f, 0.f, 0.f, 0.f};
 #pragma unroll
         for (int j = 0; j < 4; ++j) {
-            float pre = xv[j] * sc[j] + sf[j];
+            float pre = bn_pre(xv[j], sc[j], sf[j]);
             if (r4) pre += rv[j];
             const float dz = (relu && !(pre > 0.f)) ? 0.f : g[j];
             a[j] = dz;
@@ -219,7 +222,7 @@
         f32x4 out, dzv;
 #pragma unroll
         for (int j = 0; j < 4; ++j) {
-            float pre = xv[j] * sc[j] + sf[j];
+            float pre = bn_pre(xv[j], sc[j], sf[j]);
             if (res) pre += rv[j];
             const float dz = (relu && !(pre > 0.f)) ? 0.f : g[j];
             dzv[j] = dz;
@@ -404,6 +407,24 @@
     return toda_rows_bn_bwd_res(dy, x, nullptr, stats, gamma, n, c, relu, sums, dx, nullptr, stream);
 }
 
+extern "C" int toda_rows_bn_bwd_from_partials(const float* dy, const float* x, const float* stats, const float* gamma, int n, int c,
+                                              int relu, double* sums, int blocks, float* dx, double* colsum_ws, float* dx_colsum,
+                                              void* stream) {
+    hipStream_t s = (hipStream_t)stream;
+    TODA_CHECK_ARG((colsum_ws == nullptr) == (dx_colsum == nullptr), "rows_bn_bwd_from_partials: colsum workspace and result go together");
+    TODA_CHECK_ARG(c >= 4 && c % 4 == 0 && c <= DN_BLOCK / 2 && DN_BLOCK % c == 0,
+                   "rows_bn_bwd_from_partials: channels must be a multiple of 4 dividing 256, <= 128 (got %d)", c);
+    TODA_CHECK_ARG(n >= 1 && blocks >= 1, "rows_bn_bwd_from_partials: rows and partials per column must be >= 1 (got %d, %d)", n, blocks);
+    hipLaunchKernelGGL(fold_partials_kernel, dim3(2 * c), dim3(DN_BLOCK), 0, s, sums, blocks, 2 * c);
+    const long long n4 = (long long)n * c / 4;
+    const int grid = ew_grid(n4, c);
+    hipLaunchKernelGGL(rows_bn_bwd_apply_kernel, dim3(grid), dim3(DN_BLOCK), 0, s, (const f32x4*)dy, (const f32x4*)x, (const f32x4*)nullptr,
+                       stats, gamma, sums, n4, c, n, relu, (f32x4*)dx, (f32x4*)nullptr, colsum_ws);
+    if (dx_colsum) hipLaunchKernelGGL(colsum_fold_kernel, dim3(c), dim3(DN_BLOCK), 0, s, (const double*)colsum_ws, grid, dx_colsum);
+    TODA_LAUNCH_CHECK();
+    return TODA_OK;
+}
+
 extern "C" int toda_bn_finalize_partials(double* sums, int blocks, int n, int c, const float* gamma, const float* beta,
                                          float* running_mean, float* running_var, float momentum, float eps, float* mean,
                                          float* invstd, float* scale, float* shift, void* stream) {
diff --git a/toda_amd/csrc/spconv.hip b/toda_amd/csrc/spconv.hip
--- a/toda_amd/csrc/spconv.hip
+++ b/toda_amd/csrc/spconv.hip
@@ -1245,14 +1245,18 @@
 };
 }
 
-static int gather_route(int c_gather, int c_produce, int n_out, bool stats, bool cls_sorted, GatherRoute* r) {
+static bool gg_bnbwd_supported(int c_gather, int c_produce) {
+    return use_split(c_gather, c_produce) && (c_produce == 32 || c_produce == 64);
+}
+
+static int gather_route(int c_gather, int c_produce, int n_out, bool stats, bool cls_sorted, GatherRoute* r, bool bnbwd = false) {
     const int Q = tiles_pow2(c_gather), NT = tiles_pow2(c_produce);
     const bool vec_ok = (c_gather & 3) == 0;
     static const int env_lds_raw = getenv("TODA_GG_LDS") ? atoi(getenv("TODA_GG_LDS")) : 1;
     const int env_lds = env_lds_raw == 2 ? 1 : (env_lds_raw == 1 ? (Q >= 2 && NT >= Q) : 0);
     r->rt = 2, r->block = SC_BLOCK, r->vec = vec_ok;
     if (use_split(c_gather, c_produce)) {
-        TODA_CHECK_ARG(!(cls_sorted && stats), "gather_gemm (split path): no statistics on a class-sorted launch");
+        TODA_CHECK_ARG(!(cls_sorted && stats) || bnbwd, "gather_gemm (split path): no forward statistics on a class-sorted launch");
         r->family = GatherRoute::SPLIT;
     } else if (vec_ok && Q == 8 && NT == 8 && !cls_sorted) {
         r->family = GatherRoute::LDS_128, r->rt = 1, r->block = 512;
@@ -1270,7 +1274,8 @@
 
 static int gather_gemm_impl(const float* in, int n_in, int c_gather, const float* wp, const int32_t* nbr, int n_out, int k_vol,
                             int c_produce, const float* bias, float* out, const int32_t* order, double* stats, int* blocks_out, void* stream,
-                            const unsigned char* cls_sorted = nullptr, const toda::GatherClasses* cls_table = nullptr) {
+                            const unsigned char* cls_sorted = nullptr, const toda::GatherClasses* cls_table = nullptr,
+                            const toda::BnBwdTap* tap = nullptr) {
     toda::GatherClasses classes = {};
     if (cls_sorted && cls_table) classes = *cls_table;
     else cls_sorted = nullptr;
@@ -1285,17 +1290,28 @@
         return TODA_OK;
     }
     GatherRoute r;
-    const int rc = gather_route(c_gather, c_produce, n_out, stats != nullptr, cls_sorted != nullptr, &r);
+    const int rc = gather_route(c_gather, c_produce, n_out, stats != nullptr, cls_sorted != nullptr, &r, tap != nullptr);
     if (rc != TODA_OK) return rc;
+    TODA_CHECK_ARG(!tap || (r.family == GatherRoute::SPLIT && stats && blocks_out && gg_bnbwd_supported(c_gather, c_produce)),
+                   "gather_gemm: no BatchNorm-backward epilogue for this launch (%d -> %d)", c_gather, c_produce);
     hipStream_t s = (hipStream_t)stream;
     const dim3 grid(r.grid), block(r.block);
     switch (r.family) {
         case GatherRoute::SPLIT:
             with_tiles(c_gather / 32, c_produce / 16, [&](auto kc, auto nt) {
                 constexpr int KC = decltype(kc)::value, NT = decltype(nt)::value;
+                if constexpr (KC <= 4 && (NT == 2 || NT == 4)) {
+                    if (tap) {
+                        GG_LAUNCH(HIP_KERNEL_NAME(gg_split_kernel<KC, NT, 4, (NT == 2), true>), grid, block, 0, s, in, n_in,
+                                  reinterpret_cast<const toda::u32x4*>(wp), nbr, n_out, k_vol, c_produce, bias, out, order, stats, cls_sorted, classes,
+                                  *tap);
+                        return;
+                    }
+                }
                 if constexpr (KC <= 4 && NT >= 2)
                     GG_LAUNCH(HIP_KERNEL_NAME(gg_split_kernel<KC, NT, (NT == 8 ? 3 : 4), (NT == 2)>), grid, block, 0, s, in, n_in,
-                              reinterpret_cast<const toda::u32x4*>(wp), nbr, n_out, k_vol, c_produce, bias, out, order, stats, cls_sorted, classes);
+                              reinterpret_cast<const toda::u32x4*>(wp), nbr, n_out, k_vol, c_produce, bias, out, order, stats, cls_sorted, classes,
+                              toda::NoTap{});
             });
             break;
         case GatherRoute::LDS_128:
@@ -1363,6 +1379,46 @@
     return gather_gemm_impl(in, n_in, c_gather, wp, nbr, n_out, k_vol, c_produce, bias, out, order, nullptr, nullptr, stream, cls_sorted, &table);
 }
 
+extern "C" int toda_spconv_gather_gemm_bnbwd_supported(int c_gather, int c_produce) { return gg_bnbwd_supported(c_gather, c_produce) ? 1 : 0; }
+
+extern "C" size_t toda_spconv_gather_gemm_bnbwd_doubles(int n_out, int c_produce) {
+    return (size_t)2 * c_produce * (1 + (size_t)cdiv(n_out > 0 ? n_out : 1, 128));
+}
+
+static int bnbwd_check(const char* who, int n_in, int c_gather, int n_out, int c_produce, const float* bn_x, const float* bn_stats, const double* sums,
+                       size_t sums_doubles, const int* blocks_out) {
+    TODA_CHECK_ARG(bn_x && bn_stats && sums && blocks_out, "%s: null argument", who);
+    TODA_CHECK_ARG(gg_bnbwd_supported(c_gather, c_produce) && n_out > 0 && n_in > 0, "%s: unsupported channel pair (%d -> %d) or matrix path, or empty table",
+                   who, c_gather, c_produce);
+    TODA_CHECK_ARG(sums_doubles >= toda_spconv_gather_gemm_bnbwd_doubles(n_out, c_produce), "%s: partials buffer too small", who);
+    return TODA_OK;
+}
+
+extern "C" int toda_spconv_gather_gemm_bnbwd_ordered(const float* in, int n_in, int c_gather, const float* wp, const int32_t* nbr, int n_out, int k_vol,
+                                                     int c_produce, float* out, const int32_t* order, const float* bn_x, const float* bn_stats, int relu,
+                                                     double* sums, size_t sums_doubles, int* blocks_out, void* stream) {
+    const int ok = bnbwd_check("gather_gemm_bnbwd_ordered", n_in, c_gather, n_out, c_produce, bn_x, bn_stats, sums, sums_doubles, blocks_out);
+    if (ok != TODA_OK) return ok;
+    const toda::BnBwdTap tap{bn_x, bn_stats, relu};
+    *blocks_out = 0;
+    return gather_gemm_impl(in, n_in, c_gather, wp, nbr, n_out, k_vol, c_produce, nullptr, out, order, sums, blocks_out, stream, nullptr, nullptr, &tap);
+}
+
+extern "C" int toda_spconv_gather_gemm_bnbwd_classed(const float* in, int n_in, int c_gather, const float* wp, const int32_t* nbr, int n_out, int k_vol,
+                                                     int c_produce, float* out, const int32_t* order, const unsigned char* cls_sorted,
+                                                     const int32_t* ksize, const int32_t* stride, const int32_t* padding, const float* bn_x,
+                                                     const float* bn_stats, int relu, double* sums, size_t sums_doubles, int* blocks_out, void* stream) {
+    const int ok = bnbwd_check("gather_gemm_bnbwd_classed", n_in, c_gather, n_out, c_produce, bn_x, bn_stats, sums, sums_doubles, blocks_out);
+    if (ok != TODA_OK) return ok;
+    TODA_CHECK_ARG(order && cls_sorted && ksize && stride && padding, "gather_gemm_bnbwd_classed: null argument");
+    TODA_CHECK_ARG(ksize[0] * ksize[1] * ksize[2] == k_vol, "gather_gemm_bnbwd_classed: kernel size does not match the table's %d offsets", k_vol);
+    GatherClasses table;
+    TODA_CHECK_ARG(class_table(ksize, stride, padding, &table) == 0, "gather_gemm_bnbwd_classed: needs <= 8 residue classes and <= 27 offsets");
+    const toda::BnBwdTap tap{bn_x, bn_stats, relu};
+    *blocks_out = 0;
+    return gather_gemm_impl(in, n_in, c_gather, wp, nbr, n_out, k_vol, c_produce, nullptr, out, order, sums, blocks_out, stream, cls_sorted, &table, &tap);
+}
+
 extern "C" int toda_spconv_gather_gemm_stats_supported(int c_gather, int c_produce) {
     return gg_stats_supported(c_gather, c_produce) ? 1 : 0;
 }
diff --git a/toda_amd/csrc/spconv_split.cuh b/toda_amd/csrc/spconv_split.cuh
--- a/toda_amd/csrc/spconv_split.cuh
+++ b/toda_amd/csrc/spconv_split.cuh
@@ -1,4 +1,7 @@
 #pragma once
+#include <type_traits>
+
+#include "bn_fold.cuh"
 #include "split_common.cuh"
 
 namespace toda {
@@ -87,11 +90,17 @@
                          (unsigned)v[6] | ((unsigned)v[7] << 16)};
 }
 
-template <int KC, int NT, int WAVES, bool IL = false>
+struct BnBwdTap {
+    const float* x;
+    const float* stats;
+    int relu;
+};
+struct NoTap {};
+template <int KC, int NT, int WAVES, bool IL = false, bool BNB = false>
 __global__ void __launch_bounds__(SC_BLOCK, WAVES)
 gg_split_kernel(const float* __restrict__ in, int n_in, const u32x4* __restrict__ wps, const int* __restrict__ nbr, int n_out, int K, int cp,
                 const float* __restrict__ bias, float* __restrict__ out, const int* __restrict__ order, double* __restrict__ stats,
-                const unsigned char* __restrict__ cls_sorted, const GatherClasses classes) {
+                const unsigned char* __restrict__ cls_sorted, const GatherClasses classes, const std::conditional_t<BNB, BnBwdTap, NoTap> tap) {
     constexpr int RT = 2;
     constexpr int CG = 32 * KC;
     constexpr int UNITS = NT * 3;
@@ -305,7 +314,7 @@
         if (++k >= KE) break;
     }
     asm volatile("s_waitcnt vmcnt(0)" ::: "memory");
-    if (row0 >= n_out && !stats) return;
+    if (row0 >= n_out && !(BNB || stats)) return;
 
 #if SP_STAMPS
     if (stats) {
@@ -314,21 +323,90 @@
         stats = nullptr;
     }
 #endif
-    if (stats) {
+    auto store_out = [&]() {
+        const bool full = cp == 16 * NT;
+#pragma unroll
+        for (int rt = 0; rt < RT; ++rt) {
+#pragma unroll
+            for (int reg = 0; reg < 4; ++reg) {
+                const int pos = row0 + rt * 16 + 4 * g + reg;
+                const int row = __shfl(rows[rt], 4 * g + reg, 64);
+                if (pos >= n_out) continue;
+                float* dst = out + (size_t)row * cp + NT * r;
+                if (full) {
+                    if constexpr (NT == 2) {
+                        *reinterpret_cast<float2*>(dst) = make_float2(acc[rt][0][reg], acc[rt][1][reg]);
+                    } else {
+#pragma unroll
+                        for (int n = 0; n < NT; n += 4)
+                            *reinterpret_cast<f32x4*>(dst + n) = f32x4{acc[rt][n][reg], acc[rt][n + 1][reg], acc[rt][n + 2][reg], acc[rt][n + 3][reg]};
+                    }
+                } else {
+#pragma unroll
+                    for (int n = 0; n < NT; ++n)
+                        if (NT * r + n < cp) dst[n] = acc[rt][n][reg];
+                }
+            }
+        }
+    };
+    if (BNB || stats) {
         float (*st_sh)[2][16 * NT] = reinterpret_cast<float (*)[2][16 * NT]>(wl);
         float sm[NT], sq[NT];
 #pragma unroll
+        for (int n = 0; n < NT; ++n) sm[n] = sq[n] = 0.0f;
+        if constexpr (BNB) {
+            float xv[RT][4][NT];
+#pragma unroll
+            for (int rt = 0; rt < RT; ++rt)
+#pragma unroll
+                for (int reg = 0; reg < 4; ++reg) {
+                    const int row = __shfl(rows[rt], 4 * g + reg, 64);
+                    const bool ok = row0 + rt * 16 + 4 * g + reg < n_out;
+                    const float* src = tap.x + (size_t)(ok ? row : 0) * cp + NT * r;
+                    if constexpr (NT == 2) {
+                        const float2 v = *reinterpret_cast<const float2*>(src);
+                        xv[rt][reg][0] = v.x, xv[rt][reg][1] = v.y;
+                    } else {
+#pragma unroll
+                        for (int n = 0; n < NT; n += 4) {
+                            const f32x4 v = *reinterpret_cast<const f32x4*>(src + n);
+#pragma unroll
+                            for (int j = 0; j < 4; ++j) xv[rt][reg][n + j] = v[j];
+                        }
+                    }
+                }
+            asm volatile("" ::: "memory");
+            store_out();
+#pragma unroll
+            for (int n = 0; n < NT; ++n) {
+                const int ch = NT * r + n;
+                const float mu = tap.stats[ch], is = tap.stats[cp + ch], sc = tap.stats[2 * cp + ch], sf = tap.stats[3 * cp + ch];
+#pragma unroll
+                for (int rt = 0; rt < RT; ++rt)
+#pragma unroll
+                    for (int reg = 0; reg < 4; ++reg)
+                        if (row0 + rt * 16 + 4 * g + reg < n_out) {
+                            const float x = xv[rt][reg][n];
+                            const float dz = (tap.relu && !(bn_pre(x, sc, sf) > 0.f)) ? 0.f : acc[rt][n][reg];
+                            sm[n] += dz;
+                            sq[n] += dz * ((x - mu) * is);
+                        }
+            }
+        } else {
+#pragma unroll
+            for (int n = 0; n < NT; ++n)
+#pragma unroll
+                for (int rt = 0; rt < RT; ++rt)
+#pragma unroll
+                    for (int reg = 0; reg < 4; ++reg)
+                        if (row0 + rt * 16 + 4 * g + reg < n_out) {
+                            const float v = acc[rt][n][reg];
+                            sm[n] += v;
+                            sq[n] += v * v;
+                        }
+        }
+#pragma unroll
         for (int n = 0; n < NT; ++n) {
-            sm[n] = sq[n] = 0.0f;
-#pragma unroll
-            for (int rt = 0; rt < RT; ++rt)
-#pragma unroll
-                for (int reg = 0; reg < 4; ++reg)
-                    if (row0 + rt * 16 + 4 * g + reg < n_out) {
-                        const float v = acc[rt][n][reg];
-                        sm[n] += v;
-                        sq[n] += v * v;
-                    }
             sm[n] += __shfl_xor(sm[n], 16, 64);
             sq[n] += __shfl_xor(sq[n], 16, 64);
             sm[n] += __shfl_xor(sm[n], 32, 64);
@@ -348,30 +426,7 @@
         }
     }
 
-    const bool full = cp == 16 * NT;
-#pragma unroll
-    for (int rt = 0; rt < RT; ++rt) {
-#pragma unroll
-        for (int reg = 0; reg < 4; ++reg) {
-            const int pos = row0 + rt * 16 + 4 * g + reg;
-            const int row = __shfl(rows[rt], 4 * g + reg, 64);
-            if (pos >= n_out) continue;
-            float* dst = out + (size_t)row * cp + NT * r;
-            if (full) {
-                if constexpr (NT == 2) {
-                    *reinterpret_cast<float2*>(dst) = make_float2(acc[rt][0][reg], acc[rt][1][reg]);
-                } else {
-#pragma unroll
-                    for (int n = 0; n < NT; n += 4)
-                        *reinterpret_cast<f32x4*>(dst + n) = f32x4{acc[rt][n][reg], acc[rt][n + 1][reg], acc[rt][n + 2][reg], acc[rt][n + 3][reg]};
-                }
-            } else {
-#pragma unroll
-                for (int n = 0; n < NT; ++n)
-                    if (NT * r + n < cp) dst[n] = acc[rt][n][reg];
-            }
-        }
-    }
+    if (!BNB) store_out();
 }
 
 template <int MTB, int NTB, int QM = 1, int QN = 1>
diff --git a/toda_amd/lib.py b/toda_amd/lib.py
--- a/toda_amd/lib.py
+++ b/toda_amd/lib.py
@@ -48,6 +48,10 @@
     "toda_spconv_gather_gemm_stats_doubles": (_sz, [_i, _i]),
     "toda_spconv_gather_gemm_stats": (_i, [_vp, _i, _i, _vp, _vp, _i, _i, _i, _vp, _vp, _vp, _sz, _vp]),
     "toda_spconv_gather_gemm_stats_partials": (_i, [_vp, _i, _i, _vp, _vp, _i, _i, _i, _vp, _vp, _vp, _sz, _vp, _vp]),
+    "toda_spconv_gather_gemm_bnbwd_supported": (_i, [_i, _i]),
+    "toda_spconv_gather_gemm_bnbwd_doubles": (_sz, [_i, _i]),
+    "toda_spconv_gather_gemm_bnbwd_ordered": (_i, [_vp, _i, _i, _vp, _vp, _i, _i, _i, _vp, _vp, _vp, _vp, _i, _vp, _sz, _vp, _vp]),
+    "toda_spconv_gather_gemm_bnbwd_classed": (_i, [_vp, _i, _i, _vp, _vp, _i, _i, _i, _vp, _vp, _vp, _vp, _vp, _vp, _vp, _vp, _i, _vp, _sz, _vp, _vp]),
     "toda_spconv_gather_gemm_compact_supported": (_i, [_i, _i, _i]),
     "toda_spconv_gather_gemm_compact": (_i, [_vp, _i, _i, _vp, _i, _i, _i, _i, _vp, _i, _i, _i, _vp, _vp, _vp]),
     "toda_spconv_gather_gemm_compact_stats_doubles": (_sz, [_i, _i]),
@@ -67,6 +71,7 @@
     "toda_rows_bn_bwd_res": (_i, [_vp, _vp, _vp, _vp, _vp, _i, _i, _i, _vp, _vp, _vp, _vp]),
     "toda_rows_bn_bwd_colsum_doubles": (_sz, [_i, _i]),
     "toda_rows_bn_bwd_res_colsum": (_i, [_vp, _vp, _vp, _vp, _vp, _i, _i, _i, _vp, _vp, _vp, _vp, _vp, _vp]),
+    "toda_rows_bn_bwd_from_partials": (_i, [_vp, _vp, _vp, _vp, _i, _i, _i, _vp, _i, _vp, _vp, _vp, _vp]),
     "toda_conv3x3s2_supported": (_i, [_i, _i, _i, _i, _i]),
     "toda_conv3x3s2_fwd": (_i, [_vp, _vp, _i, _i, _i, _i, _i, _vp, _vp]),
     "toda_conv3x3s2_dgrad": (_i, [_vp, _vp, _i, _i, _i, _i, _i, _vp, _vp]),
diff --git a/toda_amd/ops.py b/toda_amd/ops.py
--- a/toda_amd/ops.py
+++ b/toda_amd/ops.py
@@ -666,7 +666,41 @@
     return out, sums
 
 
+BN_BWD_TAP = _os.environ.get("TODA_BN_BWD_TAP", "1") != "0"
+BN_BWD_TAP_MIN_ROWS = int(_os.environ.get("TODA_BN_BWD_TAP_MIN_ROWS", "0"))
+_BN_TAP_ARG = [None]
+_BN_TAP_RES = [None]
+
+
+def gather_gemm_bnbwd_supported(c_gather, c_produce):
+    return bool(L.load().toda_spconv_gather_gemm_bnbwd_supported(int(c_gather), int(c_produce)))
+
+
+def _bnbwd_launch(entry, feat, wp, nbr, c_produce, order, tap, *geom):
+    import ctypes
+    lib = L.load()
+    K, n_out = nbr.shape
+    bn_x, bn_stats, relu = tap
+    if tuple(bn_x.shape) != (n_out, c_produce) or not bn_x.is_contiguous() or tuple(bn_stats.shape) != (4, c_produce) or not bn_stats.is_contiguous():
+        raise RuntimeError(f"{entry}: the BatchNorm input {tuple(bn_x.shape)} / statistics {tuple(bn_stats.shape)} do not match the launch's "
+                           f"output ({n_out}, {c_produce})")
+    out = torch.empty((n_out, c_produce), dtype=torch.float32, device=feat.device)
+    nd = lib.toda_spconv_gather_gemm_bnbwd_doubles(n_out, c_produce)
+    sums = torch.empty((nd,), dtype=torch.float64, device=feat.device)
+    blocks = ctypes.c_int(0)
+    rc = getattr(lib, entry)(L.ptr(feat), feat.shape[0], feat.shape[1], L.ptr(wp), L.ptr(nbr), n_out, K, c_produce, L.ptr(out), L.ptr(order), *geom,
+                             L.ptr(bn_x), L.ptr(bn_stats), int(bool(relu)), L.ptr(sums), nd, ctypes.addressof(blocks), L.stream())
+    L.check(rc, entry)
+    _BN_TAP_RES[0] = (sums, int(blocks.value))
+    return out
+
+
 def gather_gemm(feat, wp, nbr, c_produce, bias=None, order=None):
+    tap, _BN_TAP_ARG[0] = _BN_TAP_ARG[0], None
+    if tap is not None:
+        if bias is not None:
+            raise RuntimeError("gather_gemm: a launch that takes BatchNorm backward sums is a data gradient and has no bias")
+        return _bnbwd_launch("toda_spconv_gather_gemm_bnbwd_ordered", feat, wp, nbr, c_produce, order, tap)
     lib = L.load()
     K, n_out = nbr.shape
     out = torch.empty((n_out, c_produce), dtype=torch.float32, device=feat.device)
@@ -725,8 +759,12 @@
 def gather_gemm_classed(feat, wp, nbr, c_produce, order, cls_sorted, ksize, stride, padding):
     lib = L.load()
     K, n_out = nbr.shape
+    ks, st, pd = L.host_i32(ksize), L.host_i32(stride), L.host_i32(padding)
+    tap, _BN_TAP_ARG[0] = _BN_TAP_ARG[0], None
+    if tap is not None:
+        return _bnbwd_launch("toda_spconv_gather_gemm_bnbwd_classed", feat, wp, nbr, c_produce, order, tap, L.ptr(cls_sorted), L.hptr(ks), L.hptr(st),
+                             L.hptr(pd))
     out = torch.empty((n_out, c_produce), dtype=torch.float32, device=feat.device)
-    ks, st, pd = L.host_i32(ksize), L.host_i32(stride), L.host_i32(padding)
     rc = lib.toda_spconv_gather_gemm_classed(L.ptr(feat), feat.shape[0], feat.shape[1], L.ptr(wp), L.ptr(nbr), n_out, K, c_produce, None,
                                              L.ptr(out), L.ptr(order), L.ptr(cls_sorted), L.hptr(ks), L.hptr(st), L.hptr(pd), L.stream())
     L.check(rc, "toda_spconv_gather_gemm_classed")
@@ -757,6 +795,37 @@
     if key not in _SIDE_STREAMS:
         _SIDE_STREAMS[key] = torch.cuda.Stream(device=device)
     return _SIDE_STREAMS[key]
+
+
+_BN_TAP_FWD = {}
+_BN_TAP_BWD = {}
+
+
+def _bn_tap_claim(features, weight, rb):
+    ent = _BN_TAP_FWD.get(features.data_ptr()) if _BN_TAP_FWD else None
+    if ent is None:
+        return None
+    ent[5] += 1
+    y = ent[0]
+    cout, cin = weight.shape[0], weight.shape[-1]
+    if (y.shape != features.shape or y.stride() != features.stride() or y._version != ent[1] or features.shape[0] < BN_BWD_TAP_MIN_ROWS
+            or _compact_route(cout, cin, rb.nbr_bwd) or not gather_gemm_bnbwd_supported(cout, cin)):
+        return None
+    return ent
+
+
+def _bn_tap_valid(ent, features):
+    if ent is None or ent[5] != 1 or ent[0]._version != ent[1] or ent[2]._version != ent[6] or ent[0].data_ptr() != features.data_ptr():
+        return None
+    return ent
+
+
+def _bn_tap_take(gy, x, stats, relu):
+    ent = _BN_TAP_BWD.pop(gy.data_ptr(), None) if _BN_TAP_BWD else None
+    if (ent is None or ent[0].shape != gy.shape or ent[0]._version != ent[3] or gy.stride() != ent[0].stride() or ent[4].data_ptr() != x.data_ptr()
+            or ent[5].data_ptr() != stats.data_ptr() or ent[6] != relu or ent[4].shape != x.shape):
+        return None
+    return ent[1], ent[2]
 
 
 class _SparseConv(torch.autograd.Function):
@@ -781,6 +850,8 @@
         else:
             out = gather_gemm(features, wp_fwd, rb.nbr_fwd, weight.shape[0], bias)
         ctx.set_materialize_grads(False)
+        tap = _bn_tap_claim(features, weight, rb)
+        ctx.bn_tap = tap if ctx.needs_input_grad[0] else None
         ctx.save_for_backward(features, weight)
         ctx.rb = rb
         ctx.wp_bwd = wp_bwd
@@ -814,10 +885,19 @@
             wp_t = ctx.wp_bwd if ctx.wp_bwd is not None else pack_weight(weight, True, rb.flip_bwd)
             _check_mm(wp_t)
             co = rb.class_order()
-            if co is not None:
-                gfeat = gather_gemm_classed(gout, wp_t, rb.nbr_bwd, weight.shape[-1], co[0], co[1], rb.ksize, rb.geom["stride"], rb.geom["padding"])
-            else:
-                gfeat = gather_gemm(gout, wp_t, rb.nbr_bwd, weight.shape[-1], None)
+            tap = _bn_tap_valid(ctx.bn_tap, features)
+            _BN_TAP_RES[0] = None
+            _BN_TAP_ARG[0] = (tap[2], tap[3], tap[4]) if tap is not None else None
+            try:
+                if co is not None:
+                    gfeat = gather_gemm_classed(gout, wp_t, rb.nbr_bwd, weight.shape[-1], co[0], co[1], rb.ksize, rb.geom["stride"], rb.geom["padding"])
+                else:
+                    gfeat = gather_gemm(gout, wp_t, rb.nbr_bwd, weight.shape[-1], None)
+            finally:
+                _BN_TAP_ARG[0] = None
+            res, _BN_TAP_RES[0] = _BN_TAP_RES[0], None
+            if tap is not None and res is not None:
+                _BN_TAP_BWD[gfeat.data_ptr()] = (gfeat, res[0], res[1], gfeat._version, tap[2], tap[3], tap[4])
         if need_w:
             gw = wgrad(features, gout, rb.nbr_fwd, tuple(weight.shape))
         if ctx.has_bias and ctx.needs_input_grad[2]:
@@ -939,6 +1019,10 @@
         lib = L.load()
         if _DX_COLSUM:
             _DX_COLSUM.clear()
+        if _BN_TAP_FWD:
+            _BN_TAP_FWD.clear()
+        if _BN_TAP_BWD:
+            _BN_TAP_BWD.clear()
         ctx.colsum = bool(colsum) and BN_BWD_COLSUM
         x = x.contiguous()
         residual = residual.contiguous() if residual is not None else None
@@ -961,6 +1045,8 @@
         L.check(rc, "toda_rows_affine_act")
         ctx.save_for_backward(x, stats, weight, residual)
         ctx.meta = (n, c, bool(relu), bool(training))
+        if BN_BWD_TAP and training and residual is None and c in (32, 64) and n > 0 and matrix_path() == "split":
+            _BN_TAP_FWD[y.data_ptr()] = [y, y._version, x, stats, bool(relu), 0, x._version]
         return y
 
     @staticmethod
@@ -989,9 +1075,24 @@
             gx = dz * stats[2]
             xhat = (x - stats[0]) * stats[1]
             return gx, (dz * xhat).sum(0), dz.sum(0), None, None, None, None, None, None, (dz if want_res else None), None, None
-        sums = torch.empty((L.load().toda_rows_reduce_doubles(n, c),), dtype=torch.float64, device=x.device)
         gx = torch.empty_like(x)
         gamma = weight if weight is not None else torch.ones(c, device=x.device)
+        tapped = _bn_tap_take(gy, x, stats, relu) if residual is None else None
+        if tapped is not None:
+            lib = L.load()
+            sums, blocks = tapped
+            cs_ws = cs = None
+            if ctx.colsum:
+                cs_ws = torch.empty((lib.toda_rows_bn_bwd_colsum_doubles(n, c),), dtype=torch.float64, device=x.device)
+                cs = torch.empty((c,), dtype=torch.float32, device=x.device)
+            rc = lib.toda_rows_bn_bwd_from_partials(L.ptr(gy), L.ptr(x), L.ptr(stats), L.ptr(gamma), n, c, int(relu), L.ptr(sums), blocks, L.ptr(gx),
+                                                    L.ptr(cs_ws), L.ptr(cs), L.stream())
+            L.check(rc, "toda_rows_bn_bwd_from_partials")
+            if ctx.colsum:
+                _DX_COLSUM[gx.data_ptr()] = (gx, cs, gx._version)
+            gs = sums[2 * c:3 * c].view(torch.float32)
+            return gx, gs[c:], gs[:c], None, None, None, None, None, None, None, None, None
+        sums = torch.empty((L.load().toda_rows_reduce_doubles(n, c),), dtype=torch.float64, device=x.device)
         gres = torch.empty_like(x) if want_res else None
         if ctx.colsum:
             lib = L.load()
```

New measurement: 149.9, median of 6. About the same (+0.6%).
